# TAMUCrypto/virgo-plus

Measured on AMD Instinct MI355X. Metric: prover sec + field-ops/sec, SHA-256 circuit, 1/2/4/8 MI355X (bit-exact), higher is better.
Workload: dtype u64 (F_p^2, p=2^61-1); 1 GPU; SHA-256 1024-block circuit (SHA256_64.pws x1024, 102347776 gates, 15 layers, 2^23 input wires), GKR sumcheck + Virgo FFT/LDT commit on GPU (BASELINE configs[2]); pass_mode=sync, field_ops_per_proof=8299342697

## Files before the change

include/vpgpu.h:

```cpp
#ifndef VPGPU_H
#define VPGPU_H
#include <stdint.h>
#ifdef __cplusplus
extern "C" {
#endif

typedef struct vp_ctx vp_ctx;
typedef struct { uint64_t real, img; } vp_F;

enum {
    VP_OK = 0,
    VP_EINVAL = -1,
    VP_EHIP = -2,
    VP_ENOGPU = -3,
    VP_EASSERT = -4,
    VP_ELIMIT = -5,
    VP_EXCHANGE = 1
};

enum { VP_MUL = 0, VP_ADD, VP_SUB, VP_ANTISUB, VP_NAAB, VP_ANTINAAB, VP_INPUT, VP_MULC, VP_ADDC, VP_XOR, VP_NOT, VP_COPY };

typedef struct {
    uint64_t size;
    int32_t bit_length;
// ... 17 lines not shown
    int32_t plan_autotune;
    int32_t real_values;
    int32_t real_pairs;
    int32_t pc_tensor_pub;
    int32_t persistent_rounds;
    int32_t persistent_timeout_ms;
    int32_t poll;
    int32_t prefetch_round1;
    int32_t interactive_fast_init;
    int32_t split_cost_percent;
    int32_t debug;
    int32_t reserved[4];
} vp_options;
void vp_options_default(vp_options *opt);

int vp_create(int device, vp_ctx **out);
int vp_create_with_options(int device, const vp_options *opt, vp_ctx **out);
int vp_get_options(const vp_ctx *, vp_options *out);
int vp_tuning_get(const vp_ctx *, const char *name, int32_t *value);
int vp_test_drivers(void);
int vp_plan_tuning_get(const vp_ctx *, int32_t v[6]);
int vp_plan_tuning_set(vp_ctx *, const int32_t v[6]);
#define VP_WARM_COMMITMENT 1u
#define VP_WARM_FFT_GKR 2u
int vp_warm(vp_ctx *, uint32_t what);
void vp_destroy(vp_ctx *);
const char *vp_last_error(const vp_ctx *);
const char *vp_version(void);
int vp_checked_build(void);

int vp_circuit_upload(vp_ctx *, int n_layers, const vp_layer_desc *layers);

int vp_evaluate(vp_ctx *, const vp_F *inputs, uint64_t n_inputs);
int vp_layer_values(vp_ctx *, int layer, vp_F *out, uint64_t n);

int vp_vres(vp_ctx *, const vp_F *r_0, int r_0_size, vp_F *out);

int vp_phase1_init(vp_ctx *, int layer, const vp_F *r_liu, const vp_F *assert_random);
int vp_phase2_init(vp_ctx *, int layer, const vp_F *r_u);
int vp_liu_init(vp_ctx *, int layer, const vp_F *r_u, const vp_F *const *r_v, const vp_F *s);

int vp_round(vp_ctx *, const vp_F *previous_random, vp_F out_poly[3]);

int vp_finalize(vp_ctx *, const vp_F *previous_random, vp_F *claims, int n_claims);

int vp_prove_gkr(vp_ctx *, const vp_F *tape, uint64_t n_tape, uint8_t *transcript, uint64_t capacity,
                 uint64_t *n_written);
int vp_gkr_sizes(vp_ctx *, uint64_t *n_tape, uint64_t *n_transcript_bytes);

int vp_set_shard(vp_ctx *, int rank, int world);
int vp_set_shard_split(vp_ctx *, int min_log);
int vp_shard_finish(vp_ctx *, uint8_t *summed, uint64_t n_bytes, uint64_t *n_transcript_bytes);
int vp_set_round_shard(vp_ctx *, int rank, int world, int min_log);
int vp_get_round_shard(vp_ctx *, int *rank, int *world, int *split_live);
int vp_shard_vu_partials(vp_ctx *, const vp_F *tape, uint64_t n_tape, vp_F *partials, uint64_t capacity, uint64_t *n);
int vp_shard_vu_set(vp_ctx *, const vp_F *sums, uint64_t n);
int vp_shard_chains(vp_ctx *, int32_t *owner, double *cost, int capacity, int *n_chains);

int vp_commit_private(vp_ctx *, uint8_t root[32]);
int vp_commit_public(vp_ctx *, const vp_F *pub, uint64_t n_pub, vp_F *inner_product_sum, vp_F all_sum[65],
                     uint8_t root_h[32]);
int vp_commit_public_eq(vp_ctx *, const vp_F *point, int n_point, vp_F *inner_product_sum, vp_F all_sum[65], uint8_t root_h[32]);
int vp_fri_step(vp_ctx *, const vp_F *r, uint8_t root[32]);
int vp_fri_commit(vp_ctx *, const vp_F *r, int n_steps, uint8_t *roots);
int vp_fri_final(vp_ctx *, vp_F *final_code);
int vp_fri_open(vp_ctx *, int oracle, uint64_t leaf, vp_F values[130], uint8_t *path, int path_capacity, int *path_len);
int vp_fri_open_many(vp_ctx *, int n, const int32_t *oracle, const uint64_t *leaf, vp_F *values , uint8_t *paths, int path_stride,
                     int32_t *path_len );
int vp_fri_query_bytes(vp_ctx *, int n_queries, uint64_t *bytes);
int vp_fri_query(vp_ctx *, int n_queries, const uint64_t *leaf0, uint8_t *out, uint64_t capacity, uint64_t *n_written);
int vp_fft_gkr_sizes(int lg, uint64_t *n_tape, uint64_t *n_msgs);
int vp_fft_gkr(vp_ctx *, int lg, const vp_F *tape, uint64_t n_tape, vp_F *msgs, uint64_t capacity, uint64_t *n_written);
int vp_fft_gkr_begin(vp_ctx *, int lg, const vp_F *tape, uint64_t n_tape);
int vp_fft_gkr_end(vp_ctx *, vp_F *msgs, uint64_t capacity, uint64_t *n_written);
int vp_fft_gkr_cancel(vp_ctx *);
int vp_commit_private_masked(vp_ctx *, const vp_F *mask, uint64_t n_mask, uint8_t root[32]);
int vp_commit_public_masked(vp_ctx *, const vp_F *pub, uint64_t n_pub, const vp_F *pub_mask, uint64_t n_pub_mask, vp_F *inner, vp_F all_sum[65], uint8_t root_h[32]);
int vp_fri_final_mask(vp_ctx *, vp_F out[32]);
int vp_commit_stats(vp_ctx *, double *commit_ms);

int vp_set_deferred(vp_ctx *, int on);
int vp_flush(vp_ctx *, int count);
int vp_pending(vp_ctx *, int *n);
int vp_phase_ms(vp_ctx *, double out[5]);
int vp_commit_private_state(vp_ctx *, uint64_t *epoch, int *valid);

int vp_pc_load_input(vp_ctx *, const vp_F *inputs, uint64_t n_inputs, int bit_length);
int vp_pc_set_shard(vp_ctx *, int rank, int world);
int vp_shard_exchange_local(vp_ctx **ctxs, int world);
int vp_pc_shard_owner(vp_ctx *, int oracle, uint64_t leaf);
int vp_shard_pending(vp_ctx *, int *n);
int vp_shard_exchange_info(vp_ctx *, int i, int *kind, uint64_t *bytes);
int vp_shard_exchange_get(vp_ctx *, int i, void *host_send);
int vp_shard_exchange_put(vp_ctx *, int i, const void *host_recv);
int vp_shard_exchange_done(vp_ctx *);
int vp_comm_unique_id(uint8_t id[128]);
int vp_comm_init(vp_ctx *, const uint8_t id[128], int rank, int world);
int vp_comm_destroy(vp_ctx *);
int vp_comm_count(vp_ctx *, int *n_ranks);
int vp_allreduce_u64(vp_ctx *, void *device_buffer, uint64_t count);

int vp_predicates(vp_ctx *, int layer, const vp_F *r_g, const vp_F *assert_random, const vp_F *r_u, const vp_F *r_v, int n_v,
                  vp_F *out, uint64_t n_out);

int vp_liu_gr(vp_ctx *, int layer, const vp_F *r_u, const vp_F *const *r_v, const vp_F *s, const vp_F *r_liu, vp_F *out);
int vp_layer_mle(vp_ctx *, int layer, const vp_F *r, int n, vp_F *out);

typedef struct {
    double gkr_ms;
    double evaluate_ms;
    double fold_ms;
    uint64_t fold_launches;
    uint64_t fold_bytes;
    uint64_t rounds;
    uint64_t launches;
} vp_stats;
int vp_get_stats(vp_ctx *, vp_stats *out);
typedef struct {
    int32_t phase, layer, round, how, tables;
    uint64_t bytes;
    double us;
} vp_round_stat;
int vp_get_round_stats(vp_ctx *, vp_round_stat *out, int capacity, int *n);
int vp_get_resident_resumes(const vp_ctx *, uint64_t *n);
int vp_set_profiling(vp_ctx *, int level);

enum { VP_K_BETA = 0, VP_K_LIGHT, VP_K_CHUNKS, VP_K_COMBINE, VP_K_DOT, VP_K_DOTFIN, VP_K_SFGEN, VP_K_SF, VP_K_SEG, VP_K_EMIT,
       VP_K_FIXUP, VP_K_NTT_SPLIT, VP_K_NTT_LDS, VP_K_NTT_UNSPLIT, VP_K_LEAF_HASH, VP_K_MERKLE, VP_K_PC_POINTWISE, VP_K_FRI_FOLD,
       VP_K_ROUND, VP_K_NTT8_COLS, VP_K_NTT8_ROWS, VP_K_NTT_LONG_SPLIT, VP_K_NTT_LONG_MERGE, VP_K_PC_OPEN_MANY, VP_K_COUNT };
typedef struct {
    int32_t kind;
    int32_t step;
    uint32_t workgroups;
    uint32_t jobs;
    uint32_t rounds, first_round;
    uint64_t bytes;
    uint64_t work;
    double us;
} vp_launch_stat;
int vp_get_launch_stats(vp_ctx *, vp_launch_stat *out, int capacity, int *n);
const char *vp_kernel_name(int kind);

int vp_test_field(vp_ctx *, int op, const vp_F *a, const vp_F *b, vp_F *out, uint64_t n);
int vp_test_beta(vp_ctx *, const vp_F *r, int n, const vp_F *init, vp_F *out);
int vp_test_sha3(vp_ctx *, const uint8_t *in, uint8_t *out, uint64_t n);
int vp_test_fft(vp_ctx *, const vp_F *coefs, int coef_len, int order, int inverse, vp_F *out);

#ifdef __cplusplus
}
#endif
#endif
```

virgo-plus_amd/__init__.py:

```python
import ctypes
import os
import shutil
import subprocess

PKG_DIR = os.path.dirname(os.path.abspath(__file__))
ROOT = os.path.dirname(PKG_DIR)
CSRC = os.path.join(PKG_DIR, "csrc")
HOST = os.path.join(PKG_DIR, "host")
LIB_GPU = os.environ.get("VP_LIBGPU") or os.path.join(CSRC, "libvpgpu.so")
LIB_GPU_CHECKED = os.path.join(ROOT, "tools", "_build", "checked", "libvpgpu.so")
LIB_GPU_TESTDRV = os.path.join(ROOT, "tools", "_build", "testdrv", "libvpgpu.so")
LIB_HOST = os.path.join(HOST, "libvphost.so")
CLI = os.path.join(HOST, "virgo_plus_run")

GPU_SRC = [os.path.join(CSRC, f) for f in ("vpgpu.hip", "vpgpu_batched.inc", "vpgpu_pc.inc", "vpgpu_pc_shard.inc", "vpgpu_fftgkr.inc", "vpgpu_upload.inc", "vp_kernels_fftgkr.h", "vp_kernels.h", "vp_kernels_round.h", "vp_kernels_persist.h", "vp_kernels_batch.h",
                                              "vp_kernels_plan.h", "vp_kernels_pc.h", "vp_kernels_ntt8.h", "vp_kernels_ntt_long.h", "vp_keccak_asm.h", "vp_check.h", "vp_field.h")] + [
    os.path.join(ROOT, "include", "vpgpu.h")]
HOST_SRC = [os.path.join(HOST, f) for f in ("circuit.cpp", "prover.cpp", "verifier.cpp", "vphost.cpp")]
HOST_HDR = [os.path.join(HOST, f) for f in ("circuit.hpp", "prover.hpp", "verifier.hpp", "vphost.h", "field.hpp",
                                              "polynomial.hpp")]


def _stale(target, sources):
    if not os.path.exists(target):
# ... 10 lines not shown


def build(force=False, verbose=False):
    def run(cmd):
        if verbose:
            print(" ".join(cmd), flush=True)
        subprocess.run(cmd, check=True)

    if os.environ.get("VP_LIBGPU"):
        pass
    elif force or _stale(LIB_GPU, GPU_SRC):
        hipcc = _hipcc()
        if hipcc is None:
            if os.path.exists(LIB_GPU):
                return
            raise RuntimeError("hipcc not found and no prebuilt libvpgpu.so")
        run([hipcc, "--offload-arch=gfx950", "-O3", "-std=c++17", "-fPIC", "-shared", "-Wno-unused-value",
             "-o", LIB_GPU, os.path.join(CSRC, "vpgpu.hip")])
    if (force or _stale(LIB_GPU_CHECKED, GPU_SRC)) and _hipcc() is not None:
        os.makedirs(os.path.dirname(LIB_GPU_CHECKED), exist_ok=True)
        run([_hipcc(), "--offload-arch=gfx950", "-O3", "-std=c++17", "-fPIC", "-shared", "-Wno-unused-value", "-DVP_CHECKED",
             "-o", LIB_GPU_CHECKED, os.path.join(CSRC, "vpgpu.hip")])
    if (force or _stale(LIB_GPU_TESTDRV, GPU_SRC)) and _hipcc() is not None:
        os.makedirs(os.path.dirname(LIB_GPU_TESTDRV), exist_ok=True)
        run([_hipcc(), "--offload-arch=gfx950", "-O3", "-std=c++17", "-fPIC", "-shared", "-Wno-unused-value", "-DVP_TEST_DRIVERS",
             "-o", LIB_GPU_TESTDRV, os.path.join(CSRC, "vpgpu.hip")])
    if force or _stale(LIB_HOST, HOST_SRC + HOST_HDR + [LIB_GPU]):
        run(["g++", "-std=c++17", "-O2", "-fPIC", "-shared", "-Wall", "-pthread", "-o", LIB_HOST] + HOST_SRC +
            ["-L" + CSRC, "-lvpgpu", "-Wl,-rpath,$ORIGIN/../csrc", "-Wl,-rpath,/opt/rocm/lib"])
    if force or _stale(CLI, [os.path.join(HOST, "virgo_plus_run.cpp"), LIB_HOST]):
        run(["g++", "-std=c++17", "-O2", "-Wall", "-pthread", "-o", CLI, os.path.join(HOST, "virgo_plus_run.cpp"),
             "-L" + HOST, "-lvphost", "-L" + CSRC, "-lvpgpu", "-Wl,-rpath,$ORIGIN", "-Wl,-rpath,$ORIGIN/../csrc",
             "-Wl,-rpath,/opt/rocm/lib"])


class VphResult(ctypes.Structure):
    _fields_ = [("prove_sec", ctypes.c_double), ("gkr_device_ms", ctypes.c_double), ("evaluate_ms", ctypes.c_double),
                ("verify_sec", ctypes.c_double), ("fold_ms", ctypes.c_double), ("fold_launches", ctypes.c_uint64),
                ("fold_bytes", ctypes.c_uint64), ("rounds", ctypes.c_uint64), ("launches", ctypes.c_uint64),
                ("proof_kb", ctypes.c_double), ("verified", ctypes.c_int)]

    def as_dict(self):
        return {k: getattr(self, k) for k, _ in self._fields_}


class RoundStat(ctypes.Structure):
    _fields_ = [("phase", ctypes.c_int32), ("layer", ctypes.c_int32), ("round", ctypes.c_int32), ("how", ctypes.c_int32), ("tables", ctypes.c_int32),
                ("bytes", ctypes.c_uint64), ("us", ctypes.c_double)]


class LaunchStat(ctypes.Structure):
    _fields_ = [("kind", ctypes.c_int32), ("step", ctypes.c_int32), ("workgroups", ctypes.c_uint32), ("jobs", ctypes.c_uint32),
                ("rounds", ctypes.c_uint32), ("first_round", ctypes.c_uint32), ("bytes", ctypes.c_uint64), ("work", ctypes.c_uint64),
                ("us", ctypes.c_double)]


_gpu = None
_host = None


def lib_gpu():
    global _gpu
    if _gpu is None:
        if not os.path.exists(LIB_GPU):
            raise RuntimeError("libvpgpu.so is not built: run __graft_entry__.build()")
        L = ctypes.CDLL(LIB_GPU, mode=ctypes.RTLD_GLOBAL)
        vp = ctypes.c_void_p
        L.vp_create.argtypes = [ctypes.c_int, ctypes.POINTER(vp)]
        L.vp_create_with_options.argtypes = [ctypes.c_int, vp, ctypes.POINTER(vp)]
        L.vp_get_options.argtypes = [vp, vp]
        L.vp_get_resident_resumes.argtypes = [vp, ctypes.POINTER(ctypes.c_uint64)]
        L.vp_set_shard_split.argtypes = [vp, ctypes.c_int]
        L.vp_set_round_shard.argtypes = [vp, ctypes.c_int, ctypes.c_int, ctypes.c_int]
        L.vp_get_round_shard.argtypes = [vp, ctypes.POINTER(ctypes.c_int), ctypes.POINTER(ctypes.c_int), ctypes.POINTER(ctypes.c_int)]
        L.vp_shard_finish.argtypes = [vp, vp, ctypes.c_uint64, vp]
        L.vp_gkr_sizes.argtypes = [vp, vp, vp]
        L.vp_options_default.argtypes = [vp]
        L.vp_tuning_get.argtypes = [vp, ctypes.c_char_p, ctypes.POINTER(ctypes.c_int32)]
        u64_ = ctypes.c_uint64
        L.vp_set_deferred.argtypes = [vp, ctypes.c_int]
        L.vp_warm.argtypes = [vp, ctypes.c_uint32]
        L.vp_flush.argtypes = [vp, ctypes.c_int]
        L.vp_pending.argtypes = [vp, ctypes.POINTER(ctypes.c_int)]
        L.vp_phase_ms.argtypes = [vp, ctypes.POINTER(ctypes.c_double)]
        L.vp_commit_private.argtypes = [vp, vp]
        L.vp_fft_gkr_sizes.argtypes = [ctypes.c_int, vp, vp]
        L.vp_fft_gkr.argtypes = [vp, ctypes.c_int, vp, u64_, vp, u64_, vp]
        L.vp_fft_gkr_begin.argtypes = [vp, ctypes.c_int, vp, u64_]
        L.vp_fft_gkr_end.argtypes = [vp, vp, u64_, vp]
        L.vp_fft_gkr_cancel.argtypes = [vp]
        L.vp_options_default.restype = None
        L.vp_destroy.argtypes = [vp]
        L.vp_last_error.argtypes = [vp]
        L.vp_last_error.restype = ctypes.c_char_p
        L.vp_version.restype = ctypes.c_char_p
        L.vp_test_field.argtypes = [vp, ctypes.c_int, vp, vp, vp, ctypes.c_uint64]
        L.vp_test_beta.argtypes = [vp, vp, ctypes.c_int, vp, vp]
        L.vp_test_sha3.argtypes = [vp, vp, vp, ctypes.c_uint64]
        L.vp_test_fft.argtypes = [vp, vp, ctypes.c_int, ctypes.c_int, ctypes.c_int, vp]
        L.vp_pc_load_input.argtypes = [vp, vp, ctypes.c_uint64, ctypes.c_int]
        L.vp_pc_set_shard.argtypes = [vp, ctypes.c_int, ctypes.c_int]
        L.vp_shard_exchange_local.argtypes = [ctypes.POINTER(vp), ctypes.c_int]
        L.vp_commit_private.argtypes = [vp, vp]
        L.vp_commit_public.argtypes = [vp, vp, ctypes.c_uint64, vp, vp, vp]
        L.vp_commit_public_eq.argtypes = [vp, vp, ctypes.c_int, vp, vp, vp]
        L.vp_fri_commit.argtypes = [vp, vp, ctypes.c_int, vp]
        L.vp_fri_step.argtypes = [vp, vp, vp]
        L.vp_commit_private_masked.argtypes = [vp, vp, ctypes.c_uint64, vp]
        L.vp_shard_pending.argtypes = [vp, ctypes.POINTER(ctypes.c_int)]
        L.vp_pc_shard_owner.argtypes = [vp, ctypes.c_int, ctypes.c_uint64]
        L.vp_fri_final.argtypes = [vp, vp]
        L.vp_fri_open.argtypes = [vp, ctypes.c_int, ctypes.c_uint64, vp, vp, ctypes.c_int, ctypes.POINTER(ctypes.c_int)]
        L.vp_fri_open_many.argtypes = [vp, ctypes.c_int, vp, vp, vp, vp, ctypes.c_int, vp]
        L.vp_fri_query_bytes.argtypes = [vp, ctypes.c_int, ctypes.POINTER(ctypes.c_uint64)]
        L.vp_fri_query.argtypes = [vp, ctypes.c_int, vp, vp, ctypes.c_uint64, ctypes.POINTER(ctypes.c_uint64)]
        L.vp_commit_stats.argtypes = [vp, ctypes.POINTER(ctypes.c_double)]
        L.vp_comm_unique_id.argtypes = [vp]
        L.vp_comm_init.argtypes = [vp, vp, ctypes.c_int, ctypes.c_int]
        L.vp_comm_destroy.argtypes = [vp]
        L.vp_comm_count.argtypes = [vp, ctypes.POINTER(ctypes.c_int)]
        L.vp_get_round_stats.argtypes = [vp, ctypes.POINTER(RoundStat), ctypes.c_int, ctypes.POINTER(ctypes.c_int)]
        L.vp_allreduce_u64.argtypes = [vp, vp, ctypes.c_uint64]
        L.vp_set_profiling.argtypes = [vp, ctypes.c_int]
        L.vp_get_launch_stats.argtypes = [vp, ctypes.POINTER(LaunchStat), ctypes.c_int, ctypes.POINTER(ctypes.c_int)]
        L.vp_kernel_name.argtypes = [ctypes.c_int]
        L.vp_kernel_name.restype = ctypes.c_char_p
        _gpu = L
    return _gpu


def lib_host():
    global _host
    if _host is None:
        lib_gpu()
        if not os.path.exists(LIB_HOST):
            raise RuntimeError("libvphost.so is not built: run __graft_entry__.build()")
        L = ctypes.CDLL(LIB_HOST)
        vp = ctypes.c_void_p
        u64 = ctypes.c_uint64
        L.vph_circuit_from_pws.restype = vp
        L.vph_circuit_from_pws.argtypes = [ctypes.c_char_p, ctypes.c_int, ctypes.c_long, ctypes.c_char_p, ctypes.c_int]
        L.vph_circuit_randomize.restype = vp
        L.vph_circuit_randomize.argtypes = [ctypes.c_int, ctypes.c_int, ctypes.c_long]
        L.vph_circuit_custom.restype = vp
        L.vph_circuit_custom.argtypes = [ctypes.c_int] + [vp] * 7
        L.vph_circuit_free.argtypes = [vp]
        L.vph_circuit_layers.argtypes = [vp]
        L.vph_circuit_gates.restype = u64
        L.vph_circuit_gates.argtypes = [vp]
        L.vph_circuit_layer_size.restype = u64
        L.vph_circuit_layer_size.argtypes = [vp, ctypes.c_int]
        L.vph_circuit_layer_bitlen.argtypes = [vp, ctypes.c_int]
        L.vph_circuit_hash.argtypes = [vp, ctypes.POINTER(u64)]
        L.vph_session_create.restype = vp
        L.vph_session_create.argtypes = [vp, ctypes.c_int, ctypes.c_char_p, ctypes.c_int]
        L.vph_session_create_opts.restype = vp
        L.vph_session_create_opts.argtypes = [vp, ctypes.c_int, vp, ctypes.c_char_p, ctypes.c_int]
        L.vph_session_create_round_sharded.restype = vp
        L.vph_session_create_round_sharded.argtypes = [vp, ctypes.POINTER(ctypes.c_int), ctypes.c_int, ctypes.c_int, vp, ctypes.c_char_p, ctypes.c_int]
        L.vph_session_create_sharded.restype = vp
        L.vph_session_create_sharded.argtypes = [vp, ctypes.POINTER(ctypes.c_int), ctypes.c_int, ctypes.c_int, ctypes.c_int, vp, ctypes.c_char_p, ctypes.c_int]
        L.vph_commit_private_masked.argtypes = [vp, vp, u64, vp, ctypes.POINTER(ctypes.c_double), ctypes.c_char_p, ctypes.c_int]
        L.vph_commit_public_eq.argtypes = [vp, vp, ctypes.c_int, vp, ctypes.POINTER(ctypes.c_double), ctypes.c_char_p, ctypes.c_int]
        L.vph_fri_open_many.argtypes = [vp, ctypes.c_int, vp, vp, vp, vp, ctypes.c_int, vp, ctypes.c_char_p, ctypes.c_int]
        L.vph_fri_query.argtypes = [vp, ctypes.c_int, vp, vp, u64, ctypes.POINTER(u64), ctypes.c_char_p, ctypes.c_int]
        L.vph_session_rank_ctx.restype = vp
# ... 623 lines not shown
        if lib_host().vph_shard_vu_set(self.h, a.ctypes.data, int(a.shape[0])):
            raise RuntimeError("shard_vu_set refused")

    def shard_finish(self, summed):
        ctx = lib_host().vph_session_ctx(self.h)
        buf = ctypes.create_string_buffer(bytes(summed), len(summed))
        n = ctypes.c_uint64(0)
        if lib_gpu().vp_shard_finish(ctx, buf, len(summed), ctypes.byref(n)):
            raise RuntimeError("shard_finish refused")
        return buf.raw[:int(n.value)]

    def shard_chains(self):
        import numpy as np
        cap = 3 * self.circuit.layers + 1
        owner = np.zeros(cap, dtype=np.int32)
        cost = np.zeros(cap, dtype=np.float64)
        n = lib_host().vph_shard_chains(self.h, owner.ctypes.data, cost.ctypes.data, cap)
        if n < 0:
            raise RuntimeError("shard_chains failed")
        return owner[:n].copy(), cost[:n].copy()

    def commit_private(self, mask=None):
        root = ctypes.create_string_buffer(32)
        ms = ctypes.c_double(0)
        err = ctypes.create_string_buffer(512)
        if mask is not None:
            import numpy as np
            mask = np.ascontiguousarray(mask, dtype=np.uint64).reshape(-1, 2)
            rc = lib_host().vph_commit_private_masked(self.h, mask.ctypes.data, mask.shape[0], ctypes.cast(root, ctypes.c_void_p), ctypes.byref(ms), err, len(err))
        else:
            rc = lib_host().vph_commit_private(self.h, ctypes.cast(root, ctypes.c_void_p), ctypes.byref(ms), err, len(err))
        if rc:
            raise RuntimeError("commit_private failed: " + err.value.decode())
        return root.raw, ms.value

    def commit_public(self, pub):
        import numpy as np
        pub = np.ascontiguousarray(pub, dtype=np.uint64)
        out = ctypes.create_string_buffer(32 + 16 + 65 * 16)
        ms = ctypes.c_double(0)
        err = ctypes.create_string_buffer(512)
        rc = lib_host().vph_commit_public(self.h, pub.ctypes.data, pub.shape[0], ctypes.cast(out, ctypes.c_void_p), ctypes.byref(ms),
                                          err, len(err))
        if rc:
            raise RuntimeError("commit_public failed: " + err.value.decode())
        return out.raw[:32], out.raw[32:48], out.raw[48:], ms.value

    def prove_full(self, batched=False):
        cap = self._cap + 32 + 32 + 16 + 65 * 16
        buf = ctypes.create_string_buffer(cap)
        n = ctypes.c_uint64(0)
        err = ctypes.create_string_buffer(512)
        rc = lib_host().vph_prove_full(self.h, ctypes.cast(buf, ctypes.c_void_p), cap, ctypes.byref(n), 1 if batched else 0, err, len(err))
        if rc < 0:
            raise RuntimeError("prove_full failed: " + err.value.decode())
        return buf.raw[: n.value], rc == 0

    def commit_public_eq(self, point):
        import numpy as np
        point = np.ascontiguousarray(point, dtype=np.uint64)
        out = ctypes.create_string_buffer(32 + 16 + 65 * 16)
        if self._shard_pc:
            ms = ctypes.c_double(0)
            err = ctypes.create_string_buffer(512)
            if lib_host().vph_commit_public_eq(self.h, point.ctypes.data, point.shape[0], ctypes.cast(out, ctypes.c_void_p), ctypes.byref(ms), err, len(err)):
                raise RuntimeError("vp_commit_public_eq failed: " + err.value.decode())
            return out.raw[:32], out.raw[32:48], out.raw[48:], ms.value
        ctx = lib_host().vph_session_ctx(self.h)
        base = ctypes.addressof(out)
        rc = lib_gpu().vp_commit_public_eq(ctx, point.ctypes.data, point.shape[0], base + 32, base + 48, base)
        if rc:
            raise RuntimeError("vp_commit_public_eq failed: %d %s" % (rc, (lib_gpu().vp_last_error(ctx) or b"").decode()))
        return out.raw[:32], out.raw[32:48], out.raw[48:], self.commit_device_ms()

    def warm(self):
        ctx = lib_host().vph_session_ctx(self.h)
        if lib_gpu().vp_warm(ctx, 3):
            raise RuntimeError("vp_warm failed: " + (lib_gpu().vp_last_error(ctx) or b"").decode())

    def draw_protocol_tape(self):
        if lib_host().vph_draw_protocol_tape(self.h):
            raise RuntimeError("draw_protocol_tape: the commitment needs an input layer of at least 2^7 wires")

    def prove_protocol(self, deferred=False, queue_next=False):
        import numpy as np
        if not hasattr(self, "_pp"):
            cap = self._cap + 32 + 32 + 16 + 65 * 16
            self._pp = (ctypes.create_string_buffer(cap), cap, ctypes.create_string_buffer(32 * 32), np.zeros((2048, 2), dtype=np.uint64),
                        (ctypes.c_double * 6)(), ctypes.c_uint64(0), ctypes.create_string_buffer(512))
        buf, cap, roots, fin, sec, n, err = self._pp
        rc = lib_host().vph_prove_protocol_ex(self.h, ctypes.cast(buf, ctypes.c_void_p), cap, ctypes.byref(n), ctypes.cast(roots, ctypes.c_void_p), len(roots),
                                              fin.ctypes.data, sec, (1 if deferred or queue_next else 0) | (2 if queue_next else 0), err, len(err))
        if rc:
            raise RuntimeError("prove_protocol failed: " + err.value.decode())
        st = self.circuit.layer_bitlen(0) - 6
        return (buf.raw[: n.value], roots.raw[:32 * st], fin.copy(),
                {"total": sec[0], "commit_private": sec[1], "gkr": sec[2], "commit_public": sec[3], "fft_gkr": sec[4], "fri_commit": sec[5]})

    def prove_and_verify_full(self, reps=33, batched_openings=False):
        cap = self._cap + 32 + 32 + 16 + 65 * 16
        buf = ctypes.create_string_buffer(cap)
        n = ctypes.c_uint64(0)
        t = [ctypes.c_double(0) for _ in range(3)]
        err = ctypes.create_string_buffer(512)
        if batched_openings:
            rc = lib_host().vph_prove_and_verify_full_ex(self.h, reps, 1, ctypes.cast(buf, ctypes.c_void_p), cap, ctypes.byref(n),
                                                         ctypes.byref(t[0]), ctypes.byref(t[1]), ctypes.byref(t[2]), err, len(err))
        else:
            rc = lib_host().vph_prove_and_verify_full(self.h, reps, ctypes.cast(buf, ctypes.c_void_p), cap, ctypes.byref(n),
                                                      ctypes.byref(t[0]), ctypes.byref(t[1]), ctypes.byref(t[2]), err, len(err))
        if rc < 0:
            raise RuntimeError("prove_and_verify_full failed: " + err.value.decode())
        pt = (ctypes.c_double * 3)()
        lib_host().vph_last_pc_times(self.h, pt)
        return buf.raw[: n.value], rc == 0, {"gkr_prove_sec": t[0].value, "pc_prove_sec": t[1].value, "verify_sec": t[2].value,
                                            "pc_fft_gkr_sec": pt[1], "pc_query_answer_sec": pt[2]}

    def last_full_record(self):
        n = ctypes.c_uint64(0)
        lib_host().vph_last_full_record(self.h, None, 0, ctypes.byref(n))
        if not n.value:
            raise RuntimeError("no accepted complete-protocol run on this session yet")
        buf = ctypes.create_string_buffer(n.value)
        if lib_host().vph_last_full_record(self.h, ctypes.cast(buf, ctypes.c_void_p), n.value, ctypes.byref(n)):
            raise RuntimeError("vph_last_full_record failed")
        return buf.raw[: n.value]

    def fri_open_many(self, requests, path_stride=OPEN_PATH_STRIDE):
        if self._shard_pc:
            import numpy as np
            n = len(requests)
            oracle = np.ascontiguousarray([r[0] for r in requests], dtype=np.int32).reshape(n)
            leaf = np.ascontiguousarray([r[1] for r in requests], dtype=np.uint64).reshape(n)
            v = np.zeros((max(n, 1), 130, 2), dtype=np.uint64)
            p = np.zeros((max(n, 1), max(path_stride, 1)), dtype=np.uint8)
            pl = np.zeros(max(n, 1), dtype=np.int32)
            err = ctypes.create_string_buffer(512)
            if lib_host().vph_fri_open_many(self.h, n, oracle.ctypes.data, leaf.ctypes.data, v.ctypes.data, p.ctypes.data, path_stride, pl.ctypes.data, err, len(err)):
                raise RuntimeError("vp_fri_open_many failed: " + err.value.decode())
            return v[:n], p[:n], pl[:n]
        ctx = self.gpu_ctx()
        rc, v, p, pl = fri_open_many(ctx, requests, path_stride)
        if rc:
            raise RuntimeError("vp_fri_open_many failed: %d %s" % (rc, (lib_gpu().vp_last_error(ctx) or b"").decode()))
        return v, p, pl

    def fri_query(self, leaf0):
        if self._shard_pc:
            import numpy as np
            leaf0 = np.ascontiguousarray(leaf0, dtype=np.uint64)
            n_bits = self.circuit.layer_bitlen(0)
            cap = leaf0.shape[0] * sum(2080 + 32 * d for d in [n_bits - 1, n_bits - 1] + [n_bits - 2 - k for k in range(n_bits - 6)])
            out = ctypes.create_string_buffer(max(cap, 1))
            n = ctypes.c_uint64(0)
            err = ctypes.create_string_buffer(512)
            if lib_host().vph_fri_query(self.h, leaf0.shape[0], leaf0.ctypes.data, ctypes.cast(out, ctypes.c_void_p), cap, ctypes.byref(n), err, len(err)):
                raise RuntimeError("vp_fri_query failed: " + err.value.decode())
            return out.raw[: n.value]
        ctx = self.gpu_ctx()
        rc, out = fri_query(ctx, leaf0)
        if rc:
            raise RuntimeError("vp_fri_query failed: %d %s" % (rc, (lib_gpu().vp_last_error(ctx) or b"").decode()))
        return out

    def last_fft_gkr(self):
        import numpy as np
        out = np.zeros((4096, 2), dtype=np.uint64)
        n = lib_host().vph_last_fft_gkr(self.h, out.ctypes.data, out.shape[0])
        if n < 0:
            raise RuntimeError("no complete-protocol run on this session yet")
        return out[:n].tobytes()

    def last_fri(self):
        import numpy as np
        roots = ctypes.create_string_buffer(32 * 32)
# ... 50 lines not shown
```

virgo-plus_amd/csrc/vpgpu.hip:

```cpp
#include <hip/hip_runtime.h>

#include <algorithm>
#include <chrono>
#include <cstdio>
#include <cstring>
#include <deque>
#include <functional>
#include <map>
#include <mutex>
#include <set>
#include <atomic>
#include <string>
#include <thread>
#include <vector>

#include "../../include/vpgpu.h"
#include "vp_kernels.h"

using namespace vp;

static_assert(sizeof(vp_F) == sizeof(F), "vp_F layout");

namespace {

// ... 113 lines not shown
    int32_t persistent_rounds, poll, debug, prefetch_round1, split_cost_percent;
    int32_t kernel_copies;
    int32_t fold_branches;
    int32_t fuse_combine;
    int32_t plan_autotune, pc_tensor_pub, persistent_timeout_ms;
    int32_t graph_explicit;
    int32_t ntt_r8;
    int32_t interactive_fast_init;
    int32_t fuse_p2;
    int32_t leaf_asm;
    int32_t real_pairs;
    int32_t fft_gkr_batched;
    int32_t split_vu;
};

struct vp_ctx {
    int device = 0;
    hipStream_t stream = nullptr;
    std::string err = "";
    int n_layers = 0, max_bl = 0;
    std::vector<LayerDev> L;
    F **d_vals = nullptr;
    unsigned long long **d_valsr = nullptr;
    F *beta_g = nullptr, *beta_u = nullptr, *bf = nullptr, *bs = nullptr, *liu_half = nullptr;
    u32 half_cap = 0;
    F *tab[2][3] = {{nullptr, nullptr, nullptr}, {nullptr, nullptr, nullptr}};
    u32 cap = 0;
    F *partials = nullptr;
    unsigned int *round_arrivals = nullptr;
    F *small = nullptr;
    F *chunk_part = nullptr; u32 chunk_cap = 0;
    F *d_tape = nullptr; u64 n_tape = 0;
    F *d_tr = nullptr; u64 n_tr = 0;
    F *h_pin = nullptr;
    unsigned long long *h_seq = nullptr, seq = 0;
    TailMail *h_req = nullptr; TailReply *h_rep = nullptr; std::atomic<bool> tail_active{false}; unsigned long long tail_seq = 0; int tail_enabled = 1;
    PTailArgs tail_args{}; F *tail_save = nullptr; bool tail_suspended = false, tail_lost = false; u64 tail_resumes = 0;
    TailAux *h_aux = nullptr;
    int poll = 1;
    F *h_io = nullptr; size_t h_io_cap = 0;
    int r1_pending = 0;
    vp_F r1_stash[3];
    F *h_stage = nullptr; u32 stage_at = 0;
    VpOpt opt{};
    int *d_flag = nullptr;
    u32 *d_vcplx = nullptr;
    int vreal = 0, plan_vreal = 0;
    bool evaluated = false;
    SumcheckState sc;
    std::vector<u64> ru_off, as_off, rv_off, sig_off, rliu_off;
    int profiling = 0;
    vp_stats st{};
    std::vector<EvPair> ev_pool; size_t ev_used = 0;
    std::vector<vp_launch_stat> lstats;
    std::vector<vp_round_stat> rlog;
    int rlog_round = 0;
    u64 rec_gen_bytes = 0, rec_gen_work = 0;
    hipEvent_t ev0 = nullptr, ev1 = nullptr;
    std::vector<void *> allocs;
    BetaJob *all_jobs = nullptr; u32 n_all_jobs = 0, beta_bpj = 1; F *half_pool = nullptr;
    F *pc_rt = nullptr, *pc_coef = nullptr, *pc_cw = nullptr; Dig *pc_tree = nullptr; int pc_lm = -1; double commit_ms = 0;
    std::map<std::pair<const void *, int>, F *> pc_rtc;
    F *pc_q0 = nullptr, *pc_eq = nullptr, *pc_cbuf = nullptr; int pc_cbuf_lm = -1; int *pc_flag = nullptr; bool pc_q_tensor = false;
    F *pc_pub = nullptr, *pc_qcw = nullptr, *pc_hcw = nullptr, *pc_tmp = nullptr, *pc_small = nullptr; Dig *pc_tree_h = nullptr; bool pc_private_done = false;
    F *pc_scr = nullptr; size_t pc_scr_cap = 0;
    F *pc_fri_all = nullptr; std::vector<size_t> fri_cw_off, fri_tree_off; F *pc_open_buf = nullptr;
    PcOpenRec *pc_many_buf = nullptr; unsigned char *pc_many_in = nullptr; u32 pc_many_cap = 0; unsigned char *h_many = nullptr; size_t h_many_cap = 0;
    Dig *pc_fri_roots = nullptr;
    F *pc_fri[2] = {nullptr, nullptr}; Dig *pc_fri_tree = nullptr; int fri_step = -1; size_t fri_tree_used = 0; bool pc_public_done = false;
    u32 pc_mask_ms = 0; F *pc_lm_cw = nullptr, *pc_qm_cw = nullptr, *pc_hm_cw = nullptr, *pc_fm = nullptr, *pc_mtmp = nullptr; std::vector<size_t> fri_m_off;
    size_t pc_mtmp_cap = 0, pc_mB = 0;

    int deferred = 0;
    struct Pending { hipEvent_t a, b; int phase; std::function<int(float)> fin; };
    std::deque<Pending> pending;
    std::vector<hipEvent_t> ev_spare;
    unsigned char *h_ring = nullptr; size_t ring_cap = 0, ring_at = 0;
    size_t ring_live = 0, ring_call = 0;
    double phase_ms[8] = {0, 0, 0, 0, 0, 0, 0, 0};
    std::string plan_cache_path;
    bool pc_dry = false;
    unsigned char *h_pub = nullptr; size_t h_pub_cap = 0;
    u64 private_epoch = 0;

    PcShard *pcs = nullptr;
    FgkState *fgk = nullptr;
    VpComm *cm = nullptr;
    F *part2 = nullptr;
    int simple_path = 0, serial = 0;
    Lane lane0; Lane *ln = nullptr;
    std::vector<Lane> lanes;
    std::vector<hipStream_t> lane_streams; std::vector<hipEvent_t> lane_events; hipEvent_t ev_fork = nullptr;
    F *pred_r = nullptr, *pred_pool = nullptr, *pred_part = nullptr, *pred_out = nullptr; BetaJob *pred_jobs = nullptr; u32 pred_bpj = 1;
    DotJob *pred_dot = nullptr; BlkMap *pred_map = nullptr;
    PlanRec *rec = nullptr;
    DotJob rec_dot{};
    SfGenJob rec_gen{};
    int fuse_init = 1;
    Plan *plan = nullptr; int plan_path = 1;
    std::recursive_mutex mu;
    bool plan_tuned = false;
    bool plan_tune_cached = false;
    int leaf_attr_done = 0;
    uint32_t opt_pinned = 0;
    hipGraphExec_t gkr_graph = nullptr; int use_graph = 1; bool graph_failed = false; u64 graph_launches = 0, graph_rounds = 0;
    int shard_rank = 0, shard_world = 1;
    int split_lw = 0, split_min_log = 11;
    struct SplitTab { int j, bl; u32 slot0; };
    struct SplitChain { u64 poly_pos = 0, claims_pos = 0, r_off = 0; int rounds = 0, has_a = 1, n_tab = 0, small_owner = 0; std::vector<SplitTab> tabs; };
    std::vector<SplitChain> split;
    F *d_trs = nullptr; u64 n_exp = 0;
    F *tr_base() const { return (split_lw > 0 && d_trs) ? d_trs : d_tr; }
    std::vector<int> chain_owner;
    std::vector<double> chain_cost;
    bool drop_round1 = false;
    std::vector<FixJob> rec_fix;
    bool owned(int chain) const { return shard_world <= 1 || chain_owner.empty() || chain_owner[chain] == shard_rank; }
    bool vu_supplied = false; float vu_pre_ms = 0; u64 vu_tape_tag = 0;
    RoundShard *rsh = nullptr;
    bool sc_open = false;

    F *zero() const { return small; }
    F *one() const { return small + 1; }
    F *add_term() const { return small + 2; }
    F *Vu() const { return small + 3; }
    F *coef() const { return small + 4; }
    F *scalarV() const { return small + 32; }
};

namespace {

#define HIPCHK(x)                                                                                   \
    do {                                                                                            \
        hipError_t e_ = (x);                                                                        \
        if (e_ != hipSuccess) {                                                                     \
            ctx->err = std::string(#x) + ": " + hipGetErrorString(e_);                              \
            return VP_EHIP;                                                                         \
        }                                                                                           \
    } while (0)
#define VPCHK(x) do { int r_ = (x); if (r_ != VP_OK) return r_; } while (0)
int tail_quit(vp_ctx *ctx);
void vp_suspend_others(vp_ctx *ctx);
static thread_local int tl_entry_depth = 0;
struct CtxLock {
    vp_ctx *c;
    CtxLock(vp_ctx *ctx, bool suspend_others) : c(ctx) {
        if (suspend_others && tl_entry_depth == 0) vp_suspend_others(ctx);
        c->mu.lock(); ++tl_entry_depth;
    }
    ~CtxLock() { --tl_entry_depth; c->mu.unlock(); }
    CtxLock(const CtxLock &) = delete; CtxLock &operator=(const CtxLock &) = delete;
};
#define VP_LOCK(ctx) CtxLock vp_ctx_lock_(ctx, false)
int flush_pending(vp_ctx *ctx, size_t count);
#define VP_ENTER_Q(ctx) CtxLock vp_ctx_lock_(ctx, true); do { HIPCHK(hipSetDevice((ctx)->device)); if ((ctx)->tail_active) (void) tail_quit(ctx); (ctx)->tail_suspended = false; (ctx)->tail_lost = false; (ctx)->ring_call = 0; } while (0)
#define VP_ENTER(ctx) VP_ENTER_Q(ctx); do { if (!(ctx)->pending.empty()) VPCHK(flush_pending((ctx), (size_t) -1)); } while (0)

constexpr u32 MAX_BLOCKS = 2048;

template <class T>
int dalloc(vp_ctx *ctx, T **p, size_t n) {
    *p = nullptr;
    if (n == 0) n = 1;
    HIPCHK(hipMalloc((void **) p, n * sizeof(T)));
    ctx->allocs.push_back((void *) *p);
    return VP_OK;
}
template <class T>
int dupload(vp_ctx *ctx, T **p, const std::vector<T> &h) {
    VPCHK(dalloc(ctx, p, h.size()));
    if (!h.empty()) HIPCHK(hipMemcpy(*p, h.data(), h.size() * sizeof(T), hipMemcpyHostToDevice));
    return VP_OK;
}
void free_all(vp_ctx *ctx) {
    for (void *p : ctx->allocs) (void) hipFree(p);
    ctx->allocs.clear();
}

inline u32 nblk(u64 n) { return (u32) ((n + VP_BLOCK - 1) / VP_BLOCK); }
inline u32 grid_for(u64 n) { return std::max<u32>(1, std::min<u32>(nblk(n), MAX_BLOCKS)); }
inline int ceil_log2(u64 x) { int b = 0; while ((1ull << b) < x) ++b; return b; }
inline bool is_unary(int ty) { return ty == VP_ADDC || ty == VP_MULC || ty == VP_COPY || ty == VP_NOT; }

void count_launch(vp_ctx *ctx) { ++ctx->st.launches; }

int prof_begin(vp_ctx *ctx, hipStream_t st, int kind, u32 grid, u32 jobs, u64 bytes, u64 work, u32 rounds = 0, u32 first_round = 0) {
    if (!ctx->profiling || ctx->ev_used >= ctx->ev_pool.size()) return -1;
    EvPair &e = ctx->ev_pool[ctx->ev_used];
    e.kind = kind; e.grid = grid; e.jobs = jobs; e.bytes = bytes; e.work = work; e.rounds = rounds; e.first_round = first_round;
    hipEventRecord(e.a, st);
    return (int) ctx->ev_used++;
}
void prof_end(vp_ctx *ctx, hipStream_t st, int slot) { if (slot >= 0) hipEventRecord(ctx->ev_pool[slot].b, st); }
void prof_collect(vp_ctx *ctx) {
    ctx->lstats.clear();
    for (size_t e = 0; e < ctx->ev_used; ++e) {
        const EvPair &p = ctx->ev_pool[e];
        float t = 0;
        if (hipEventElapsedTime(&t, p.a, p.b) != hipSuccess) t = 0;
        vp_launch_stat s{};
        s.kind = p.kind; s.step = (int) e; s.workgroups = p.grid; s.jobs = p.jobs; s.rounds = p.rounds; s.first_round = p.first_round;
        s.bytes = p.bytes; s.work = p.work; s.us = 1e3 * (double) t;
        ctx->lstats.push_back(s);
    }
}

int run_beta_half(vp_ctx *ctx, const F *r, int n, const F *init) {
    hipLaunchKernelGGL(k_beta_half, dim3(1), dim3(VP_BLOCK), 0, ctx->stream, r, n, init, ctx->bf, ctx->bs);
    count_launch(ctx);
    return VP_OK;
}

template <int PHASE>
int run_init_rows(vp_ctx *ctx, const Csr &c, InitArgs &a) {
    a.rowptr = c.rowptr; a.e_g = c.e_g; a.e_x = c.e_x; a.e_tl = c.e_tl; a.n_rows = c.n_rows;
    if (c.n_rows) {
        hipLaunchKernelGGL(k_init_light<PHASE>, dim3(nblk(c.n_rows)), dim3(VP_BLOCK), 0, ctx->stream, a);
        count_launch(ctx);
    }
    if (c.n_chunks) {
        hipLaunchKernelGGL(k_init_chunks<PHASE>, dim3((c.n_chunks + 3) / 4), dim3(VP_BLOCK), 0, ctx->stream, a,
                           c.chunk_beg, c.chunk_end, c.n_chunks, ctx->chunk_part);
        hipLaunchKernelGGL(k_init_combine, dim3((c.n_heavy + 3) / 4), dim3(VP_BLOCK), 0, ctx->stream, c.heavy_row,
                           c.heavy_cptr, c.n_heavy, ctx->chunk_part, a.M, a.A);
        count_launch(ctx); count_launch(ctx);
    }
    return VP_OK;
}

int do_phase1_init(vp_ctx *ctx, int i, const F *d_rliu, const F *d_assert) {
    LayerDev &cur = ctx->L[i], &pre = ctx->L[i - 1];
    VPCHK(run_beta_half(ctx, d_rliu, cur.bl, ctx->one()));
    hipLaunchKernelGGL(k_beta_expand, dim3(grid_for(cur.size)), dim3(VP_BLOCK), 0, ctx->stream, ctx->bf, ctx->bs,
                       cur.bl >> 1, (u32) cur.size, ctx->beta_g);
    count_launch(ctx);
    if (cur.n_assert) {
        hipLaunchKernelGGL(k_scale_entries, dim3(nblk(cur.n_assert)), dim3(VP_BLOCK), 0, ctx->stream, ctx->beta_g,
// ... 620 lines not shown
              (o->fuse_min_log != d.fuse_min_log ? 8u : 0u) | (o->sf3b_grid != d.sf3b_grid ? 16u : 0u) | (o->graph_explicit != d.graph_explicit ? 32u : 0u);
    return VP_OK;
}

int vp_plan_tuning_get(const vp_ctx *ctx, int32_t v[6]) {
    if (!ctx || !v) return VP_EINVAL;
    v[0] = ctx->opt.fuse_combine; v[1] = ctx->opt.fold_branches; v[2] = ctx->opt.plan_align; v[3] = ctx->opt.fuse_min_log; v[4] = ctx->opt.sf3b_grid; v[5] = ctx->opt.graph_explicit;
    return VP_OK;
}
int vp_plan_tuning_set(vp_ctx *ctx, const int32_t v[6]) {
    if (!ctx || !v) return VP_EINVAL;
    if (v[0] < 0 || v[0] > 2 || v[1] < 0 || v[1] > 1 || v[2] < 0 || v[2] > 2 || v[3] < 0 || v[3] > 30 || v[4] < 1 || v[4] > 4096 || v[5] < 0 || v[5] > 3) return VP_EINVAL;
    VP_ENTER(ctx);
    if (ctx->plan || ctx->gkr_graph) { ctx->err = "vp_plan_tuning_set: the context has already recorded its launch plan"; return VP_EINVAL; }
    ctx->opt.fuse_combine = v[0]; ctx->opt.fold_branches = v[1]; ctx->opt.plan_align = v[2]; ctx->opt.fuse_min_log = v[3]; ctx->opt.sf3b_grid = v[4]; ctx->opt.graph_explicit = v[5];
    ctx->plan_tuned = true;
    return VP_OK;
}
int vp_create(int device, vp_ctx **out) { return vp_create_with_options(device, nullptr, out); }
int vp_get_options(const vp_ctx *ctx, vp_options *out) {
    if (!ctx || !out) return VP_EINVAL;
    opt_to_public(ctx->opt, out);
    return VP_OK;
}

static std::recursive_mutex g_rand_mu;
struct RandKeep {
    char priv[128]; char *caller;
    RandKeep() { g_rand_mu.lock(); memset(priv, 0, sizeof priv); caller = initstate(1u, priv, sizeof priv); }
    ~RandKeep() { if (caller) setstate(caller); g_rand_mu.unlock(); }
};

int vp_create_with_options(int device, const vp_options *user, vp_ctx **out) {
    if (!out) return VP_EINVAL;
    *out = nullptr;
    RandKeep keep_callers_random_stream;
    int n = 0;
    if (hipGetDeviceCount(&n) != hipSuccess || n <= 0 || device < 0 || device >= n) return VP_ENOGPU;
    if (hipSetDevice(device) != hipSuccess) return VP_ENOGPU;
    vp_ctx *ctx = new vp_ctx();
    ctx->device = device;
    if (resolve_options(&ctx->opt, user, &ctx->opt_pinned) != VP_OK) { delete ctx; return VP_EINVAL; }
    if (const char *pcf = getenv("VP_PLAN_CACHE")) ctx->plan_cache_path = pcf;
    if (hipStreamCreateWithFlags(&ctx->stream, hipStreamNonBlocking) != hipSuccess) { delete ctx; return VP_EHIP; }
    if (hipHostMalloc((void **) &ctx->h_pin, (4 + VP_MAX_TAB) * sizeof(F), hipHostMallocDefault) != hipSuccess) {
        delete ctx; return VP_EHIP;
    }
    if (hipHostMalloc((void **) &ctx->h_seq, 64, hipHostMallocDefault) != hipSuccess) { delete ctx; return VP_EHIP; }
    *ctx->h_seq = 0;
    if (hipHostMalloc((void **) &ctx->h_req, sizeof(TailMail), hipHostMallocDefault) != hipSuccess ||
        hipHostMalloc((void **) &ctx->h_rep, sizeof(TailReply), hipHostMallocDefault) != hipSuccess) { delete ctx; return VP_EHIP; }
    if (hipHostMalloc((void **) &ctx->h_aux, sizeof(TailAux), hipHostMallocDefault) != hipSuccess) { delete ctx; return VP_EHIP; }
    if (hipHostMalloc((void **) &ctx->h_stage, 4096 * sizeof(F), hipHostMallocDefault) != hipSuccess) { delete ctx; return VP_EHIP; }
    memset(ctx->h_req, 0, sizeof(TailMail)); memset(ctx->h_rep, 0, sizeof(TailReply)); memset(ctx->h_aux, 0, sizeof(TailAux));
    (void) hipFuncSetAttribute(reinterpret_cast<const void *>(k_phase), hipFuncAttributeMaxDynamicSharedMemorySize, 3 * 2 * VP_PH_PMAX * (int) sizeof(F));
    ctx->poll = ctx->opt.poll; ctx->tail_enabled = ctx->opt.persistent_rounds;
    hipEventCreate(&ctx->ev0); hipEventCreate(&ctx->ev1);
    (void) hipFuncSetAttribute(reinterpret_cast<const void *>(k_emit_multi), hipFuncAttributeMaxDynamicSharedMemorySize, 160 * 1024 - 256);
    (void) hipFuncSetAttribute(reinterpret_cast<const void *>(k_emit), hipFuncAttributeMaxDynamicSharedMemorySize, 160 * 1024 - 256);
    (void) hipFuncSetAttribute(reinterpret_cast<const void *>(k_ntt_lds), hipFuncAttributeMaxDynamicSharedMemorySize, 160 * 1024 - 256);
    (void) hipFuncSetAttribute(reinterpret_cast<const void *>(k_ntt8_cols<false>), hipFuncAttributeMaxDynamicSharedMemorySize, 80 * 1024);
    (void) hipFuncSetAttribute(reinterpret_cast<const void *>(k_ntt8_cols<true>), hipFuncAttributeMaxDynamicSharedMemorySize, 80 * 1024);
    (void) hipFuncSetAttribute(reinterpret_cast<const void *>(k_ntt8_rows<false>), hipFuncAttributeMaxDynamicSharedMemorySize, 80 * 1024);
    (void) hipFuncSetAttribute(reinterpret_cast<const void *>(k_ntt8_rows<true>), hipFuncAttributeMaxDynamicSharedMemorySize, 80 * 1024);
    { std::lock_guard<std::mutex> lk(g_ctx_mu); g_ctxs.push_back(ctx); }
    *out = ctx;
    return VP_OK;
}

static void free_plan(vp_ctx *ctx);
void vp_free_shard_state(vp_ctx *ctx);
void vp_free_comm(vp_ctx *ctx);
void vp_free_fgk(vp_ctx *ctx);

static void rs_free(vp_ctx *ctx);
void vp_destroy(vp_ctx *ctx) {
    if (!ctx) return;
    if (tl_entry_depth == 0) vp_suspend_others(ctx);
    { std::lock_guard<std::mutex> lk(g_ctx_mu); g_ctxs.erase(std::remove(g_ctxs.begin(), g_ctxs.end(), ctx), g_ctxs.end()); }
    { std::lock_guard<std::recursive_mutex> lo(ctx->mu); }
    (void) hipSetDevice(ctx->device);
    if (ctx->tail_active) (void) tail_quit(ctx);
    (void) hipStreamSynchronize(ctx->stream);
    vp_free_shard_state(ctx);
    rs_free(ctx);
    vp_free_comm(ctx);
    vp_free_fgk(ctx);
    if (ctx->gkr_graph) (void) hipGraphExecDestroy(ctx->gkr_graph);
    free_plan(ctx);
    free_all(ctx);
    for (auto &e : ctx->ev_pool) { (void) hipEventDestroy(e.a); (void) hipEventDestroy(e.b); }
    if (ctx->ev0) (void) hipEventDestroy(ctx->ev0);
    if (ctx->ev1) (void) hipEventDestroy(ctx->ev1);
    if (ctx->h_pin) (void) hipHostFree(ctx->h_pin);
    if (ctx->h_seq) (void) hipHostFree(ctx->h_seq);
    if (ctx->h_req) (void) hipHostFree(ctx->h_req);
    if (ctx->h_rep) (void) hipHostFree(ctx->h_rep);
    if (ctx->h_aux) (void) hipHostFree(ctx->h_aux);
    if (ctx->h_stage) (void) hipHostFree(ctx->h_stage);
    if (ctx->h_io) (void) hipHostFree(ctx->h_io);
    if (ctx->h_ring) (void) hipHostFree(ctx->h_ring);
    if (ctx->h_pub) (void) hipHostFree(ctx->h_pub);
    if (ctx->h_many) (void) hipHostFree(ctx->h_many);
    for (auto &p : ctx->pending) { (void) hipEventDestroy(p.a); (void) hipEventDestroy(p.b); }
    for (auto e : ctx->ev_spare) (void) hipEventDestroy(e);
    for (auto st : ctx->lane_streams) (void) hipStreamDestroy(st);
    for (auto ev : ctx->lane_events) (void) hipEventDestroy(ev);
    if (ctx->ev_fork) (void) hipEventDestroy(ctx->ev_fork);
    (void) hipStreamDestroy(ctx->stream);
    delete ctx;
}

int vp_circuit_upload(vp_ctx *ctx, int n_layers, const vp_layer_desc *ld) {
    if (!ctx || !ld || n_layers < 2) return VP_EINVAL;
    if (n_layers > VP_MAX_TAB) { ctx->err = "too many layers"; return VP_ELIMIT; }
    RandKeep keep_callers_random_stream;
    VP_ENTER(ctx);
    HIPCHK(hipStreamSynchronize(ctx->stream));
    if (ctx->gkr_graph) { (void) hipGraphExecDestroy(ctx->gkr_graph); ctx->gkr_graph = nullptr; }
    ctx->graph_failed = false; ctx->plan_tuned = false; ctx->plan_tune_cached = false;
    free_plan(ctx);
    vp_free_shard_state(ctx);
    free_all(ctx);
    ctx->L.assign(n_layers, LayerDev());
    ctx->n_layers = n_layers;
    ctx->evaluated = false;
    ctx->chain_owner.clear(); ctx->chain_cost.clear();
    ctx->chunk_cap = 0;
    ctx->pred_r = ctx->pred_pool = ctx->pred_part = ctx->pred_out = nullptr; ctx->pred_jobs = nullptr; ctx->pred_dot = nullptr; ctx->pred_map = nullptr;
    ctx->pc_rt = ctx->pc_coef = ctx->pc_cw = nullptr; ctx->pc_tree = nullptr; ctx->pc_lm = -1; ctx->pc_rtc.clear();
    ctx->pc_pub = ctx->pc_qcw = ctx->pc_hcw = ctx->pc_tmp = ctx->pc_small = nullptr; ctx->pc_tree_h = nullptr; ctx->pc_private_done = false;
    ctx->pc_q0 = nullptr; ctx->pc_eq = nullptr; ctx->pc_cbuf = nullptr; ctx->pc_cbuf_lm = -1; ctx->pc_flag = nullptr; ctx->pc_q_tensor = false;
    ctx->pc_scr = nullptr; ctx->pc_scr_cap = 0; ctx->pc_fri_all = nullptr; ctx->pc_open_buf = nullptr; ctx->pc_many_buf = nullptr; ctx->pc_many_in = nullptr; ctx->pc_many_cap = 0; ctx->fri_cw_off.clear(); ctx->fri_tree_off.clear();
    ctx->pc_fri[0] = ctx->pc_fri[1] = nullptr; ctx->pc_fri_tree = nullptr; ctx->pc_fri_roots = nullptr; ctx->fri_step = -1; ctx->pc_public_done = false;
    ctx->pc_mask_ms = 0; ctx->pc_lm_cw = ctx->pc_qm_cw = ctx->pc_hm_cw = ctx->pc_fm = ctx->pc_mtmp = nullptr; ctx->fri_m_off.clear(); ctx->pc_mtmp_cap = 0; ctx->pc_mB = 0;
    int max_bl = 0;
    for (int i = 0; i < n_layers; ++i) {
        if (ld[i].size == 0 || ld[i].size > (1ull << 30) || ld[i].bit_length < 0 || ld[i].bit_length > 30 ||
            (1ull << ld[i].bit_length) < ld[i].size) { ctx->err = "bad layer size"; return VP_ELIMIT; }
        max_bl = std::max(max_bl, (int) ld[i].bit_length);
    }
    ctx->max_bl = max_bl;
    UpScratch S;
    const bool up_dbg = (ctx->opt.debug & 2) != 0;
    const auto up_t0 = std::chrono::steady_clock::now();
    auto up_since = [&]() { return std::chrono::duration<double>(std::chrono::steady_clock::now() - up_t0).count(); };
    u64 *d_sizes = nullptr;
    {
        std::vector<u64> sizes(n_layers);
        for (int i = 0; i < n_layers; ++i) sizes[i] = ld[i].size;
        VPCHK(dupload(ctx, &d_sizes, sizes));
    }
    for (int i = 0; i < n_layers; ++i) {
        LayerDev &D = ctx->L[i];
        const vp_layer_desc &L = ld[i];
        D.size = L.size; D.bl = L.bit_length;
        const u64 nval = i == 0 ? (1ull << L.bit_length) : L.size;
        VPCHK(dalloc(ctx, &D.val, nval));
        if (i == 0) continue;
        if (!L.ty || !L.l || !L.u || !L.v || !L.lv || !L.dad_size || !L.dad_bitlen || !L.dad_id) { ctx->err = "layer arrays missing"; return VP_EINVAL; }
        VPCHK(upload_layer_dev(ctx, S, i, ld, d_sizes));
    }
    if (up_dbg) fprintf(stderr, "[vp_circuit_upload] layers %.3f s", up_since());
    u32 cap = 0;
    for (int i = 1; i < n_layers; ++i) cap = std::max<u32>(cap, std::max<u32>(1u << ctx->L[i - 1].bl, ctx->L[i].p2_total));
    ctx->cap = cap;
    for (int b = 0; b < 2; ++b) for (int t = 0; t < 3; ++t) VPCHK(dalloc(ctx, &ctx->tab[b][t], (size_t) cap));
    VPCHK(dalloc(ctx, &ctx->beta_g, (size_t) 1 << max_bl));
    VPCHK(dalloc(ctx, &ctx->beta_u, (size_t) 1 << max_bl));
    ctx->half_cap = 1u << ((max_bl + 1) / 2);
    VPCHK(dalloc(ctx, &ctx->bf, (size_t) ctx->half_cap));
    VPCHK(dalloc(ctx, &ctx->bs, (size_t) ctx->half_cap));
    VPCHK(dalloc(ctx, &ctx->liu_half, (size_t) 2 * (n_layers + 1) * ctx->half_cap));
    VPCHK(dalloc(ctx, &ctx->partials, (size_t) 3 * MAX_BLOCKS));
    VPCHK(dalloc(ctx, &ctx->round_arrivals, (size_t) 16)); HIPCHK(hipMemsetAsync(ctx->round_arrivals, 0, 64, ctx->stream));
    VPCHK(dalloc(ctx, &ctx->chunk_part, (size_t) 2 * std::max<u32>(1, ctx->chunk_cap)));
    VPCHK(dalloc(ctx, &ctx->small, (size_t) 32 + VP_MAX_TAB));
    VPCHK(dalloc(ctx, &ctx->d_flag, (size_t) 1));
    VPCHK(dalloc(ctx, &ctx->d_vcplx, (size_t) 1));
    {
        std::vector<F> sm(32 + VP_MAX_TAB, f_zero());
        sm[1] = f_one();
        HIPCHK(hipMemcpy(ctx->small, sm.data(), sm.size() * sizeof(F), hipMemcpyHostToDevice));
        std::vector<F *> vals(n_layers);
        for (int i = 0; i < n_layers; ++i) vals[i] = ctx->L[i].val;
        VPCHK(dupload(ctx, &ctx->d_vals, vals));
    }
    if (up_dbg) fprintf(stderr, "  shared %.3f", up_since());
    compute_layout(ctx);
    VPCHK(dalloc(ctx, &ctx->d_tape, (size_t) ctx->n_tape));
    VPCHK(dalloc(ctx, &ctx->d_tr, (size_t) ctx->n_tr + 3 + VP_MAX_TAB));
    HIPCHK(hipMemset(ctx->d_tape, 0, ctx->n_tape * sizeof(F)));
    for (int i = 1; i < n_layers; ++i) {
        LayerDev &D = ctx->L[i];
        std::vector<BetaJob> jobs;
        const u32 hc = ctx->half_cap;
        auto add = [&](const F *r, const F *init, int nbits, int k) {
            BetaJob jb{};
            const size_t q = jobs.size();
            jb.r = r; jb.init = init; jb.bf = ctx->liu_half + 2 * q * hc; jb.bs = ctx->liu_half + (2 * q + 1) * hc; jb.n = nbits;
// ... 47 lines not shown
            D.job_hg = hg_id[i]; D.job_hu = hu_id[i]; D.job_liu0 = liu_id[i].front(); D.job_liun = (int) liu_id[i].size();
            std::vector<Half> hs;
            for (int q : liu_id[i]) hs.push_back(half_of(q));
            VPCHK(dupload(ctx, &D.liu_H, hs));
            VPCHK(upload_liu_dev(ctx, S, i));
        }
    if (up_dbg) fprintf(stderr, "  liulists %.3f", up_since());
        VPCHK(dalloc(ctx, &ctx->part2, (size_t) 32 * MAX_BLOCKS * 3));
        VPCHK(dalloc(ctx, &ctx->tail_save, (size_t) 3 * 2 * VP_PH_PMAX + 8 + VP_MAX_TAB));
        ctx->lane0.stream = ctx->stream;
        for (int b = 0; b < 2; ++b) for (int t = 0; t < 3; ++t) ctx->lane0.tab[b][t] = ctx->tab[b][t];
        ctx->lane0.part2 = ctx->part2; ctx->lane0.chunk_part = ctx->chunk_part; ctx->lane0.Vu = ctx->Vu();
        ctx->ln = &ctx->lane0;
        const int n_lanes = 2 * (n_layers - 1);
        while ((int) ctx->lane_streams.size() < std::max(n_lanes, 3)) {
            hipStream_t st; hipEvent_t ev;
            HIPCHK(hipStreamCreateWithFlags(&st, hipStreamNonBlocking));
            HIPCHK(hipEventCreateWithFlags(&ev, hipEventDisableTiming));
            ctx->lane_streams.push_back(st); ctx->lane_events.push_back(ev);
        }
        if (!ctx->ev_fork) HIPCHK(hipEventCreateWithFlags(&ctx->ev_fork, hipEventDisableTiming));
        ctx->lanes.assign(n_lanes + (n_layers - 1), Lane());
        F *vus = nullptr;
        VPCHK(dalloc(ctx, &vus, (size_t) n_layers));
        for (int i = 1; i < n_layers; ++i) {
            for (int h = 0; h < 2; ++h) {
                Lane &ln = ctx->lanes[2 * (i - 1) + h];
                ln.stream = ctx->lane_streams[2 * (i - 1) + h];
                ln.done = ctx->lane_events[2 * (i - 1) + h];
                const size_t capi = h == 0 ? std::max<size_t>((size_t) 1 << ctx->L[i - 1].bl, ctx->L[i].p2_total) : ((size_t) 1 << ctx->L[i - 1].bl);
                for (int b = 0; b < 2; ++b) for (int t = 0; t < 3; ++t) {
                    if (h == 1 && t == 2) { ln.tab[b][t] = ctx->tab[0][2]; continue; }
                    VPCHK(dalloc(ctx, &ln.tab[b][t], capi));
                }
                VPCHK(dalloc(ctx, &ln.part2, (size_t) 16 * MAX_BLOCKS * 3));
                const u32 nch = h == 0 ? std::max(ctx->L[i].c1.n_chunks, ctx->L[i].c2.n_chunks) : 0;
                VPCHK(dalloc(ctx, &ln.chunk_part, (size_t) 2 * std::max<u32>(1, nch)));
                ln.Vu = vus + i;
            }
            if (ctx->L[i].max_dad_bl != -1) {
                Lane &ln = ctx->lanes[n_lanes + (i - 1)];
                ln.stream = ctx->stream;
                for (int b = 0; b < 2; ++b) for (int t = 0; t < 3; ++t) VPCHK(dalloc(ctx, &ln.tab[b][t], std::max<size_t>(1, ctx->L[i].p2_total)));
                VPCHK(dalloc(ctx, &ln.part2, (size_t) 16 * MAX_BLOCKS * 3));
                VPCHK(dalloc(ctx, &ln.chunk_part, (size_t) 2 * std::max<u32>(1, ctx->L[i].c2.n_chunks)));
                VPCHK(dalloc(ctx, &ln.dot_part, (size_t) nblk(ctx->L[i - 1].size) + 1));
                ln.Vu = vus + i;
            }
        }
        ctx->serial = ctx->opt.serial; ctx->use_graph = ctx->opt.use_graph;
        ctx->simple_path = ctx->opt.gkr_path == VP_PATH_SIMPLE;
        ctx->plan_path = ctx->opt.gkr_path == VP_PATH_LANES ? 0 : 1;
        ctx->fuse_init = ctx->opt.fuse_init;
    }
    if (up_dbg) fprintf(stderr, "  total %.3f s\n", up_since());
#ifdef VP_CHECKED
    {
        VpChkDesc d{};
        d.n_layers = (unsigned) n_layers;
        unsigned long long cap = 1;
        for (int i = 0; i < n_layers; ++i) {
            d.lsize[i] = (unsigned) ctx->L[i].size;
            cap = std::max<unsigned long long>(cap, 1ull << ctx->L[i].bl);
            cap = std::max<unsigned long long>(cap, ctx->L[i].p2_total);
            d.n_liu_tables_max = std::max<unsigned>(d.n_liu_tables_max, (unsigned) ctx->L[i].job_liun);
        }
        d.table_cap = cap;
        if (getenv("VP_CHECKED_INJECT")) d.lsize[0] = 1;
        HIPCHK(hipMemcpyToSymbol(HIP_SYMBOL(g_vp_chk), &d, sizeof d));
        const unsigned int z[4] = {0, 0, 0, 0};
        HIPCHK(hipMemcpyToSymbol(HIP_SYMBOL(g_vp_chk_err), z, sizeof z));
    }
#endif
    if (ctx->ev_pool.empty()) {
        ctx->ev_pool.resize(1024);
        for (auto &e : ctx->ev_pool) { hipEventCreate(&e.a); hipEventCreate(&e.b); e.bytes = 0; e.kind = -1; e.grid = e.jobs = e.rounds = e.first_round = 0; e.work = 0; }
    }
    return VP_OK;
}

int vp_evaluate(vp_ctx *ctx, const vp_F *inputs, uint64_t n_inputs) {
    if (!ctx || !inputs || ctx->n_layers < 2 || n_inputs != ctx->L[0].size) return VP_EINVAL;
    VP_ENTER(ctx);
    LayerDev &L0 = ctx->L[0];
    ctx->pc_private_done = false; ctx->pc_public_done = false; ctx->pc_mask_ms = 0;
    HIPCHK(hipEventRecord(ctx->ev0, ctx->stream));
    HIPCHK(hipMemsetAsync(L0.val, 0, (sizeof(F) << L0.bl), ctx->stream));
    HIPCHK(hipMemcpyAsync(L0.val, inputs, n_inputs * sizeof(F), hipMemcpyHostToDevice, ctx->stream));
    HIPCHK(hipMemsetAsync(ctx->d_flag, 0, sizeof(int), ctx->stream));
    HIPCHK(hipMemsetAsync(ctx->d_vcplx, 0, sizeof(u32), ctx->stream));
    hipLaunchKernelGGL(k_mark_complex, dim3(nblk(L0.size)), dim3(VP_BLOCK), 0, ctx->stream, L0.val, (u32) L0.size, ctx->d_vcplx);
    for (int i = 1; i < ctx->n_layers; ++i) {
        LayerDev &D = ctx->L[i];
        hipLaunchKernelGGL(k_evaluate_layer, dim3(nblk(D.size)), dim3(VP_BLOCK), 0, ctx->stream, i, (u32) D.size, D.ty,
                           D.gl, D.gu, D.gv, D.gc, ctx->d_vals, ctx->d_vcplx);
        if (D.n_assert)
            hipLaunchKernelGGL(k_check_asserts, dim3(nblk(D.n_assert)), dim3(VP_BLOCK), 0, ctx->stream, D.assert_idx,
                               D.n_assert, D.val, ctx->d_flag);
    }
    HIPCHK(hipEventRecord(ctx->ev1, ctx->stream));
    int flag = 0; u32 vcplx = 1;
    HIPCHK(hipMemcpyAsync(&flag, ctx->d_flag, sizeof(int), hipMemcpyDeviceToHost, ctx->stream));
    HIPCHK(hipMemcpyAsync(&vcplx, ctx->d_vcplx, sizeof(u32), hipMemcpyDeviceToHost, ctx->stream));
    VPCHK(check_stream(ctx));
    ctx->vreal = (vcplx == 0 && ctx->opt.real_values) ? 1 : 0;
    if (ctx->vreal) {
        std::vector<unsigned long long *> vr(ctx->n_layers);
        for (int i = 0; i < ctx->n_layers; ++i) {
            LayerDev &D = ctx->L[i];
            if (!D.valr) VPCHK(dalloc(ctx, &D.valr, (size_t) D.size));
            hipLaunchKernelGGL(k_real_parts, dim3(nblk(D.size)), dim3(VP_BLOCK), 0, ctx->stream, D.val, (u32) D.size, D.valr);
            vr[i] = D.valr;
        }
        if (!ctx->d_valsr) VPCHK(dalloc(ctx, &ctx->d_valsr, (size_t) ctx->n_layers));
        HIPCHK(hipMemcpyAsync(ctx->d_valsr, vr.data(), vr.size() * sizeof(unsigned long long *), hipMemcpyHostToDevice, ctx->stream));
        HIPCHK(hipStreamSynchronize(ctx->stream));
    }
    float ms = 0;
    hipEventElapsedTime(&ms, ctx->ev0, ctx->ev1);
    ctx->st.evaluate_ms = ms;
    ctx->evaluated = true;
    HIPCHK(hipMemsetAsync(ctx->add_term(), 0, sizeof(F), ctx->stream));
    if (flag) { ctx->err = "assert gate is non-zero"; return VP_EASSERT; }
    return VP_OK;
}

int vp_layer_values(vp_ctx *ctx, int layer, vp_F *out, uint64_t n) {
    if (!ctx || !out || layer < 0 || layer >= ctx->n_layers || n > ctx->L[layer].size) return VP_EINVAL;
    VP_ENTER(ctx);
    VPCHK(check_stream(ctx));
    HIPCHK(hipMemcpy(out, ctx->L[layer].val, n * sizeof(F), hipMemcpyDeviceToHost));
    return VP_OK;
}

static int stage(vp_ctx *ctx, u64 off, const vp_F *src, u64 n) {
    if (!n) return VP_OK;
    if (!src || off + n > ctx->n_tape) return VP_EINVAL;
    if (n > 1024) { HIPCHK(hipMemcpy(ctx->d_tape + off, src, n * sizeof(F), hipMemcpyHostToDevice)); return VP_OK; }
    if (ctx->stage_at + n > 4096) ctx->stage_at = 0;
    F *slot = ctx->h_stage + ctx->stage_at;
    memcpy(slot, src, n * sizeof(F));
    ctx->stage_at += (u32) n;
    HIPCHK(hipMemcpyAsync(ctx->d_tape + off, slot, n * sizeof(F), hipMemcpyHostToDevice, ctx->stream));
    return VP_OK;
}
static int round1_prefetch(vp_ctx *ctx) {
    ctx->r1_pending = 0;
    if (!ctx->opt.prefetch_round1 || ctx->sc.total_rounds < 1 || ctx->profiling) return check_stream(ctx);
    const F zero = f_zero();
    if (tail_try_launch(ctx, zero)) { ctx->r1_pending = 1; return VP_OK; }
    VPCHK(do_round(ctx, nullptr, zero, ctx->d_tr + ctx->n_tr, ctx->h_pin));
    ctx->r1_pending = 2;
    return VP_OK;
}

int vp_predicates(vp_ctx *ctx, int layer, const vp_F *r_g, const vp_F *assert_random, const vp_F *r_u, const vp_F *r_v, int n_v,
                  vp_F *out, uint64_t n_out) {
    if (!ctx || layer < 1 || layer >= ctx->n_layers || !assert_random || !out) return VP_EINVAL;
    LayerDev &D = ctx->L[layer], &pre = ctx->L[layer - 1];
    if ((D.bl > 0 && !r_g) || (pre.bl > 0 && !r_u)) return VP_EINVAL;
    if (n_v < 0 || n_v > 31 || (n_v > 0 && !r_v) || n_out != D.p_buckets) { ctx->err = "vp_predicates: bad sizes"; return VP_EINVAL; }
    VP_ENTER(ctx);
    if (!ctx->pred_r) {
        u32 max_chunks = 1, max_buckets = 1;
        for (int i = 1; i < ctx->n_layers; ++i) { max_chunks = std::max(max_chunks, ctx->L[i].p_chunks); max_buckets = std::max(max_buckets, ctx->L[i].p_buckets); }
        VPCHK(dalloc(ctx, &ctx->pred_r, (size_t) 3 * 32 + 2));
// ... 385 lines not shown
    {
        LayerDev &T = ctx->L[n - 1];
        VPCHK(run_beta_half(ctx, ctx->d_tape, T.bl, ctx->one()));
        hipLaunchKernelGGL(k_vres, dim3(1), dim3(VP_BLOCK), 0, ctx->stream, ctx->bf, ctx->bs, T.bl >> 1, T.val,
                           (u32) T.size, tr + pos, (F *) nullptr);
        count_launch(ctx);
        pos += 1;
    }
    for (int i = n - 1; i >= 1; --i) {
        const int pbl = ctx->L[i - 1].bl;
        const F *ru = ctx->d_tape + ctx->ru_off[i];
        VPCHK(do_phase1_init(ctx, i, rliu_ptr(ctx, i), ctx->d_tape + ctx->as_off[i]));
        for (int j = 0; j < pbl; ++j) { VPCHK(do_round(ctx, j ? ru + (j - 1) : ctx->zero(), zero, tr + pos, nullptr)); pos += 3; }
        VPCHK(do_finalize(ctx, pbl ? ru + (pbl - 1) : ctx->zero(), zero, tr + pos, nullptr));
        pos += 1;
        const int mdb = ctx->L[i].max_dad_bl;
        if (mdb != -1) {
            const F *rv = ctx->d_tape + ctx->rv_off[i];
            VPCHK(do_phase2_init(ctx, i, ru));
            for (int j = 0; j < mdb; ++j) { VPCHK(do_round(ctx, j ? rv + (j - 1) : ctx->zero(), zero, tr + pos, nullptr)); pos += 3; }
            VPCHK(do_finalize(ctx, mdb ? rv + (mdb - 1) : ctx->zero(), zero, tr + pos, nullptr));
            pos += i;
        }
        const F *rl = ctx->d_tape + ctx->rliu_off[i];
        VPCHK(do_liu_init(ctx, i));
        for (int j = 0; j < pbl; ++j) { VPCHK(do_round(ctx, j ? rl + (j - 1) : ctx->zero(), zero, tr + pos, nullptr)); pos += 3; }
        VPCHK(do_finalize(ctx, pbl ? rl + (pbl - 1) : ctx->zero(), zero, tr + pos, nullptr));
        pos += 1;
    }
    HIPCHK(hipEventRecord(ctx->ev1, ctx->stream));
    if (pos != ctx->n_tr) { ctx->err = "internal: transcript size"; return VP_EINVAL; }
    HIPCHK(hipMemcpyAsync(transcript, tr, pos * sizeof(F), hipMemcpyDeviceToHost, ctx->stream));
    VPCHK(check_stream(ctx));
    float ms = 0;
    hipEventElapsedTime(&ms, ctx->ev0, ctx->ev1);
    ctx->st.gkr_ms = ms;
    ctx->st.fold_ms = 0; ctx->st.fold_bytes = 0; ctx->st.fold_launches = ctx->ev_used;
    if (ctx->profiling) prof_collect(ctx);
    for (size_t e = 0; e < ctx->ev_used; ++e) {
        float t = 0;
        hipEventElapsedTime(&t, ctx->ev_pool[e].a, ctx->ev_pool[e].b);
        ctx->st.fold_ms += t; ctx->st.fold_bytes += ctx->ev_pool[e].bytes;
    }
    if (n_written) *n_written = pos * sizeof(F);
    return VP_OK;
#endif
}

int vp_get_stats(vp_ctx *ctx, vp_stats *out) {
    if (!ctx || !out) return VP_EINVAL;
    VP_LOCK(ctx);
    *out = ctx->st;
    return VP_OK;
}
int vp_get_resident_resumes(const vp_ctx *cctx, uint64_t *n) {
    if (!cctx || !n) return VP_EINVAL;
    vp_ctx *ctx = const_cast<vp_ctx *>(cctx);
    VP_LOCK(ctx);
    *n = ctx->tail_resumes;
    return VP_OK;
}
int vp_get_round_stats(vp_ctx *ctx, vp_round_stat *out, int capacity, int *n) {
    if (!ctx || !n || (capacity > 0 && !out)) return VP_EINVAL;
    VP_LOCK(ctx);
    *n = (int) ctx->rlog.size();
    for (int i = 0; i < *n && i < capacity; ++i) out[i] = ctx->rlog[i];
    return VP_OK;
}
int vp_set_deferred(vp_ctx *ctx, int on) {
    if (!ctx) return VP_EINVAL;
    VP_ENTER_Q(ctx);
    ctx->deferred = on ? 1 : 0;
    return VP_OK;
}
int vp_pending(vp_ctx *ctx, int *n) {
    if (!ctx || !n) return VP_EINVAL;
    VP_LOCK(ctx);
    *n = (int) ctx->pending.size();
    return VP_OK;
}
int vp_flush(vp_ctx *ctx, int count) {
    if (!ctx) return VP_EINVAL;
    VP_ENTER_Q(ctx);
    return flush_pending(ctx, count < 0 ? (size_t) -1 : (size_t) count);
}
int vp_phase_ms(vp_ctx *ctx, double out[5]) {
    if (!ctx || !out) return VP_EINVAL;
    VP_LOCK(ctx);
    for (int i = 0; i < 5; ++i) out[i] = ctx->phase_ms[i];
    return VP_OK;
}
int vp_commit_private_state(vp_ctx *ctx, uint64_t *epoch, int *valid) {
    if (!ctx || !epoch || !valid) return VP_EINVAL;
    VP_LOCK(ctx);
    *epoch = ctx->private_epoch;
    *valid = ctx->pc_private_done && !ctx->pcs ? 1 : 0;
    return VP_OK;
}
int vp_set_profiling(vp_ctx *ctx, int level) {
    if (!ctx) return VP_EINVAL;
    ctx->profiling = level;
    return VP_OK;
}
int vp_get_launch_stats(vp_ctx *ctx, vp_launch_stat *out, int capacity, int *n) {
    if (!ctx || !n || (capacity > 0 && !out)) return VP_EINVAL;
    VP_LOCK(ctx);
    *n = (int) ctx->lstats.size();
    for (int i = 0; i < *n && i < capacity; ++i) out[i] = ctx->lstats[i];
    return VP_OK;
}
const char *vp_kernel_name(int kind) {
    static const char *names[VP_K_COUNT] = {"k_beta_half_direct", "k_light_multi", "k_chunks_multi", "k_combine_multi", "k_dot_multi", "k_dotfin_multi",
        "k_sumfold3b_gen_multi", "k_sumfold3b_multi", "k_seg_multi", "k_emit_multi", "k_fixup", "k_ntt_split", "k_ntt_lds", "k_ntt_unsplit",
        "k_leaf_hash", "k_merkle", "k_pc_pointwise", "k_fri_fold", "k_round", "k_ntt8_cols", "k_ntt8_rows",
        "k_ntt_long_split", "k_ntt_long_merge", "k_pc_open_many"};
    return (kind >= 0 && kind < VP_K_COUNT) ? names[kind] : "?";
}

int vp_test_field(vp_ctx *ctx, int op, const vp_F *a, const vp_F *b, vp_F *out, uint64_t n) {
    if (!ctx || !a || !b || !out || op < 0 || op > 38) return VP_EINVAL;
    const unsigned group = op == 32 || op == 33 ? 8 : op == 34 || op == 35 ? 4 : op == 36 ? 2 : 1;
    if (n % group) return VP_EINVAL;
    if (n == 0) return VP_OK;
    VP_ENTER(ctx);
    F *da = nullptr, *db = nullptr, *dout = nullptr;
    HIPCHK(hipMalloc((void **) &da, n * sizeof(F)));
    HIPCHK(hipMalloc((void **) &db, n * sizeof(F)));
    HIPCHK(hipMalloc((void **) &dout, n * sizeof(F)));
    HIPCHK(hipMemcpy(da, a, n * sizeof(F), hipMemcpyHostToDevice));
    HIPCHK(hipMemcpy(db, b, n * sizeof(F), hipMemcpyHostToDevice));
    const dim3 grid((unsigned) ((n / group + 255) / 256));
    if (op <= 3) hipLaunchKernelGGL(k_test_field, grid, dim3(256), 0, ctx->stream, op, da, db, dout, (u64) n);
    else if (op <= 31) hipLaunchKernelGGL(k_test_field_lazy, grid, dim3(256), 0, ctx->stream, op, da, db, dout, (u64) n);
    else if (op <= 36) hipLaunchKernelGGL(k_test_field_dft, grid, dim3(256), 0, ctx->stream, op, da, dout, (u64) (n / group));
    else hipLaunchKernelGGL(k_test_field_sum, grid, dim3(256), 0, ctx->stream, op, da, db, dout, (u64) n);
    int rc = check_stream(ctx);
    if (rc == VP_OK && hipMemcpy(out, dout, n * sizeof(F), hipMemcpyDeviceToHost) != hipSuccess) rc = VP_EHIP;
    (void) hipFree(da); (void) hipFree(db); (void) hipFree(dout);
    return rc;
}

int vp_test_beta(vp_ctx *ctx, const vp_F *r, int n, const vp_F *init, vp_F *out) {
    if (!ctx || !init || !out || n < 0 || n > 28 || (n && !r)) return VP_EINVAL;
    VP_ENTER(ctx);
    F *dr = nullptr, *dbf = nullptr, *dbs = nullptr, *dout = nullptr;
    const size_t half = (size_t) 1 << ((n + 1) / 2);
    HIPCHK(hipMalloc((void **) &dr, (n + 2) * sizeof(F)));
    HIPCHK(hipMalloc((void **) &dbf, half * sizeof(F)));
    HIPCHK(hipMalloc((void **) &dbs, half * sizeof(F)));
    HIPCHK(hipMalloc((void **) &dout, sizeof(F) << n));
    if (n) HIPCHK(hipMemcpy(dr, r, n * sizeof(F), hipMemcpyHostToDevice));
    HIPCHK(hipMemcpy(dr + n, init, sizeof(F), hipMemcpyHostToDevice));
    hipLaunchKernelGGL(k_beta_half, dim3(1), dim3(VP_BLOCK), 0, ctx->stream, dr, n, dr + n, dbf, dbs);
    hipLaunchKernelGGL(k_beta_expand, dim3(grid_for(1ull << n)), dim3(VP_BLOCK), 0, ctx->stream, dbf, dbs, n >> 1,
                       (u32) (1u << n), dout);
    int rc = check_stream(ctx);
    if (rc == VP_OK && hipMemcpy(out, dout, sizeof(F) << n, hipMemcpyDeviceToHost) != hipSuccess) rc = VP_EHIP;
    (void) hipFree(dr); (void) hipFree(dbf); (void) hipFree(dbs); (void) hipFree(dout);
    return rc;
}

}

#include "vpgpu_batched.inc"
#include "vpgpu_pc.inc"
#include "vpgpu_pc_shard.inc"
#include "vpgpu_fftgkr.inc"
// ... 1 lines not shown
```

virgo-plus_amd/csrc/vpgpu_pc.inc:

```
namespace {

constexpr int PC_MAX_LN = 13;
#ifndef VP_NTT_SPLIT_LOG
#define VP_NTT_SPLIT_LOG 12
#endif
constexpr int PC_SPLIT_LN = VP_NTT_SPLIT_LOG;

#define PC_PROF(kind, grid, jobs, bytes, work, launch)                                                   \
    do {                                                                                                  \
        const int sl_ = prof_begin(ctx, ctx->stream, (kind), (u32) (grid), (u32) (jobs), (u64) (bytes), (u64) (work)); \
        launch;                                                                                           \
        prof_end(ctx, ctx->stream, sl_);                                                                  \
    } while (0)

F host_pow(F x, unsigned __int128 e) { F r = f_one(); while (e) { if (e & 1) r = f_mul(r, x); x = f_mul(x, x); e >>= 1; } return r; }
F host_root_of_unity(int log_order) {
    F r = f_make(2147483648ull, 1033321771269002680ull);
    for (int i = 0; i < 62 - log_order; ++i) r = f_mul(r, r);
    return r;
}
F host_inv_real(u64 x) { return host_pow(f_make(x, 0), (unsigned __int128) P61 - 2); }

int pc_root_table(vp_ctx *ctx, int lm) {
    if (ctx->pc_lm == lm && ctx->pc_rt) return VP_OK;
// ... 224 lines not shown
    if (ctx->pc_dry) { const F *rtp = nullptr; return pc_compact_roots(ctx, lm, PC_SPLIT_LN, &rtp); }
    F *s1 = ctx->pc_scr;
    SplitArgs sa{};
    sa.in = in; sa.out = s1; sa.RT = ctx->pc_rt; sa.half_m = 1u << (lm - 1); sa.ln = ln; sa.l1 = l1; sa.inverse = inverse;
    sa.in_stride = in_stride; sa.ncoset = nc;
    const dim3 g1(nblk(N2), rows, nc);
    {
        const u64 tr = (u64) rows * nc;
        const int sl_ = prof_begin(ctx, ctx->stream, VP_K_NTT_SPLIT, (u32) (nblk(N2) * rows * nc), (u32) tr, 32ull * N * tr,
                                   tr * (split_dft_mults(l1) * (N >> l1) + (N - (N >> l1)) + (!inverse && nc > 1 ? N : 0)));
        if (l1 == 5) hipLaunchKernelGGL(k_ntt_split<5>, g1, dim3(VP_BLOCK), 0, ctx->stream, sa);
        else if (l1 == 1) hipLaunchKernelGGL(k_ntt_split<1>, g1, dim3(VP_BLOCK), 0, ctx->stream, sa);
        else if (l1 == 2) hipLaunchKernelGGL(k_ntt_split<2>, g1, dim3(VP_BLOCK), 0, ctx->stream, sa);
        else if (l1 == 3) hipLaunchKernelGGL(k_ntt_split<3>, g1, dim3(VP_BLOCK), 0, ctx->stream, sa);
        else hipLaunchKernelGGL(k_ntt_split<4>, g1, dim3(VP_BLOCK), 0, ctx->stream, sa);
        prof_end(ctx, ctx->stream, sl_);
    }
    NttArgs a{};
    a.in = s1; a.RT = ctx->pc_rt; a.half_m = 1u << (lm - 1); a.lm = lm; a.ln = PC_SPLIT_LN; a.inverse = inverse;
    a.in_stride = N2; a.inv_n = f_one();
    VPCHK(pc_compact_roots(ctx, lm, PC_SPLIT_LN, &a.RTp));
    a.half_p = a.RTp == ctx->pc_rt ? a.half_m : 1u << (PC_SPLIT_LN - 1);
    const u32 long_rows = rows * nc;
    for (u32 r0 = 0; r0 < long_rows; r0 += 1024) {
        NttArgs b = a;
        const u32 nr = std::min<u32>(1024, long_rows - r0);
        b.in = s1 + (size_t) r0 * N; b.out = out + (size_t) r0 * N;
        b.scat_l1 = l1; b.scat_rows = nr; b.scat_do_scale = inverse ? 1 : 0; b.scat_scale = inverse ? host_inv_real(1ull << ln) : f_one();
        const u64 nt = (u64) ((nr + 7) / 8 * 8) << l1;
        PC_PROF(VP_K_NTT_LDS, nt, (u64) nr << l1, 32ull * N2 * ((u64) nr << l1), ((u64) nr << l1) * ntt_lds_mults(PC_SPLIT_LN) + (inverse ? (u64) N * nr : 0),
                hipLaunchKernelGGL(k_ntt_lds, dim3((u32) nt, 1), dim3(1024), sizeof(F) << PC_SPLIT_LN, ctx->stream, b));
    }
    return VP_OK;
}

static inline u32 pc_leaf_wg(const vp_ctx *ctx, u64 n_leaves) {
#ifdef VP_CHECKED
    (void) ctx; (void) n_leaves; return 0;
#else
    if (!ctx->opt.leaf_asm) return 0;
    return n_leaves >= (1u << 18) ? 1024u : n_leaves >= (1u << 17) ? 512u : 0u;
#endif
}
static inline size_t pc_leaf_lds(u32 wg) { return wg == 1024 ? 0 : 96 * 1024; }
static inline int pc_leaf_prepare(vp_ctx *ctx) {
    if (ctx->leaf_attr_done) return ctx->leaf_attr_done > 0 ? VP_OK : VP_EHIP;
    hipError_t err = hipFuncSetAttribute((const void *) k_leaf_hash, hipFuncAttributeMaxDynamicSharedMemorySize, 96 * 1024);
    if (err == hipSuccess) err = hipFuncSetAttribute((const void *) k_leaf_hash_multi, hipFuncAttributeMaxDynamicSharedMemorySize, 96 * 1024);
    ctx->leaf_attr_done = err == hipSuccess ? 1 : -1;
    if (err != hipSuccess) { ctx->err = "hipFuncSetAttribute (leaf hash)"; return VP_EHIP; }
    return VP_OK;
}
static inline u32 pc_leaf_blocks(u32 wg, u64 n_leaves) { const u32 th = wg ? wg : VP_BLOCK; return (u32) ((n_leaves + th - 1) / th); }
static inline void pc_launch_leaf_hash(vp_ctx *ctx, const F *cw, u32 N, Dig *leaves) {
    const u32 n_leaves = 16 * N, wg = pc_leaf_wg(ctx, n_leaves);
    if (wg && pc_leaf_prepare(ctx) == VP_OK) hipLaunchKernelGGL(k_leaf_hash, dim3(pc_leaf_blocks(wg, n_leaves)), dim3(wg), pc_leaf_lds(wg), ctx->stream, cw, N, 64, leaves);
    else hipLaunchKernelGGL(k_leaf_hash_c, dim3(nblk(n_leaves)), dim3(VP_BLOCK), 0, ctx->stream, cw, N, 64, leaves);
}
static inline u32 pc_launch_leaf_hash_multi(vp_ctx *ctx, FriLeafArgs &la) {
    u64 all = 0;
    for (int q = 0; q < la.n; ++q) all += la.N[q] >= 2 ? 16ull * la.N[q] : 16ull;
    u32 wg = pc_leaf_wg(ctx, all);
    if (wg && pc_leaf_prepare(ctx) != VP_OK) wg = 0;
    u32 blocks = 0, leaves = 0;
    for (int q = 0; q < la.n; ++q) {
        const u32 nl = la.N[q] >= 2 ? 16 * la.N[q] : 16u;
        la.blk_start[q] = blocks; la.leaf_start[q] = leaves;
        blocks += nblk(nl); leaves += nl;
    }
    la.blk_start[la.n] = blocks; la.leaf_start[la.n] = leaves;
    if (wg) { blocks = pc_leaf_blocks(wg, leaves); hipLaunchKernelGGL(k_leaf_hash_multi, dim3(blocks), dim3(wg), pc_leaf_lds(wg), ctx->stream, la); }
    else hipLaunchKernelGGL(k_leaf_hash_multi_c, dim3(blocks), dim3(VP_BLOCK), 0, ctx->stream, la);
    return blocks;
}

int pc_merkle(vp_ctx *ctx, Dig *tree, u32 n_leaves) {
    u32 c = n_leaves >> 1;
    for (; c > 512; c >>= 1)
        PC_PROF(VP_K_MERKLE, nblk(c), 1, 96ull * c, c, hipLaunchKernelGGL(k_merkle_level, dim3(nblk(c)), dim3(VP_BLOCK), 0, ctx->stream, tree, c, c));
    if (c >= 1) PC_PROF(VP_K_MERKLE, 1, 1, 96ull * 2 * c, 2 * c - 1, hipLaunchKernelGGL(k_merkle_top, dim3(1), dim3(VP_BLOCK), 0, ctx->stream, tree, 2 * c));
    return VP_OK;
}

int pcs_commit_private(vp_ctx *ctx, uint8_t root[32]);
int pcs_commit_public(vp_ctx *ctx, const vp_F *pub, uint64_t n_pub, const vp_F *point, vp_F *inner, vp_F all_sum[65], uint8_t root_h[32]);
int pcs_fri_commit(vp_ctx *ctx, const vp_F *r, int n_steps, uint8_t *roots);
int pcs_fri_step(vp_ctx *ctx, const vp_F *r, uint8_t root[32]);
bool pcs_private_done(vp_ctx *ctx);
bool pcs_public_done(vp_ctx *ctx);
int pcs_fri_done(vp_ctx *ctx);
bool pcs_fri_one_pass(vp_ctx *ctx);
int pcs_fri_final(vp_ctx *ctx, vp_F *final_code);
int pcs_fri_open(vp_ctx *ctx, int oracle, uint64_t leaf, vp_F values[130], uint8_t *path, int path_capacity, int *path_len);
int pcs_open_desc(vp_ctx *ctx, int oracle, PcOpenDesc *d);
bool pcs_owns(vp_ctx *ctx, uint64_t leaf);

constexpr int PC_MANY_PIECE = 4096, PC_MANY_MAX = 1 << 16;
static inline size_t pc_many_in_bytes(u32 cap) { return VP_OPEN_MAX_ORACLES * sizeof(PcOpenDesc) + (size_t) cap * sizeof(uint2); }
static int pc_many_reserve(vp_ctx *ctx, u32 want) {
    want = std::min<u32>(want, PC_MANY_PIECE);
    if (ctx->pc_many_buf && ctx->pc_many_cap >= want) return VP_OK;
    const u32 cap = want <= 1024 ? 1024 : PC_MANY_PIECE;
    const size_t hb = pc_many_in_bytes(cap) + (size_t) cap * sizeof(PcOpenRec);
    if (ctx->h_many_cap < hb) {
        if (ctx->h_many) (void) hipHostFree(ctx->h_many);
        ctx->h_many = nullptr; ctx->h_many_cap = 0;
        HIPCHK(hipHostMalloc((void **) &ctx->h_many, hb, hipHostMallocDefault));
        ctx->h_many_cap = hb;
    }
    ctx->pc_many_cap = 0;
    VPCHK(dalloc(ctx, &ctx->pc_many_buf, (size_t) cap));
    VPCHK(dalloc(ctx, &ctx->pc_many_in, pc_many_in_bytes(cap)));
    ctx->pc_many_cap = cap;
    return VP_OK;
}
static int pc_open_desc(vp_ctx *ctx, int oracle, PcOpenDesc *d) {
    *d = PcOpenDesc{};
    if (oracle < 0 || ctx->L.empty()) return VP_EINVAL;
    if (oracle >= VP_OPEN_MAX_ORACLES) { ctx->err = "FRI level not committed yet"; return VP_EINVAL; }
    if (ctx->pcs) return pcs_open_desc(ctx, oracle, d);
    const int n = ctx->L[0].bl, ln = n - 6, lm = n - 1;
    const u32 N = 1u << ln, M = 1u << lm;
    if (oracle == 0) { if (!ctx->pc_private_done) return VP_EINVAL; d->cw = ctx->pc_cw; d->tree = ctx->pc_tree; d->Nc = N; d->n_leaves = M >> 1; }
    else if (oracle == 1) { if (!ctx->pc_public_done) return VP_EINVAL; d->cw = ctx->pc_hcw; d->tree = ctx->pc_tree_h; d->Nc = N; d->n_leaves = M >> 1; }
    else {
        const int lvl = oracle - 2;
        if (lvl >= ctx->fri_step || lvl >= (int) ctx->fri_cw_off.size()) { ctx->err = "FRI level not committed yet"; return VP_EINVAL; }
        d->cw = ctx->pc_fri_all + ctx->fri_cw_off[lvl]; d->tree = ctx->pc_fri_tree + ctx->fri_tree_off[lvl];
        d->Nc = N >> (lvl + 1); d->n_leaves = 16 * d->Nc;
    }
    if (ctx->pc_mask_ms) d->mask = oracle == 0 ? ctx->pc_lm_cw : oracle == 1 ? ctx->pc_hm_cw : (oracle - 2 < (int) ctx->fri_m_off.size() ? ctx->pc_fm + ctx->fri_m_off[oracle - 2] : nullptr);
    return VP_OK;
}
static inline int pc_open_depth(u32 n_leaves) { int depth = 0; while ((1u << depth) < n_leaves) ++depth; return depth; }
struct PcManyPlan { PcOpenDesc tab[VP_OPEN_MAX_ORACLES]; std::vector<int> plen, dlen; u64 bytes = 0, layout = 0; };
static int pc_many_plan(vp_ctx *ctx, int n, const int32_t *oracle, const uint64_t *leaf, int path_stride, PcManyPlan &pl) {
    int have[VP_OPEN_MAX_ORACLES]; for (int &h : have) h = 0;
    pl.plen.assign((size_t) n, 0); pl.dlen.assign((size_t) n, 0); pl.bytes = pl.layout = 0;
    for (auto &t : pl.tab) t = PcOpenDesc{};
    for (int i = 0; i < n; ++i) {
        const int o = oracle[i];
        if (o < 0) return VP_EINVAL;
        if (o >= VP_OPEN_MAX_ORACLES || !have[o]) { VPCHK(pc_open_desc(ctx, o, &pl.tab[std::min(o, VP_OPEN_MAX_ORACLES - 1)])); have[o] = 1; }
        const PcOpenDesc &d = pl.tab[o];
        if (leaf[i] >= d.n_leaves) return VP_EINVAL;
        const int depth = pc_open_depth(d.n_leaves);
        if (depth + 1 > VP_OPEN_MAX_PATH) return VP_ELIMIT;
        if (path_stride >= 0 && path_stride < 32 * (depth + 1)) return VP_EINVAL;
        pl.dlen[i] = depth + 1;
        pl.layout += 130 * sizeof(F) + 32ull * (depth + 1);
        if (d.top && !pcs_owns(ctx, leaf[i])) continue;
        pl.plen[i] = depth + 1;
        pl.bytes += 130 * sizeof(F) + 32ull * (depth + 1);
    }
    return VP_OK;
}
static int pc_many_run(vp_ctx *ctx, int n, const int32_t *oracle, const uint64_t *leaf, const PcManyPlan &pl, const std::function<void(int, const PcOpenRec &)> &sink) {
    std::vector<int> mine; mine.reserve((size_t) n);
    for (int i = 0; i < n; ++i) if (pl.plen[i]) mine.push_back(i);
    ctx->ev_used = 0;
    if (mine.empty()) { if (ctx->profiling) prof_collect(ctx); return VP_OK; }
    VPCHK(pc_many_reserve(ctx, (u32) std::min<size_t>(mine.size(), PC_MANY_PIECE)));
    const u32 cap = ctx->pc_many_cap;
    PcOpenDesc *h_tab = reinterpret_cast<PcOpenDesc *>(ctx->h_many);
    uint2 *h_req = reinterpret_cast<uint2 *>(ctx->h_many + VP_OPEN_MAX_ORACLES * sizeof(PcOpenDesc));
    const PcOpenRec *h_rec = reinterpret_cast<const PcOpenRec *>(ctx->h_many + pc_many_in_bytes(cap));
    const PcOpenDesc *d_tab = reinterpret_cast<const PcOpenDesc *>(ctx->pc_many_in);
    const uint2 *d_req = reinterpret_cast<const uint2 *>(ctx->pc_many_in + VP_OPEN_MAX_ORACLES * sizeof(PcOpenDesc));
    memcpy(h_tab, pl.tab, sizeof pl.tab);
    for (size_t at = 0; at < mine.size(); at += PC_MANY_PIECE) {
        const u32 cnt = (u32) std::min<size_t>(PC_MANY_PIECE, mine.size() - at);
        u64 bytes = 0;
        for (u32 j = 0; j < cnt; ++j) {
            const int i = mine[at + j];
            h_req[j] = make_uint2((u32) oracle[i], (u32) leaf[i]);
            bytes += 130 * sizeof(F) + 32ull * pl.plen[i];
        }
        HIPCHK(hipMemcpyAsync(ctx->pc_many_in, ctx->h_many, pc_many_in_bytes(cnt), hipMemcpyHostToDevice, ctx->stream));
        PC_PROF(VP_K_PC_OPEN_MANY, cnt, cnt, bytes, 0,
                hipLaunchKernelGGL(k_pc_open_many, dim3(cnt), dim3(128), 0, ctx->stream, d_tab, (u32) VP_OPEN_MAX_ORACLES, d_req, cnt, ctx->pc_many_buf));
        HIPCHK(hipMemcpyAsync(const_cast<PcOpenRec *>(h_rec), ctx->pc_many_buf, (size_t) cnt * sizeof(PcOpenRec), hipMemcpyDeviceToHost, ctx->stream));
        VPCHK(check_stream(ctx));
        for (u32 j = 0; j < cnt; ++j) sink(mine[at + j], h_rec[j]);
    }
    if (ctx->profiling) prof_collect(ctx);
    return VP_OK;
}


static int pc_mask_geometry(vp_ctx *ctx, uint64_t n_mask, u32 *ms_out) {
    const int n = ctx->L[0].bl, lm = n - 1;
    const u64 M = 1ull << lm;
    if (n_mask < 1 || n_mask > M) { ctx->err = "mask longer than a slice"; return VP_EINVAL; }
    u64 gap = 1;
    while (gap * 2 <= M / n_mask) gap *= 2;
    const u64 ms = M / gap;
    if (ms < 8) { ctx->err = "mask pads to fewer than 8 elements: the reference's transforms of that size read stale scratch (RS_polynomial.cpp:104-133), its commitment is not a function of such a mask"; return VP_EINVAL; }
    if (gap < 2) { ctx->err = "mask longer than half a slice (the reference asserts mask_position_gap != 1, poly_commit.h:195)"; return VP_EINVAL; }
    if (2 * ms > (1ull << PC_MAX_LN_SPLIT)) { ctx->err = "mask pads to more than 2^16 elements: its quotient's transform would be longer than 2^17 points (not supported)"; return VP_ELIMIT; }
    *ms_out = (u32) ms;
    return VP_OK;
}
static inline F *pc_mask_S0(vp_ctx *ctx) { return ctx->pc_mtmp + ctx->pc_mtmp_cap - 64; }
static int pc_mask_alloc(vp_ctx *ctx, u32 ms) {
    const int n = ctx->L[0].bl;
    const size_t M = (size_t) 1 << (n - 1), N = (size_t) 1 << (n - 6), B = std::max<size_t>(ms, N);
    if (!ctx->pc_lm_cw) { VPCHK(dalloc(ctx, &ctx->pc_lm_cw, M)); VPCHK(dalloc(ctx, &ctx->pc_qm_cw, M)); VPCHK(dalloc(ctx, &ctx->pc_hm_cw, M)); VPCHK(dalloc(ctx, &ctx->pc_fm, M)); }
    const size_t need = 6 * B + 32 * N + 64;
    if (ctx->pc_mtmp_cap < need) {
        F *fresh = nullptr;
        VPCHK(dalloc(ctx, &fresh, need));
        if (ctx->pc_mtmp) {
            HIPCHK(hipStreamSynchronize(ctx->stream));
            auto it = std::find(ctx->allocs.begin(), ctx->allocs.end(), (void *) ctx->pc_mtmp);
            if (it != ctx->allocs.end()) ctx->allocs.erase(it);
            (void) hipFree(ctx->pc_mtmp);
        }
        ctx->pc_mtmp = fresh; ctx->pc_mtmp_cap = need;
    }
    ctx->pc_mB = B;
    return VP_OK;
}
static int pc_mask_encode(vp_ctx *ctx, F *coef, u32 ms, F *dst) {
    const int n = ctx->L[0].bl, ln = n - 6, lm = n - 1;
    const u32 N = 1u << ln;
    if (ms <= N) {
        if (ms < N) hipLaunchKernelGGL(k_zero_f, dim3(nblk(N - ms)), dim3(VP_BLOCK), 0, ctx->stream, coef + ms, N - ms);
        return pc_launch_ntt(ctx, coef, dst, ln, lm, 0, 1, 32, N);
    }
    F *rows = ctx->pc_mtmp + 6 * ctx->pc_mB;
    hipLaunchKernelGGL(k_mask_combine, dim3(nblk((u64) 32 * N)), dim3(VP_BLOCK), 0, ctx->stream, (const F *) coef, N, ms / N, (const F *) ctx->pc_rt, 1u << (lm - 1), rows);
    return pc_launch_ntt(ctx, rows, dst, ln, lm, 0, 32, 1, N);
}
static int pc_mask_lde(vp_ctx *ctx, const vp_F *mask, uint64_t n_mask, u32 ms, F *dst) {
    const int lm = ctx->L[0].bl - 1;
    for (uint64_t i = 0; i < n_mask; ++i) if (mask[i].real >= P61 || mask[i].img >= P61) { ctx->err = "non-canonical mask element"; return VP_EINVAL; }
    std::vector<F> h(ms, f_zero());
    for (uint64_t i = 0; i < n_mask; ++i) h[i] = f_make(mask[i].real, mask[i].img);
    F *t = ctx->pc_mtmp;
    HIPCHK(hipMemcpyAsync(t, h.data(), (size_t) ms * sizeof(F), hipMemcpyHostToDevice, ctx->stream));
    HIPCHK(hipStreamSynchronize(ctx->stream));
    VPCHK(pc_launch_ntt(ctx, t, t + ctx->pc_mB, ilog2(ms), lm, 1, 1, 1, ms));
    return pc_mask_encode(ctx, t + ctx->pc_mB, ms, dst);
}
static inline void pc_launch_leaf_hash_masked(vp_ctx *ctx, const F *cw, u32 N, const F *mask, Dig *leaves) {
    const u32 n_leaves = N >= 2 ? 16 * N : 16u;
    hipLaunchKernelGGL(k_leaf_hash_cm, dim3(nblk(n_leaves)), dim3(VP_BLOCK), 0, ctx->stream, cw, N, 64, mask, leaves);
}

int pc_public_alloc(vp_ctx *ctx) {
    if (ctx->pc_pub) return VP_OK;
    const int n = ctx->L[0].bl, ln = n - 6, lm = n - 1;
    const u32 N = 1u << ln, M = 1u << lm;
    VPCHK(dalloc(ctx, &ctx->pc_pub, (size_t) 1 << n));
    VPCHK(dalloc(ctx, &ctx->pc_qcw, (size_t) 64 * M));
    VPCHK(dalloc(ctx, &ctx->pc_hcw, (size_t) 64 * M));
    VPCHK(dalloc(ctx, &ctx->pc_tmp, (size_t) 3 * 128 * N));
    VPCHK(dalloc(ctx, &ctx->pc_small, (size_t) 1024 + 160 + 64));
    VPCHK(dalloc(ctx, &ctx->pc_q0, (size_t) M));
    VPCHK(dalloc(ctx, &ctx->pc_flag, (size_t) 1));
    VPCHK(dalloc(ctx, &ctx->pc_eq, (size_t) 32 + 2 * ((size_t) 1 << ((n + 1) / 2))));
    VPCHK(dalloc(ctx, &ctx->pc_cbuf, (size_t) 64));
    VPCHK(dalloc(ctx, &ctx->pc_tree_h, (size_t) M));
    VPCHK(dalloc(ctx, &ctx->pc_fri_all, (size_t) 64 * M));
    VPCHK(dalloc(ctx, &ctx->pc_fri_tree, (size_t) M));
    VPCHK(dalloc(ctx, &ctx->pc_fri_roots, (size_t) VP_FRI_MAX));
    return VP_OK;
}

int pc_commit_public_body(vp_ctx *ctx, hipEvent_t &ev_a, const F corner[64], int tensor_state, vp_F *inner, vp_F all_sum[65], uint8_t root_h[32],
                          const vp_F *pub_mask = nullptr, uint64_t n_pub_mask = 0) {
    const int n = ctx->L[0].bl, ln = n - 6, lm = n - 1;
    const u32 N = 1u << ln, M = 1u << lm;
    F *P = ctx->pc_tmp, *ST = ctx->pc_tmp + (size_t) 128 * N, *H = ctx->pc_tmp + (size_t) 256 * N;
    F *parts = ctx->pc_small, *d_inner = ctx->pc_small + 1024, *d_all = ctx->pc_small + 1025;
    const u32 used = (u32) ctx->L[0].size, g = std::min<u32>(1024, nblk(used));
    PC_PROF(VP_K_PC_POINTWISE, g, 1, 32ull * used, used, hipLaunchKernelGGL(k_pc_dot, dim3(g), dim3(VP_BLOCK), 0, ctx->stream, ctx->L[0].val, ctx->pc_pub, used, parts));
    hipLaunchKernelGGL(k_pc_sum_parts, dim3(1), dim3(VP_BLOCK), 0, ctx->stream, parts, g, d_inner);
    F *qscal = ctx->pc_small + 1184;
    bool tensor = false;
    if (ctx->opt.pc_tensor_pub && (corner[0].re | corner[0].im) != 0 && corner[0].re < P61 && corner[0].im < P61) {
        if (tensor_state == 1) tensor = true;
        else {
            HIPCHK(hipMemsetAsync(ctx->pc_flag, 0, sizeof(int), ctx->stream));
            PC_PROF(VP_K_PC_POINTWISE, nblk((u64) 64 * N), 1, 16ull * 64 * N, (u64) 2 * 64 * N,
                    hipLaunchKernelGGL(k_pc_rank1_check, dim3(nblk((u64) 64 * N)), dim3(VP_BLOCK), 0, ctx->stream, (const F *) ctx->pc_pub, N, 64u, ctx->pc_flag));
            int bad = 1;
            HIPCHK(hipMemcpyAsync(&bad, ctx->pc_flag, sizeof(int), hipMemcpyDeviceToHost, ctx->stream));
            HIPCHK(hipStreamSynchronize(ctx->stream));
            tensor = bad == 0;
        }
    }
    ctx->pc_q_tensor = tensor;
    if (tensor) {
        F *sc = nullptr;
        VPCHK(ring_alloc(ctx, 64 * sizeof(F), (void **) &sc));
        const F inv0 = host_pow(corner[0], (unsigned __int128) P61 * P61 - 2);
        for (int i = 0; i < 64; ++i) sc[i] = f_mul(corner[i], inv0);
        HIPCHK(hipMemcpyAsync(qscal, sc, 64 * sizeof(F), hipMemcpyHostToDevice, ctx->stream));
        VPCHK(pc_launch_ntt(ctx, ctx->pc_pub, ctx->pc_coef, ln, lm, 1, 1, 1, N));
        VPCHK(pc_launch_ntt(ctx, ctx->pc_coef, ctx->pc_q0, ln, lm, 0, 1, 32, N));
    } else {
        VPCHK(pc_launch_ntt(ctx, ctx->pc_pub, ctx->pc_coef, ln, lm, 1, 64, 1, N));
        VPCHK(pc_launch_ntt(ctx, ctx->pc_coef, ctx->pc_qcw, ln, lm, 0, 64, 32, N));
    }
    const F *q0 = tensor ? ctx->pc_q0 : nullptr, *qs = tensor ? qscal : nullptr;
    PC_PROF(VP_K_PC_POINTWISE, nblk((u64) 128 * N), 1, 48ull * 128 * N, (u64) 128 * N,
            hipLaunchKernelGGL(k_pc_products, dim3(nblk((u64) 128 * N)), dim3(VP_BLOCK), 0, ctx->stream, ctx->pc_cw, ctx->pc_qcw, N, P, 64u, q0, qs));
    VPCHK(pc_launch_ntt(ctx, P, ST, ln, lm, 1, 128, 1, N));
    hipLaunchKernelGGL(k_zero_f, dim3(1), dim3(128), 0, ctx->stream, d_all, 65u);
    PC_PROF(VP_K_PC_POINTWISE, nblk((u64) 64 * N), 1, 48ull * 64 * N, (u64) 2 * 64 * N,
            hipLaunchKernelGGL(k_pc_quotient, dim3(nblk((u64) 64 * N)), dim3(VP_BLOCK), 0, ctx->stream, ST, N, ctx->pc_rt, M >> 1,
                               host_inv_real(2), f_make(N, 0), H, d_all, 64u));
    VPCHK(pc_launch_ntt(ctx, H, ctx->pc_hcw, ln, lm, 0, 64, 32, N));
    const u32 n_leaves = M >> 1;
    if (pub_mask) {
        const u32 ms = ctx->pc_mask_ms, gap = M / ms;
        const size_t B = ctx->pc_mB;
        F *t = ctx->pc_mtmp, *S0m = pc_mask_S0(ctx);
        VPCHK(pc_mask_lde(ctx, pub_mask, n_pub_mask, ms, ctx->pc_qm_cw));
        hipLaunchKernelGGL(k_mask_lq, dim3(nblk(2 * ms)), dim3(VP_BLOCK), 0, ctx->stream, (const F *) ctx->pc_lm_cw, (const F *) ctx->pc_qm_cw, N, gap >> 1, 2 * ms, t + 2 * B);
        VPCHK(pc_launch_ntt(ctx, t + 2 * B, t + 4 * B, ilog2(2 * ms), lm, 1, 1, 1, 2 * ms));
        hipLaunchKernelGGL(k_mask_hcoef, dim3(nblk((u64) B)), dim3(VP_BLOCK), 0, ctx->stream, (const F *) (t + 4 * B), ms, (u32) B, f_make(ms, 0), t, S0m, d_all + 64);
        VPCHK(pc_mask_encode(ctx, t, ms, ctx->pc_hm_cw));
        pc_launch_leaf_hash_masked(ctx, ctx->pc_hcw, N, ctx->pc_hm_cw, ctx->pc_tree_h + n_leaves);
    } else
    PC_PROF(VP_K_LEAF_HASH, nblk(n_leaves), 1, (u64) n_leaves * (64 * 32 + 32), (u64) n_leaves * 65,
            pc_launch_leaf_hash(ctx, ctx->pc_hcw, N, ctx->pc_tree_h + n_leaves));
    VPCHK(pc_merkle(ctx, ctx->pc_tree_h, n_leaves));
    unsigned char *st = nullptr;
    VPCHK(ring_alloc(ctx, 32 + 66 * sizeof(F), (void **) &st));
    HIPCHK(hipMemcpyAsync(st, ctx->pc_tree_h + 1, 32, hipMemcpyDeviceToHost, ctx->stream));
    HIPCHK(hipMemcpyAsync(st + 32, d_inner, 66 * sizeof(F), hipMemcpyDeviceToHost, ctx->stream));
    ctx->pc_public_done = true; ctx->fri_step = -1;
    return defer_end(ctx, ev_a, VP_PH_PUBLIC, [ctx, st, root_h, inner, all_sum](float ms) {
        memcpy(root_h, st, 32); memcpy(inner, st + 32, sizeof(F)); memcpy(all_sum, st + 32 + sizeof(F), 65 * sizeof(F));
        ctx->commit_ms = ms;
        return VP_OK;
    });
}

}

extern "C" {

static int pc_commit_private_body(vp_ctx *ctx, uint8_t root[32], const vp_F *mask, uint64_t n_mask) {
    const int n = ctx->L[0].bl;
    if (n < 7) { ctx->err = "input layer too small for the commitment (bit length < 7)"; return VP_EINVAL; }
    if (ctx->pcs) { if (mask) { ctx->err = "masked commitment: not on a sharded commitment"; return VP_EINVAL; } VPCHK(flush_pending(ctx, (size_t) -1)); return pcs_commit_private(ctx, root); }
    const int ln = n - 6, lm = n - 1;
    if (n > PC_MAX_N) { ctx->err = "input layer of more than 2^25 wires: the reference's commitment indexes its codeword with int (poly_commit.h:87-166), "
                                   "which overflows at 2^26 wires"; return VP_ELIMIT; }
    const u32 N = 1u << ln, M = 1u << lm;
    u32 ms = 0;
    if (mask) { VPCHK(pc_mask_geometry(ctx, n_mask, &ms)); VPCHK(flush_pending(ctx, (size_t) -1)); }
    VPCHK(pc_root_table(ctx, lm));
    if (mask) VPCHK(pc_mask_alloc(ctx, ms));
    if (!ctx->pc_coef) {
        VPCHK(dalloc(ctx, &ctx->pc_coef, (size_t) 64 * N));
        VPCHK(dalloc(ctx, &ctx->pc_cw, (size_t) 64 * M));
        VPCHK(dalloc(ctx, &ctx->pc_tree, (size_t) M));
    }
    ctx->ev_used = 0;
    hipEvent_t ev_a = nullptr;
    VPCHK(defer_begin(ctx, &ev_a));
    EvGuard ev_guard{ctx, &ev_a};
    if (ctx->opt.real_pairs && ctx->vreal == 1 && ctx->opt.ntt_r8 && ln >= 13 && ln <= 17) {
        VPCHK(pc_launch_ntt8(ctx, ctx->L[0].val, ctx->pc_coef, ln, lm, 1, 32, 1, N, 32));
        VPCHK(pc_launch_ntt8(ctx, ctx->pc_coef, ctx->pc_cw, ln, lm, 0, 32, 32, N, 32));
    } else {
        VPCHK(pc_launch_ntt(ctx, ctx->L[0].val, ctx->pc_coef, ln, lm, 1, 64, 1, N));
        VPCHK(pc_launch_ntt(ctx, ctx->pc_coef, ctx->pc_cw, ln, lm, 0, 64, 32, N));
    }
    const u32 n_leaves = M >> 1;
    ctx->pc_mask_ms = 0;
    if (mask) {
        VPCHK(pc_mask_lde(ctx, mask, n_mask, ms, ctx->pc_lm_cw));
        pc_launch_leaf_hash_masked(ctx, ctx->pc_cw, N, ctx->pc_lm_cw, ctx->pc_tree + n_leaves);
        ctx->pc_mask_ms = ms;
    } else
    PC_PROF(VP_K_LEAF_HASH, nblk(n_leaves), 1, (u64) n_leaves * (64 * 32 + 32), (u64) n_leaves * 65,
            pc_launch_leaf_hash(ctx, ctx->pc_cw, N, ctx->pc_tree + n_leaves));
    VPCHK(pc_merkle(ctx, ctx->pc_tree, n_leaves));
    void *st = nullptr;
    VPCHK(ring_alloc(ctx, 32, &st));
    HIPCHK(hipMemcpyAsync(st, ctx->pc_tree + 1, 32, hipMemcpyDeviceToHost, ctx->stream));
    ctx->pc_private_done = true; ++ctx->private_epoch;
    ctx->pc_public_done = false;
    return defer_end(ctx, ev_a, VP_PH_PRIVATE, [ctx, root, st](float ms) { memcpy(root, st, 32); ctx->commit_ms = ms; return VP_OK; });
}

int vp_commit_private(vp_ctx *ctx, uint8_t root[32]) {
    if (!ctx || !ctx->evaluated || !root) return VP_EINVAL;
    VP_ENTER_Q(ctx);
    return pc_commit_private_body(ctx, root, nullptr, 0);
}
int vp_commit_private_masked(vp_ctx *ctx, const vp_F *mask, uint64_t n_mask, uint8_t root[32]) {
    if (!ctx || !ctx->evaluated || !root || !mask) return VP_EINVAL;
    VP_ENTER(ctx);
    const int keep = ctx->deferred;
    ctx->deferred = 0;
    const int rc = pc_commit_private_body(ctx, root, mask, n_mask);
    ctx->deferred = keep;
    return rc;
}

static int pc_upload_pub(vp_ctx *ctx, const vp_F *pub, size_t bytes) {
    if (!ctx->h_pub || ctx->h_pub_cap < bytes || bytes < ((size_t) 8 << 20)) {
        HIPCHK(hipMemcpyAsync(ctx->pc_pub, pub, bytes, hipMemcpyHostToDevice, ctx->stream));
        return VP_OK;
    }
    const size_t piece = (size_t) 4 << 20, n_pieces = (bytes + piece - 1) / piece;
    const int n_thr = 4;
    std::vector<std::atomic<int>> ready(n_pieces);
    for (auto &r : ready) r.store(0, std::memory_order_relaxed);
    const unsigned char *src = reinterpret_cast<const unsigned char *>(pub);
    std::vector<std::thread> thr;
    for (int t = 0; t < n_thr; ++t)
        thr.emplace_back([&, t]() {
            for (size_t q = t; q < n_pieces; q += n_thr) {
                const size_t off = q * piece, len = std::min(piece, bytes - off);
                memcpy(ctx->h_pub + off, src + off, len);
                ready[q].store(1, std::memory_order_release);
            }
        });
    int rc = VP_OK;
    for (size_t q = 0; q < n_pieces && rc == VP_OK; ++q) {
        while (!ready[q].load(std::memory_order_acquire)) std::this_thread::yield();
        const size_t off = q * piece, len = std::min(piece, bytes - off);
        if (hipMemcpyAsync(reinterpret_cast<unsigned char *>(ctx->pc_pub) + off, ctx->h_pub + off, len, hipMemcpyHostToDevice, ctx->stream) != hipSuccess) { ctx->err = "hipMemcpyAsync (public vector)"; rc = VP_EHIP; }
    }
    for (auto &t : thr) t.join();
    return rc;
}

static int pc_fold0_consts(vp_ctx *ctx, int lm);
static int pc_warm(vp_ctx *ctx) {
    const int n = ctx->L[0].bl;
    if (n < 7 || ctx->pcs) return VP_OK;
    const int ln = n - 6, lm = n - 1;
    if (n > PC_MAX_N) return VP_OK;
    const u32 N = 1u << ln, M = 1u << lm;
    VPCHK(pc_root_table(ctx, lm));
    if (!ctx->pc_coef) {
        VPCHK(dalloc(ctx, &ctx->pc_coef, (size_t) 64 * N));
        VPCHK(dalloc(ctx, &ctx->pc_cw, (size_t) 64 * M));
        VPCHK(dalloc(ctx, &ctx->pc_tree, (size_t) M));
    }
    VPCHK(pc_public_alloc(ctx));
    struct Dry { vp_ctx *c; ~Dry() { c->pc_dry = false; } } dry{ctx};
    ctx->pc_dry = true;
    if (ctx->opt.real_pairs && ctx->vreal == 1 && ctx->opt.ntt_r8 && ln >= 13 && ln <= 17) {
        VPCHK(pc_launch_ntt8(ctx, ctx->L[0].val, ctx->pc_coef, ln, lm, 1, 32, 1, N, 32));
        VPCHK(pc_launch_ntt8(ctx, ctx->pc_coef, ctx->pc_cw, ln, lm, 0, 32, 32, N, 32));
    }
    VPCHK(pc_launch_ntt(ctx, ctx->L[0].val, ctx->pc_coef, ln, lm, 1, 64, 1, N));
    VPCHK(pc_launch_ntt(ctx, ctx->pc_coef, ctx->pc_cw, ln, lm, 0, 64, 32, N));
    VPCHK(pc_launch_ntt(ctx, ctx->pc_pub, ctx->pc_coef, ln, lm, 1, 1, 1, N));
    VPCHK(pc_launch_ntt(ctx, ctx->pc_coef, ctx->pc_q0, ln, lm, 0, 1, 32, N));
    VPCHK(pc_launch_ntt(ctx, ctx->pc_tmp, ctx->pc_tmp + (size_t) 128 * N, ln, lm, 1, 128, 1, N));
    ctx->pc_dry = false;
    VPCHK(pc_fold0_consts(ctx, lm));
// ... 5 lines not shown
        else { ctx->h_pub = nullptr; (void) hipGetLastError(); }
    }
    return VP_OK;
}
static int pc_commit_public_host(vp_ctx *ctx, const vp_F *pub, uint64_t n_pub, vp_F *inner, vp_F all_sum[65], uint8_t root_h[32], const vp_F *pub_mask, uint64_t n_pub_mask) {
    if (ctx->pcs) { if (pub_mask) { ctx->err = "masked commitment: not on a sharded commitment"; return VP_EINVAL; } return pcs_commit_public(ctx, pub, n_pub, nullptr, inner, all_sum, root_h); }
    if (!ctx->pc_private_done) return VP_EINVAL;
    const int n = ctx->L[0].bl;
    if (n_pub != (1ull << n)) return VP_EINVAL;
    const u32 N = 1u << (n - 6);
    VPCHK(pc_public_alloc(ctx));
    VPCHK(pc_upload_pub(ctx, pub, sizeof(F) << n));
    ctx->ev_used = 0;
    hipEvent_t ev_a = nullptr;
    VPCHK(defer_begin(ctx, &ev_a));
    EvGuard ev_guard{ctx, &ev_a};
    F corner[64];
    for (int i = 0; i < 64; ++i) corner[i] = f_make(pub[(size_t) i * N].real, pub[(size_t) i * N].img);
    const int keep_deferred = ctx->deferred;
    ctx->deferred = 0;
    const int rc = pc_commit_public_body(ctx, ev_a, corner, 0, inner, all_sum, root_h, pub_mask, n_pub_mask);
    ctx->deferred = keep_deferred;
    return rc;
}

int vp_commit_public(vp_ctx *ctx, const vp_F *pub, uint64_t n_pub, vp_F *inner, vp_F all_sum[65], uint8_t root_h[32]) {
    if (!ctx || !ctx->evaluated || !pub || !inner || !all_sum || !root_h) return VP_EINVAL;
    VP_ENTER(ctx);
    if (ctx->pc_mask_ms) { ctx->err = "vp_commit_public: the private commitment carries a mask (vp_commit_public_masked)"; return VP_EINVAL; }
    return pc_commit_public_host(ctx, pub, n_pub, inner, all_sum, root_h, nullptr, 0);
}
int vp_commit_public_masked(vp_ctx *ctx, const vp_F *pub, uint64_t n_pub, const vp_F *pub_mask, uint64_t n_pub_mask, vp_F *inner, vp_F all_sum[65], uint8_t root_h[32]) {
    if (!ctx || !ctx->evaluated || !pub || !pub_mask || !inner || !all_sum || !root_h) return VP_EINVAL;
    VP_ENTER(ctx);
    if (!ctx->pc_mask_ms) { ctx->err = "vp_commit_public_masked: vp_commit_private_masked first"; return VP_EINVAL; }
    if (n_pub_mask < 1 || n_pub_mask > ctx->pc_mask_ms) { ctx->err = "public mask longer than the private commitment's padded mask"; return VP_EINVAL; }
    return pc_commit_public_host(ctx, pub, n_pub, inner, all_sum, root_h, pub_mask, n_pub_mask);
}

int vp_commit_public_eq(vp_ctx *ctx, const vp_F *point, int n_point, vp_F *inner, vp_F all_sum[65], uint8_t root_h[32]) {
    if (!ctx || !ctx->evaluated || !point || !inner || !all_sum || !root_h) return VP_EINVAL;
    VP_ENTER_Q(ctx);
    if (ctx->pc_mask_ms) { ctx->err = "vp_commit_public_eq: the private commitment carries a mask (vp_commit_public_masked)"; return VP_EINVAL; }
    if (!(ctx->pcs ? pcs_private_done(ctx) : ctx->pc_private_done)) return VP_EINVAL;
    const int n = ctx->L[0].bl;
    if (n_point != n) return VP_EINVAL;
    for (int i = 0; i < n; ++i) if (point[i].real >= P61 || point[i].img >= P61) { ctx->err = "vp_commit_public_eq: non-canonical coordinate"; return VP_EINVAL; }
    if (ctx->pcs) { VPCHK(flush_pending(ctx, (size_t) -1)); return pcs_commit_public(ctx, nullptr, 0, point, inner, all_sum, root_h); }
    const u32 N = 1u << (n - 6);
    VPCHK(pc_public_alloc(ctx));
    F *dr = ctx->pc_eq, *dbf = ctx->pc_eq + 32, *dbs = dbf + ((size_t) 1 << ((n + 1) / 2));
    F *hr = nullptr;
    VPCHK(ring_alloc(ctx, 32 * sizeof(F), (void **) &hr));
    for (int i = 0; i < n; ++i) hr[i] = f_make(point[i].real, point[i].img);
    hr[n] = f_one();
    ctx->ev_used = 0;
    hipEvent_t ev_a = nullptr;
    VPCHK(defer_begin(ctx, &ev_a));
    EvGuard ev_guard{ctx, &ev_a};
    HIPCHK(hipMemcpyAsync(dr, hr, (n + 1) * sizeof(F), hipMemcpyHostToDevice, ctx->stream));
    hipLaunchKernelGGL(k_beta_half, dim3(1), dim3(VP_BLOCK), 0, ctx->stream, (const F *) dr, n, (const F *) (dr + n), dbf, dbs);
    PC_PROF(VP_K_PC_POINTWISE, grid_for(1ull << n), 1, 16ull << n, 1ull << n,
            hipLaunchKernelGGL(k_beta_expand, dim3(grid_for(1ull << n)), dim3(VP_BLOCK), 0, ctx->stream, (const F *) dbf, (const F *) dbs, n >> 1,
                               (u32) (1u << n), ctx->pc_pub));
    F corner[64];
    {
        F low = f_one();
        for (int k = 0; k < n - 6; ++k) low = f_mul(low, f_sub(f_one(), hr[k]));
        for (int i = 0; i < 64; ++i) {
            F v = low;
            for (int k = 0; k < 6; ++k) v = f_mul(v, ((i >> k) & 1) ? hr[n - 6 + k] : f_sub(f_one(), hr[n - 6 + k]));
            corner[i] = v;
        }
    }
    (void) N;
    return pc_commit_public_body(ctx, ev_a, corner, 1, inner, all_sum, root_h);
}

int vp_fri_step(vp_ctx *ctx, const vp_F *r, uint8_t root[32]) {
    if (!ctx || !r || !root) return VP_EINVAL;
    if (ctx->pcs) { VP_ENTER(ctx); return pcs_fri_step(ctx, r, root); }
    if (!ctx->pc_public_done) return VP_EINVAL;
    VP_ENTER(ctx);
    const int n = ctx->L[0].bl, ln = n - 6, lm = n - 1;
    const u32 N = 1u << ln, M = 1u << lm;
    if (!ctx->pc_fri_all) {
        VPCHK(dalloc(ctx, &ctx->pc_fri_all, (size_t) 64 * M));
        VPCHK(dalloc(ctx, &ctx->pc_fri_tree, (size_t) M));
    }
    HIPCHK(hipEventRecord(ctx->ev0, ctx->stream));
    if (ctx->fri_step < 0) {
        hipLaunchKernelGGL(k_pc_virtual_oracle, dim3(nblk((u64) 64 * M)), dim3(VP_BLOCK), 0, ctx->stream, ctx->pc_cw, ctx->pc_qcw,
                           ctx->pc_hcw, ctx->pc_small + 1025 + 80, N, ctx->pc_rt, M >> 1, f_make(N, 0), 64u,
                           (const F *) (ctx->pc_q_tensor ? ctx->pc_q0 : nullptr), (const F *) (ctx->pc_q_tensor ? ctx->pc_small + 1184 : nullptr));
        ctx->fri_step = 0; ctx->fri_tree_used = 0;
        ctx->fri_cw_off.clear(); ctx->fri_tree_off.clear(); ctx->fri_m_off.clear();
        if (ctx->pc_mask_ms)
            hipLaunchKernelGGL(k_mask_vo, dim3(nblk(M)), dim3(VP_BLOCK), 0, ctx->stream, (const F *) ctx->pc_lm_cw, (const F *) ctx->pc_qm_cw, (const F *) ctx->pc_hm_cw,
                               (const F *) pc_mask_S0(ctx), N, ctx->pc_rt, M >> 1, f_make(ctx->pc_mask_ms, 0), ctx->pc_mask_ms, ctx->pc_qm_cw);
    }
    const int k = ctx->fri_step;
    if (k >= ln) { ctx->err = "FRI commit phase already finished"; return VP_EINVAL; }
    const u32 Nk = N >> k, No = Nk >> 1;
    size_t cw_off = 0;
    for (int q = 0; q < k; ++q) cw_off += (size_t) 64 * 32 * (N >> (q + 1));
    const F *in = k == 0 ? ctx->pc_qcw : ctx->pc_fri_all + ctx->fri_cw_off[k - 1];
    F *out = ctx->pc_fri_all + cw_off;
    ctx->fri_cw_off.push_back(cw_off);
    ctx->fri_tree_off.push_back(ctx->fri_tree_used);
    F rf; memcpy(&rf, r, sizeof(F));
    hipLaunchKernelGGL(k_fri_fold, dim3(nblk((u64) (64 / VP_FOLD_SPT) * 32 * No)), dim3(VP_BLOCK), 0, ctx->stream, in, out, Nk, k, ctx->pc_rt, M >> 1, rf,
                       host_inv_real(2), 0, 0u);
    const u32 n_leaves = 16 * No;
    Dig *tree = ctx->pc_fri_tree + ctx->fri_tree_used;
    if (ctx->pc_mask_ms) {
        size_t m_off = 0;
        for (int q = 0; q < k; ++q) m_off += (size_t) 32 * (N >> (q + 1));
        const F *in_m = k == 0 ? ctx->pc_qm_cw : ctx->pc_fm + ctx->fri_m_off[k - 1];
        F *out_m = ctx->pc_fm + m_off;
        ctx->fri_m_off.push_back(m_off);
        hipLaunchKernelGGL(k_fri_fold_one, dim3(nblk((u64) 32 * No)), dim3(VP_BLOCK), 0, ctx->stream, in_m, out_m, Nk, k, ctx->pc_rt, M >> 1, rf, host_inv_real(2));
        pc_launch_leaf_hash_masked(ctx, out, No, out_m, tree + n_leaves);
    } else
    if (No >= 2) pc_launch_leaf_hash(ctx, out, No, tree + n_leaves);
    else hipLaunchKernelGGL(k_leaf_hash_final, dim3(1), dim3(64), 0, ctx->stream, out, 64, tree + n_leaves);
    VPCHK(pc_merkle(ctx, tree, n_leaves));
    HIPCHK(hipEventRecord(ctx->ev1, ctx->stream));
    HIPCHK(hipMemcpyAsync(root, tree + 1, 32, hipMemcpyDeviceToHost, ctx->stream));
    VPCHK(check_stream(ctx));
    ctx->fri_tree_used += 2 * (size_t) n_leaves;
    ctx->fri_step = k + 1;
    float ms = 0;
    hipEventElapsedTime(&ms, ctx->ev0, ctx->ev1);
    ctx->commit_ms = ms;
    return VP_OK;
}

static int pc_fold0_consts(vp_ctx *ctx, int lm) {
    if (ctx->pc_cbuf_lm == lm) return VP_OK;
    F *cb = nullptr;
    VPCHK(ring_alloc(ctx, 64 * sizeof(F), (void **) &cb));
    const F wM = host_root_of_unity(lm), wMi = host_pow(wM, (unsigned __int128) P61 * P61 - 2), w32 = host_root_of_unity(5);
    F pb = f_one(), pn = f_one();
    for (int b = 0; b < 32; ++b) { cb[b] = pb; cb[32 + b] = f_sub(pn, f_one()); pb = f_mul(pb, wMi); pn = f_mul(pn, w32); }
    HIPCHK(hipMemcpyAsync(ctx->pc_cbuf, cb, 64 * sizeof(F), hipMemcpyHostToDevice, ctx->stream));
    ctx->pc_cbuf_lm = lm;
    return VP_OK;
}

int vp_fri_commit(vp_ctx *ctx, const vp_F *r, int n_steps, uint8_t *roots) {
    if (!ctx || !r || !roots || n_steps < 1) return VP_EINVAL;
    VP_ENTER_Q(ctx);
    if (ctx->pcs) { VPCHK(flush_pending(ctx, (size_t) -1)); return pcs_fri_commit(ctx, r, n_steps, roots); }
    if (!ctx->pc_public_done) return VP_EINVAL;
    const int n = ctx->L[0].bl, ln = n - 6, lm = n - 1;
    const u32 N = 1u << ln, M = 1u << lm;
    if (ctx->fri_step >= 0 && ctx->fri_step != 0) { ctx->err = "vp_fri_commit after vp_fri_step"; return VP_EINVAL; }
    if (n_steps > ln || n_steps > VP_FRI_MAX) { ctx->err = "too many FRI steps"; return VP_EINVAL; }
    if (ctx->pc_mask_ms) {
        VPCHK(flush_pending(ctx, (size_t) -1));
        double ms_sum = 0;
        for (int k = 0; k < n_steps; ++k) { VPCHK(vp_fri_step(ctx, r + k, roots + 32 * (size_t) k)); ms_sum += ctx->commit_ms; }
        ctx->commit_ms = ms_sum;
        return VP_OK;
    }
    if (!ctx->pc_fri_all) {
        VPCHK(dalloc(ctx, &ctx->pc_fri_all, (size_t) 64 * M));
        VPCHK(dalloc(ctx, &ctx->pc_fri_tree, (size_t) M));
    }
    Dig *d_roots = nullptr;
    if (!ctx->pc_fri_roots) VPCHK(dalloc(ctx, &ctx->pc_fri_roots, (size_t) VP_FRI_MAX));
    d_roots = ctx->pc_fri_roots;
    ctx->ev_used = 0;
    hipEvent_t ev_a = nullptr;
    VPCHK(defer_begin(ctx, &ev_a));
    EvGuard ev_guard{ctx, &ev_a};
    ctx->fri_step = 0; ctx->fri_tree_used = 0;
    ctx->fri_cw_off.clear(); ctx->fri_tree_off.clear();
    FriLeafArgs la{}; MerkleArgs ma{};
    u32 blocks = 0; size_t cw_off = 0;
    const bool fold3 = n_steps >= 3 && ln >= 9;
    for (int k = 0; k < n_steps; ++k) {
        const u32 Nk = N >> k, No = Nk >> 1;
        const F *in = k == 0 ? ctx->pc_qcw : ctx->pc_fri_all + ctx->fri_cw_off[k - 1];
        F *out = ctx->pc_fri_all + cw_off;
        ctx->fri_cw_off.push_back(cw_off);
        ctx->fri_tree_off.push_back(ctx->fri_tree_used);
        F rf; memcpy(&rf, r + k, sizeof(F));
        if (fold3 && k < 3) {
            if (k == 0) {
                const F *rtn = nullptr;
                VPCHK(pc_circle_roots(ctx, lm, ln, &rtn));
                VPCHK(pc_fold0_consts(ctx, lm));
                F r1, r2; memcpy(&r1, r + 1, sizeof(F)); memcpy(&r2, r + 2, sizeof(F));
                F *o1 = out, *o2 = o1 + (size_t) 64 * 32 * No, *o3 = o2 + (size_t) 64 * 32 * (No >> 1);
                const u32 E = N >> 3;
                const bool grouped = (64 / VP_VO_SPT / VP_VO_GRP) * 32 * (E >> 6) >= 2048;
                const u32 grid3 = (64 / VP_VO_SPT / (grouped ? VP_VO_GRP : 1)) * 32 * (E >> 6);
                const void *fold3 = ctx->pc_q_tensor ? (grouped ? (const void *) k_fri_fold0_vo3<true, VP_VO_GRP> : (const void *) k_fri_fold0_vo3<true, 1>)
                                                     : (grouped ? (const void *) k_fri_fold0_vo3<false, VP_VO_GRP> : (const void *) k_fri_fold0_vo3<false, 1>);
                const F *a_lcw = ctx->pc_cw, *a_qcw = ctx->pc_qcw, *a_hcw = ctx->pc_hcw, *a_S0 = ctx->pc_small + 1025 + 80, *a_cb = ctx->pc_cbuf;
                const F *a_q0 = ctx->pc_q_tensor ? ctx->pc_q0 : nullptr, *a_qs = ctx->pc_q_tensor ? ctx->pc_small + 1184 : nullptr;
                u32 a_N = N;
                F a_half = f_mul(f_make(N, 0), host_inv_real(2)), a_inv2 = host_inv_real(2);
                void *args3[] = {&a_lcw, &a_qcw, &a_hcw, &a_S0, &o1, &o2, &o3, &a_N, &rtn, &a_cb, &rf, &r1, &r2, &a_half, &a_inv2, &a_q0, &a_qs};
                PC_PROF(VP_K_FRI_FOLD, grid3, 1, (ctx->pc_q_tensor ? 80ull : 112ull) * 64 * 32 * No + 16ull * 64 * 32 * ((No >> 1) + (No >> 2)),
                        (u64) (ctx->pc_q_tensor ? 9 : 7) * 64 * 32 * No + 3ull * 64 * 32 * ((No >> 1) + (No >> 2)),
                        (void) hipLaunchKernel(fold3, dim3(grid3), dim3(256), args3, 0, ctx->stream));
            }
        }
        else if (k == 0)
        {
            const F *rtn = nullptr;
            VPCHK(pc_circle_roots(ctx, lm, ln, &rtn));
            VPCHK(pc_fold0_consts(ctx, lm));
            PC_PROF(VP_K_FRI_FOLD, nblk((u64) (64 / VP_VO_SPT) * 32 * No), 1, (ctx->pc_q_tensor ? 80ull : 112ull) * 64 * 32 * No, (u64) (ctx->pc_q_tensor ? 9 : 7) * 64 * 32 * No,
                    hipLaunchKernelGGL(k_fri_fold0_vo, dim3(nblk((u64) (64 / VP_VO_SPT) * 32 * No)), dim3(VP_BLOCK), 0, ctx->stream, (const F *) ctx->pc_cw, (const F *) ctx->pc_qcw,
                                       (const F *) ctx->pc_hcw, (const F *) (ctx->pc_small + 1025 + 80), out, N, rtn, (const F *) ctx->pc_cbuf, rf,
                                       f_mul(f_make(N, 0), host_inv_real(2)),
                                       (const F *) (ctx->pc_q_tensor ? ctx->pc_q0 : nullptr), (const F *) (ctx->pc_q_tensor ? ctx->pc_small + 1184 : nullptr)));
        }
        else
        PC_PROF(VP_K_FRI_FOLD, nblk((u64) 64 * 32 * No), 1, 48ull * 64 * 32 * No, (u64) 3 * 64 * 32 * No,
                hipLaunchKernelGGL(k_fri_fold, dim3(nblk((u64) (64 / VP_FOLD_SPT) * 32 * No)), dim3(VP_BLOCK), 0, ctx->stream, in, out, Nk, k, ctx->pc_rt, M >> 1, rf,
                                   host_inv_real(2), 0, 0u));
        const u32 n_leaves = 16 * No;
        Dig *tree = ctx->pc_fri_tree + ctx->fri_tree_used;
        ma.tree[k] = tree; ma.count[k] = n_leaves;
        {
            la.cw[la.n] = out; la.leaves[la.n] = tree + n_leaves; la.N[la.n] = No; blocks += nblk(n_leaves); ++la.n;
        }
        cw_off += (size_t) 64 * 32 * No;
        ctx->fri_tree_used += 2 * (size_t) n_leaves;
    }
    u64 all_leaves = 0;
    for (int k = 0; k < n_steps; ++k) all_leaves += ma.count[k];
    if (la.n) PC_PROF(VP_K_LEAF_HASH, blocks, la.n, all_leaves * (64 * 32 + 32), all_leaves * 65, pc_launch_leaf_hash_multi(ctx, la));
    for (;;) {
        MerkleArgs lv{}; u32 b = 0;
        for (int k = 0; k < n_steps; ++k) {
            const u32 c = ma.count[k] >> 1;
            if (c <= 512) continue;
            lv.tree[lv.n] = ma.tree[k]; lv.count[lv.n] = c; lv.blk_start[lv.n] = b; b += nblk(c); ++lv.n;
            ma.count[k] = c;
        }
        if (!lv.n) break;
        lv.blk_start[lv.n] = b;
        u64 hs = 0;
        for (int q = 0; q < lv.n; ++q) hs += lv.count[q];
        PC_PROF(VP_K_MERKLE, b, lv.n, 96ull * hs, hs, hipLaunchKernelGGL(k_merkle_level_multi, dim3(b), dim3(VP_BLOCK), 0, ctx->stream, lv));
    }
    ma.n = n_steps;
    {
        u64 hs = 0;
        for (int k = 0; k < n_steps; ++k) hs += ma.count[k] ? ma.count[k] - 1 : 0;
        PC_PROF(VP_K_MERKLE, n_steps, n_steps, 96ull * hs, hs, hipLaunchKernelGGL(k_merkle_top_multi, dim3(n_steps), dim3(VP_BLOCK), 0, ctx->stream, ma, d_roots));
    }
    void *st = nullptr;
    VPCHK(ring_alloc(ctx, (size_t) 32 * n_steps, &st));
    HIPCHK(hipMemcpyAsync(st, d_roots, (size_t) 32 * n_steps, hipMemcpyDeviceToHost, ctx->stream));
    ctx->fri_step = n_steps;
    return defer_end(ctx, ev_a, VP_PH_FRI, [ctx, st, roots, n_steps](float ms) { memcpy(roots, st, (size_t) 32 * n_steps); ctx->commit_ms = ms; return VP_OK; });
}

int vp_fri_final(vp_ctx *ctx, vp_F *final_code) {
    if (!ctx || !final_code) return VP_EINVAL;
    VP_ENTER_Q(ctx);
    if (ctx->pcs) { VPCHK(flush_pending(ctx, (size_t) -1)); return pcs_fri_final(ctx, final_code); }
    if (!ctx->pc_public_done) return VP_EINVAL;
    const int ln = ctx->L[0].bl - 6;
    if (ctx->fri_step != ln) { ctx->err = "FRI commit phase not finished"; return VP_EINVAL; }
    hipEvent_t ev_a = nullptr;
    VPCHK(defer_begin(ctx, &ev_a));
    EvGuard ev_guard{ctx, &ev_a};
    F *cw = nullptr;
    VPCHK(ring_alloc(ctx, 64 * 32 * sizeof(F), (void **) &cw));
    HIPCHK(hipMemcpyAsync(cw, ctx->pc_fri_all + ctx->fri_cw_off[ln - 1], 64 * 32 * sizeof(F), hipMemcpyDeviceToHost, ctx->stream));
    return defer_end(ctx, ev_a, VP_PH_FRI_FINAL, [cw, final_code](float) {
        F *o = reinterpret_cast<F *>(final_code);
        for (u32 i = 0; i < 16; ++i) for (u32 s = 0; s < 64; ++s) for (u32 hi = 0; hi < 2; ++hi) o[(i << 7) | (s << 1) | hi] = cw[s * 32 + i + 16 * hi];
        return VP_OK;
    });
}

int vp_fri_final_mask(vp_ctx *ctx, vp_F out[32]) {
    if (!ctx || !out) return VP_EINVAL;
    VP_ENTER(ctx);
    if (ctx->pcs) { ctx->err = "vp_fri_final_mask: not on a sharded commitment"; return VP_EINVAL; }
    if (!ctx->pc_public_done) return VP_EINVAL;
    const int ln = ctx->L[0].bl - 6;
    if (ctx->fri_step != ln) { ctx->err = "FRI commit phase not finished"; return VP_EINVAL; }
    memset(out, 0, 32 * sizeof(vp_F));
    if (!ctx->pc_mask_ms) return VP_OK;
    F v[32];
    HIPCHK(hipMemcpyAsync(v, ctx->pc_fm + ctx->fri_m_off[ln - 1], sizeof v, hipMemcpyDeviceToHost, ctx->stream));
    VPCHK(check_stream(ctx));
    for (u32 i = 0; i < 16; ++i) for (u32 hi = 0; hi < 2; ++hi) { out[2 * i + hi].real = v[i + 16 * hi].re; out[2 * i + hi].img = v[i + 16 * hi].im; }
    return VP_OK;
}

int vp_fri_open(vp_ctx *ctx, int oracle, uint64_t leaf, vp_F values[130], uint8_t *path, int path_capacity, int *path_len) {
    if (!ctx || !values || !path || !path_len || oracle < 0) return VP_EINVAL;
    VP_ENTER(ctx);
    if (ctx->pcs) return pcs_fri_open(ctx, oracle, leaf, values, path, path_capacity, path_len);
    const int n = ctx->L[0].bl, ln = n - 6, lm = n - 1;
    const u32 N = 1u << ln, M = 1u << lm;
    const F *cw; const Dig *tree; u32 Nc, n_leaves;
    if (oracle == 0) { if (!ctx->pc_private_done) return VP_EINVAL; cw = ctx->pc_cw; tree = ctx->pc_tree; Nc = N; n_leaves = M >> 1; }
    else if (oracle == 1) { if (!ctx->pc_public_done) return VP_EINVAL; cw = ctx->pc_hcw; tree = ctx->pc_tree_h; Nc = N; n_leaves = M >> 1; }
    else {
        const int lvl = oracle - 2;
        if (lvl >= ctx->fri_step || lvl >= (int) ctx->fri_cw_off.size()) { ctx->err = "FRI level not committed yet"; return VP_EINVAL; }
        cw = ctx->pc_fri_all + ctx->fri_cw_off[lvl]; tree = ctx->pc_fri_tree + ctx->fri_tree_off[lvl];
        Nc = N >> (lvl + 1); n_leaves = 16 * Nc;
    }
    if (leaf >= n_leaves) return VP_EINVAL;
    int depth = 0; while ((1u << depth) < n_leaves) ++depth;
    if (path_capacity < 32 * (depth + 1)) return VP_EINVAL;
    if (!ctx->pc_open_buf) VPCHK(dalloc(ctx, &ctx->pc_open_buf, (size_t) 130 + 2 * 40));
    Dig *dpath = reinterpret_cast<Dig *>(ctx->pc_open_buf + 130);
    const F *mask_cw = nullptr;
    if (ctx->pc_mask_ms) mask_cw = oracle == 0 ? ctx->pc_lm_cw : oracle == 1 ? ctx->pc_hm_cw : (oracle - 2 < (int) ctx->fri_m_off.size() ? ctx->pc_fm + ctx->fri_m_off[oracle - 2] : nullptr);
    hipLaunchKernelGGL(k_pc_open, dim3(1), dim3(128), 0, ctx->stream, cw, Nc, tree, n_leaves, (u32) leaf, ctx->pc_open_buf, dpath, mask_cw);
    HIPCHK(hipMemcpyAsync(values, ctx->pc_open_buf, 130 * sizeof(F), hipMemcpyDeviceToHost, ctx->stream));
    HIPCHK(hipMemcpyAsync(path, dpath, 32 * (size_t) (depth + 1), hipMemcpyDeviceToHost, ctx->stream));
    VPCHK(check_stream(ctx));
    *path_len = depth + 1;
    return VP_OK;
}

int vp_fri_open_many(vp_ctx *ctx, int n, const int32_t *oracle, const uint64_t *leaf, vp_F *values, uint8_t *paths, int path_stride, int32_t *path_len) {
    if (!ctx || n < 0) return VP_EINVAL;
    if (n == 0) return VP_OK;
    if (!oracle || !leaf || !values || !paths || !path_len || path_stride < 0) return VP_EINVAL;
    if (n > PC_MANY_MAX) { ctx->err = "vp_fri_open_many: more than 2^16 requests"; return VP_ELIMIT; }
    VP_ENTER(ctx);
    PcManyPlan pl;
    VPCHK(pc_many_plan(ctx, n, oracle, leaf, path_stride, pl));
    VPCHK(pc_many_run(ctx, n, oracle, leaf, pl, [&](int i, const PcOpenRec &r) {
        memcpy(values + (size_t) 130 * i, r.v, 130 * sizeof(F));
        memcpy(paths + (size_t) path_stride * i, r.path, 32 * (size_t) pl.plen[i]);
    }));
    for (int i = 0; i < n; ++i) path_len[i] = pl.plen[i];
    return VP_OK;
}

static int pc_query_requests(vp_ctx *ctx, int n_queries, const uint64_t *leaf0, std::vector<int32_t> &oracle, std::vector<uint64_t> &leaf) {
    if (ctx->pcs && pcs_fri_one_pass(ctx)) { ctx->err = "vp_fri_query: not after vp_fri_commit on a sharded commitment (merge vp_fri_open_many over the ranks)"; return VP_EINVAL; }
    if (ctx->L.empty() || !(ctx->pcs ? pcs_public_done(ctx) : ctx->pc_public_done)) return VP_EINVAL;
    const int ln = ctx->L[0].bl - 6;
    if ((ctx->pcs ? pcs_fri_done(ctx) : ctx->fri_step) != ln) { ctx->err = "FRI commit phase not finished"; return VP_EINVAL; }
    if ((u64) n_queries * (u64) (2 + ln) > (u64) PC_MANY_MAX) { ctx->err = "vp_fri_query: more than 2^16 openings"; return VP_ELIMIT; }
    const u64 M = 1ull << (ctx->L[0].bl - 1);
    oracle.clear(); leaf.clear();
    for (int q = 0; q < n_queries; ++q) {
        const u64 l0 = leaf0 ? leaf0[q] : 0;
        oracle.push_back(0); leaf.push_back(l0);
        oracle.push_back(1); leaf.push_back(l0);
        u64 D = M, t = l0;
        for (int k = 0; k < ln; ++k) { const u64 Dn = D / 2, lf = t % (Dn / 2); oracle.push_back(2 + k); leaf.push_back(lf); t = lf; D = Dn; }
    }
    return VP_OK;
}
int vp_fri_query_bytes(vp_ctx *ctx, int n_queries, uint64_t *bytes) {
    if (!ctx || !bytes || n_queries < 0) return VP_EINVAL;
    VP_ENTER(ctx);
    std::vector<int32_t> oracle; std::vector<uint64_t> leaf;
    VPCHK(pc_query_requests(ctx, n_queries, nullptr, oracle, leaf));
    PcManyPlan pl;
    VPCHK(pc_many_plan(ctx, (int) oracle.size(), oracle.data(), leaf.data(), -1, pl));
    *bytes = pl.layout;
    return VP_OK;
}
int vp_fri_query(vp_ctx *ctx, int n_queries, const uint64_t *leaf0, uint8_t *out, uint64_t capacity, uint64_t *n_written) {
    if (!ctx || n_queries < 0 || !n_written || (n_queries > 0 && (!leaf0 || !out))) return VP_EINVAL;
    VP_ENTER(ctx);
    std::vector<int32_t> oracle; std::vector<uint64_t> leaf;
    VPCHK(pc_query_requests(ctx, n_queries, leaf0, oracle, leaf));
    const int n = (int) oracle.size();
    PcManyPlan pl;
    VPCHK(pc_many_plan(ctx, n, oracle.data(), leaf.data(), -1, pl));
    if (pl.layout > capacity) { ctx->err = "vp_fri_query: output buffer too small (vp_fri_query_bytes)"; return VP_EINVAL; }
    std::vector<u64> at((size_t) n + 1, 0);
    for (int i = 0; i < n; ++i) at[i + 1] = at[i] + 130 * sizeof(F) + 32ull * pl.dlen[i];
    VPCHK(pc_many_run(ctx, n, oracle.data(), leaf.data(), pl, [&](int i, const PcOpenRec &r) {
        memcpy(out + at[i], r.v, 130 * sizeof(F));
        memcpy(out + at[i] + 130 * sizeof(F), r.path, 32 * (size_t) pl.plen[i]);
// ... 85 lines not shown
```

virgo-plus_amd/csrc/vpgpu_pc_shard.inc:

```
#include <dlfcn.h>

struct PcShard {
    int rank = 0, world = 1, lw = 0, S = 64;
    int op = 0, stage = 0;
    F *coef = nullptr, *lcw = nullptr, *qcw = nullptr, *hcw = nullptr, *tmp = nullptr, *small = nullptr, *pub = nullptr;
    F *l_loc = nullptr, *h_loc = nullptr, *fri_loc = nullptr; std::vector<size_t> fri_off;
    Dig *tree_l = nullptr, *tree_h = nullptr, *tree_f = nullptr;
    Dig *top_l = nullptr, *top_h = nullptr, *top_f = nullptr; std::vector<size_t> top_f_off;
    F *tail = nullptr; Dig *tail_tree = nullptr; std::vector<size_t> tail_cw_off, tail_tree_off;
    std::vector<size_t> tree_f_off;
    F *send = nullptr; size_t send_cap = 0;
    unsigned char *ag_send = nullptr, *ag_recv = nullptr; size_t ag_cap = 0;
    Dig *d_roots = nullptr;
    int n_local = 0, n_steps = 0;
    int f_done = 0, f_mode = 0;
    F step_r;
    float acc_ms = 0;
    F *eq = nullptr; F pt[32];
    std::vector<F> fri_r;
    bool private_done = false, public_done = false;
    F *pub0 = nullptr, *q0cw = nullptr, *qscal = nullptr; int *flag = nullptr; bool q_tensor = false;
    struct X { int kind; const void *send; void *recv; size_t bytes; } x[2];
    int nx = 0;
};
// ... 560 lines not shown
        vals[2 * t] = row[al]; vals[2 * t + 1] = row[al + (Nl >> 1)];
    } else if (t == 64) { vals[128] = f_zero(); vals[129] = f_zero(); }
    u32 depth = 5;
    while ((1u << (depth - 5)) < n5) ++depth;
    if (t <= depth) {
        if (t == depth) path[t] = tree_loc[nl + leaf_loc];
        else if (t < 5) path[t] = tree_loc[((nl + leaf_loc) >> t) ^ 1];
        else path[t] = top[((n5 + a) >> (t - 5)) ^ 1];
    }
}

int pcs_fri_open(vp_ctx *ctx, int oracle, uint64_t leaf, vp_F values[130], uint8_t *path, int path_capacity, int *path_len) {
    PcShard &s = *ctx->pcs;
    const int n = ctx->L[0].bl, ln = n - 6;
    const u32 N = 1u << ln, Nl = N >> s.lw;
    if (!ctx->pc_open_buf) VPCHK(dalloc(ctx, &ctx->pc_open_buf, (size_t) 130 + 2 * 40));
    Dig *dpath = reinterpret_cast<Dig *>(ctx->pc_open_buf + 130);
    u32 n_leaves;
    if (oracle >= 2 && oracle - 2 >= s.n_local - 1) {
        const int q = oracle - 2 - (s.n_local - 1);
        if (oracle - 2 >= s.f_done || q >= (int) s.tail_tree_off.size()) { ctx->err = "FRI level not committed yet"; return VP_EINVAL; }
        const u32 Nt = (1u << s.lw) >> q;
        n_leaves = Nt >= 2 ? 16 * Nt : 16;
        if (leaf >= n_leaves) return VP_EINVAL;
        hipLaunchKernelGGL(k_pc_open, dim3(1), dim3(128), 0, ctx->stream, s.tail + s.tail_cw_off[q], Nt, s.tail_tree + s.tail_tree_off[q], n_leaves, (u32) leaf,
                           ctx->pc_open_buf, dpath, (const F *) nullptr);
    } else {
        const F *cw; const Dig *tl, *top; u32 Nc;
        if (oracle == 0) { if (!s.private_done) return VP_EINVAL; cw = s.l_loc; tl = s.tree_l; top = s.top_l; Nc = Nl; }
        else if (oracle == 1) { if (!s.public_done) return VP_EINVAL; cw = s.h_loc; tl = s.tree_h; top = s.top_h; Nc = Nl; }
        else {
            const int lvl = oracle - 2;
            if (lvl >= s.f_done || lvl + 1 >= (int) s.fri_off.size() || lvl >= (int) s.tree_f_off.size()) { ctx->err = "FRI level not committed yet"; return VP_EINVAL; }
            cw = s.fri_loc + s.fri_off[lvl + 1]; tl = s.tree_f + s.tree_f_off[lvl]; top = s.top_f + s.top_f_off[lvl]; Nc = Nl >> (lvl + 1);
        }
        n_leaves = (16 * Nc) << s.lw;
        if (leaf >= n_leaves) return VP_EINVAL;
        if ((int) ((leaf >> 5) & (u64) (s.world - 1)) != s.rank) { ctx->err = "this rank does not own the leaf (owner = (leaf >> 5) mod world)"; return VP_EINVAL; }
        hipLaunchKernelGGL(k_pc_open_sh, dim3(1), dim3(128), 0, ctx->stream, cw, Nc, tl, top, (Nc >> 1) << s.lw, (u32) leaf, s.lw, ctx->pc_open_buf, dpath);
    }
    int depth = 0; while ((1u << depth) < n_leaves) ++depth;
    if (path_capacity < 32 * (depth + 1)) return VP_EINVAL;
    HIPCHK(hipMemcpyAsync(values, ctx->pc_open_buf, 130 * sizeof(F), hipMemcpyDeviceToHost, ctx->stream));
    HIPCHK(hipMemcpyAsync(path, dpath, 32 * (size_t) (depth + 1), hipMemcpyDeviceToHost, ctx->stream));
    VPCHK(check_stream(ctx));
    *path_len = depth + 1;
    return VP_OK;
}

int pcs_open_desc(vp_ctx *ctx, int oracle, PcOpenDesc *d) {
    PcShard &s = *ctx->pcs;
    const int n = ctx->L[0].bl, ln = n - 6;
    const u32 N = 1u << ln, Nl = N >> s.lw;
    if (oracle >= 2 && oracle - 2 >= s.n_local - 1) {
        const int q = oracle - 2 - (s.n_local - 1);
        if (oracle - 2 >= s.f_done || q >= (int) s.tail_tree_off.size()) { ctx->err = "FRI level not committed yet"; return VP_EINVAL; }
        const u32 Nt = (1u << s.lw) >> q;
        d->cw = s.tail + s.tail_cw_off[q]; d->tree = s.tail_tree + s.tail_tree_off[q]; d->Nc = Nt; d->n_leaves = Nt >= 2 ? 16 * Nt : 16;
        return VP_OK;
    }
    if (oracle == 0) { if (!s.private_done) return VP_EINVAL; d->cw = s.l_loc; d->tree = s.tree_l; d->top = s.top_l; d->Nc = Nl; }
    else if (oracle == 1) { if (!s.public_done) return VP_EINVAL; d->cw = s.h_loc; d->tree = s.tree_h; d->top = s.top_h; d->Nc = Nl; }
    else {
        const int lvl = oracle - 2;
        if (lvl >= s.f_done || lvl + 1 >= (int) s.fri_off.size() || lvl >= (int) s.tree_f_off.size()) { ctx->err = "FRI level not committed yet"; return VP_EINVAL; }
        d->cw = s.fri_loc + s.fri_off[lvl + 1]; d->tree = s.tree_f + s.tree_f_off[lvl]; d->top = s.top_f + s.top_f_off[lvl]; d->Nc = Nl >> (lvl + 1);
    }
    d->n_leaves = (16 * d->Nc) << s.lw; d->n5 = (d->Nc >> 1) << s.lw; d->lw = (u32) s.lw;
    return VP_OK;
}
bool pcs_private_done(vp_ctx *ctx) { return ctx->pcs->private_done; }
bool pcs_public_done(vp_ctx *ctx) { return ctx->pcs->public_done; }
int pcs_fri_done(vp_ctx *ctx) { return ctx->pcs->f_done; }
bool pcs_fri_one_pass(vp_ctx *ctx) { return ctx->pcs->f_mode == 1; }
bool pcs_owns(vp_ctx *ctx, uint64_t leaf) { const PcShard &s = *ctx->pcs; return (int) ((leaf >> 5) & (u64) (s.world - 1)) == s.rank; }

}

extern "C" {

int vp_pc_load_input(vp_ctx *ctx, const vp_F *inputs, uint64_t n_inputs, int bit_length) {
    if (!ctx || !inputs || bit_length < 7 || bit_length > 30 || n_inputs == 0 || n_inputs > (1ull << bit_length)) return VP_EINVAL;
    VP_ENTER(ctx);
    HIPCHK(hipStreamSynchronize(ctx->stream));
    if (ctx->gkr_graph) { (void) hipGraphExecDestroy(ctx->gkr_graph); ctx->gkr_graph = nullptr; }
    free_plan(ctx);
    free_all(ctx);
    vp_free_shard_state(ctx);
    ctx->L.assign(1, LayerDev());
    ctx->n_layers = 1;
    ctx->L[0].size = n_inputs; ctx->L[0].bl = bit_length;
    ctx->vreal = 0; ctx->plan_vreal = 0;
    VPCHK(dalloc(ctx, &ctx->L[0].val, (size_t) 1 << bit_length));
    HIPCHK(hipMemsetAsync(ctx->L[0].val, 0, sizeof(F) << bit_length, ctx->stream));
    HIPCHK(hipMemcpyAsync(ctx->L[0].val, inputs, n_inputs * sizeof(F), hipMemcpyHostToDevice, ctx->stream));
    VPCHK(check_stream(ctx));
    ctx->pc_rt = ctx->pc_coef = ctx->pc_cw = nullptr; ctx->pc_tree = nullptr; ctx->pc_lm = -1; ctx->pc_rtc.clear();
    ctx->pc_pub = ctx->pc_qcw = ctx->pc_hcw = ctx->pc_tmp = ctx->pc_small = nullptr; ctx->pc_tree_h = nullptr; ctx->pc_private_done = false;
    ctx->pc_q0 = nullptr; ctx->pc_eq = nullptr; ctx->pc_cbuf = nullptr; ctx->pc_cbuf_lm = -1; ctx->pc_flag = nullptr; ctx->pc_q_tensor = false;
    ctx->pc_scr = nullptr; ctx->pc_scr_cap = 0; ctx->pc_fri_all = nullptr; ctx->pc_open_buf = nullptr; ctx->pc_many_buf = nullptr; ctx->pc_many_in = nullptr; ctx->pc_many_cap = 0; ctx->fri_cw_off.clear(); ctx->fri_tree_off.clear();
    ctx->pc_fri[0] = ctx->pc_fri[1] = nullptr; ctx->pc_fri_tree = nullptr; ctx->pc_fri_roots = nullptr; ctx->fri_step = -1; ctx->pc_public_done = false;
    ctx->pc_mask_ms = 0; ctx->pc_lm_cw = ctx->pc_qm_cw = ctx->pc_hm_cw = ctx->pc_fm = ctx->pc_mtmp = nullptr; ctx->fri_m_off.clear(); ctx->pc_mtmp_cap = 0; ctx->pc_mB = 0;
    ctx->evaluated = true;
    if (ctx->ev_pool.empty()) {
        ctx->ev_pool.resize(1024);
        for (auto &e : ctx->ev_pool) { hipEventCreate(&e.a); hipEventCreate(&e.b); e.bytes = 0; e.kind = -1; e.grid = e.jobs = e.rounds = e.first_round = 0; e.work = 0; }
    }
    return VP_OK;
}

int vp_pc_set_shard(vp_ctx *ctx, int rank, int world) {
    if (!ctx || world < 1 || rank < 0 || rank >= world || (world & (world - 1)) || world > 64) return VP_EINVAL;
    if (!ctx->evaluated || ctx->L.empty()) { ctx->err = "vp_pc_set_shard: no input layer yet"; return VP_EINVAL; }
    const int ln = ctx->L[0].bl - 6;
    int lw = 0; while ((1 << lw) < world) ++lw;
    if (world > 1 && ln - lw < 1) { ctx->err = "vp_pc_set_shard: slice too short for this many ranks"; return VP_ELIMIT; }
    if (world > 1 && ln > PC_MAX_LN_LONG) { ctx->err = "vp_pc_set_shard: input layer of more than 2^25 wires"; return VP_ELIMIT; }
    VP_ENTER(ctx);
    HIPCHK(hipStreamSynchronize(ctx->stream));
    vp_free_shard_state(ctx);
    if (world == 1 && !(ctx->cm && ctx->cm->comm && ctx->cm->world == 1)) return VP_OK;
    ctx->pcs = new PcShard();
    ctx->pcs->rank = rank; ctx->pcs->world = world; ctx->pcs->lw = lw; ctx->pcs->S = 64 / world;
    ctx->pcs->n_local = ln - lw;
    return VP_OK;
}

static bool pending_x(vp_ctx *ctx, int i, int *kind, const void **send, void **recv, size_t *bytes, int *world) {
    if (ctx->pcs && ctx->pcs->nx) {
        if (i < 0 || i >= ctx->pcs->nx) return false;
        const PcShard::X &x = ctx->pcs->x[i];
        *kind = x.kind; *send = x.send; *recv = x.recv; *bytes = x.bytes; *world = ctx->pcs->world;
        return true;
    }
    if (ctx->rsh && ctx->rsh->nx) {
        if (i != 0) return false;
        const RoundShard::X &x = ctx->rsh->x;
        *kind = x.kind; *send = x.send; *recv = x.recv; *bytes = x.bytes; *world = ctx->rsh->world;
        return true;
    }
    return false;
}
static int rs_exchange_local(vp_ctx **ctxs, int world) {
    vp_ctx *ctx = ctxs[0];
    const int nx = ctx->rsh->nx;
    const size_t bytes = ctx->rsh->x.bytes;
    for (int r = 0; r < world; ++r)
        if (ctxs[r]->rsh->nx != nx || (nx && ctxs[r]->rsh->x.bytes != bytes)) { ctx->err = "vp_shard_exchange_local: ranks are at different gathers"; return VP_EINVAL; }
    if (!nx) return VP_OK;
    for (int dst = 0; dst < world; ++dst) {
        vp_ctx *d = ctxs[dst];
        HIPCHK(hipSetDevice(d->device));
        for (int src = 0; src < world; ++src)
            HIPCHK(hipMemcpyAsync((char *) d->rsh->x.recv + (size_t) src * bytes, ctxs[src]->rsh->x.send, bytes, hipMemcpyDeviceToDevice, d->stream));
    }
    for (int dst = 0; dst < world; ++dst) {
        HIPCHK(hipSetDevice(ctxs[dst]->device));
        HIPCHK(hipStreamSynchronize(ctxs[dst]->stream));
    }
    for (int r = 0; r < world; ++r) ctxs[r]->rsh->nx = 0;
    return VP_OK;
}

int vp_shard_exchange_local(vp_ctx **ctxs, int world) {
    if (!ctxs || world < 1) return VP_EINVAL;
    {
        bool rs = true;
        for (int r = 0; r < world; ++r)
            if (!ctxs[r] || !ctxs[r]->rsh || ctxs[r]->rsh->world != world || ctxs[r]->rsh->rank != r || (ctxs[r]->pcs && ctxs[r]->pcs->nx)) rs = false;
        if (rs && ctxs[0]->rsh->nx) return rs_exchange_local(ctxs, world);
    }
    for (int r = 0; r < world; ++r) if (!ctxs[r] || !ctxs[r]->pcs || ctxs[r]->pcs->world != world || ctxs[r]->pcs->rank != r) return VP_EINVAL;
    const int nx = ctxs[0]->pcs->nx;
    for (int r = 0; r < world; ++r) if (ctxs[r]->pcs->nx != nx) { ctxs[0]->err = "vp_shard_exchange_local: ranks are at different collectives"; return VP_EINVAL; }
    vp_ctx *ctx = ctxs[0];
    for (int i = 0; i < nx; ++i) {
        const size_t bytes = ctxs[0]->pcs->x[i].bytes;
        const int kind = ctxs[0]->pcs->x[i].kind;
        for (int r = 0; r < world; ++r) if (ctxs[r]->pcs->x[i].bytes != bytes || ctxs[r]->pcs->x[i].kind != kind) { ctx->err = "vp_shard_exchange_local: mismatched collective"; return VP_EINVAL; }
        for (int src = 0; src < world; ++src)
            for (int dst = 0; dst < world; ++dst) {
                const PcShard::X &xs = ctxs[src]->pcs->x[i], &xd = ctxs[dst]->pcs->x[i];
                const char *from = (const char *) xs.send + (kind == 1 ? (size_t) dst * bytes : 0);
                HIPCHK(hipMemcpy((char *) xd.recv + (size_t) src * bytes, from, bytes, hipMemcpyDeviceToDevice));
            }
    }
    for (int r = 0; r < world; ++r) ctxs[r]->pcs->nx = 0;
    HIPCHK(hipDeviceSynchronize());
    return VP_OK;
}

int vp_shard_pending(vp_ctx *ctx, int *n) {
    if (!ctx || !n) return VP_EINVAL;
    VP_LOCK(ctx);
    *n = ctx->pcs ? ctx->pcs->nx : 0;
    if (!*n && ctx->rsh) *n = ctx->rsh->nx;
    return VP_OK;
}
int vp_shard_exchange_info(vp_ctx *ctx, int i, int *kind, uint64_t *bytes) {
    if (!ctx || !kind || !bytes) return VP_EINVAL;
    VP_LOCK(ctx);
// ... 97 lines not shown
```

virgo-plus_amd/host/vphost.cpp:

```cpp
#include "vphost.h"

#include <chrono>
#include <cstdlib>
#include <cstring>
#include <memory>
#include <string>

#include "circuit.hpp"
#include "prover.hpp"
#include "verifier.hpp"

struct vph_circuit { layeredCircuit c; };
struct vph_session {
    vph_circuit *circ;
    std::unique_ptr<prover> p;
    std::vector<F> tape;
    std::vector<uint8_t> fri_roots; std::vector<F> fri_final, fri_r;
    std::vector<uint8_t> full_record;
    std::vector<F> fft_gkr_msgs; double pc_times[3] = {0, 0, 0};
    double t_init = 0, t_round = 0, t_fin = 0;
    std::vector<F> last_point;
    std::vector<F> ptape_fft, ptape_fri;
    std::vector<uint8_t> pp_gkr, pp_roots; std::vector<F> pp_all, pp_final; F pp_inner; uint64_t pp_written = 0;
    uint8_t pp_root_l[32], pp_root_h[32], pp_root_next[32];
// ... 427 lines not shown
    if (rc != VP_OK) { set_err(err, errlen, std::string("vp_fri_final: ") + vp_last_error(ctx)); return rc; }
    return 0;
}

int vph_fri_commit_batched(vph_session *s, const uint64_t *r_pairs, int n_steps, uint8_t *roots, uint64_t *final_pairs, char *err, int errlen) {
    if (s->p->commitmentSharded()) return fri_commit_sharded(s, r_pairs, n_steps, roots, final_pairs, true, err, errlen);
    vp_ctx *ctx = s->p->context();
    int rc = vp_fri_commit(ctx, reinterpret_cast<const vp_F *>(r_pairs), n_steps, roots);
    if (rc != VP_OK) { set_err(err, errlen, std::string("vp_fri_commit: ") + vp_last_error(ctx)); return rc; }
    rc = vp_fri_final(ctx, reinterpret_cast<vp_F *>(final_pairs));
    if (rc != VP_OK) { set_err(err, errlen, std::string("vp_fri_final: ") + vp_last_error(ctx)); return rc; }
    return 0;
}

int vph_prove_full(vph_session *s, uint8_t *transcript, uint64_t capacity, uint64_t *n_written, int batched, char *err, int errlen) {
    try {
        F::init();
        std::vector<uint8_t> out;
        prover::hhash_digest rl = s->p->commit_private();
        out.insert(out.end(), rl.b, rl.b + 32);
        verifier v(batched ? nullptr : s->p.get(), s->circ->c);
        bool ok;
        if (batched) {
            std::vector<F> tape = v.drawTape();
            std::vector<uint8_t> tr;
            s->p->proveGKR(tape, tr);
            v.pred_dev = s->p.get();
            ok = v.check(tape, tr);
        } else {
            ok = v.verify();
        }
        out.insert(out.end(), v.transcript().begin(), v.transcript().end());
        s->last_point.assign(v.finalPoint().begin(), v.finalPoint().begin() + s->circ->c.circuit[0].bitLength);
        std::vector<F> pub;
        initBetaTable(pub, s->circ->c.circuit[0].bitLength, v.finalPoint().begin(), F_ONE);
        pub.resize(1ull << s->circ->c.circuit[0].bitLength);
        F inner; std::vector<F> all_sum;
        prover::hhash_digest rh = s->p->commit_public(pub, inner, all_sum);
        out.insert(out.end(), rh.b, rh.b + 32);
        const uint8_t *ib = reinterpret_cast<const uint8_t *>(&inner);
        out.insert(out.end(), ib, ib + 16);
        const uint8_t *ab = reinterpret_cast<const uint8_t *>(all_sum.data());
        out.insert(out.end(), ab, ab + 65 * 16);
        if (out.size() > capacity) { set_err(err, errlen, "transcript buffer too small"); return -1; }
        memcpy(transcript, out.data(), out.size());
        if (n_written) *n_written = out.size();
        return ok ? 0 : 1;
    } catch (const std::exception &e) {
        set_err(err, errlen, e.what());
        return -2;
    }
}

int vph_draw_protocol_tape(vph_session *s) {
    const int n = s->circ->c.circuit[0].bitLength;
    if (n < 7) return -1;
    F::init();
    verifier v(nullptr, s->circ->c);
    s->tape = v.drawTape();
    const int ln = n - 6;
    s->ptape_fft.resize((size_t) verifier::fftGkrDraws(ln));
    for (auto &x : s->ptape_fft) x = F::random();
    s->ptape_fri.resize(ln);
    for (auto &x : s->ptape_fri) x = F::random();
    return 0;
}
int vph_prove_protocol_ex(vph_session *s, uint8_t *transcript, uint64_t capacity, uint64_t *n_written, uint8_t *fri_roots, uint64_t roots_cap,
                          uint64_t *final_pairs, double sec[6], int flags, char *err, int errlen) {
    if (s->p->commitmentSharded()) { set_err(err, errlen, "vph_prove_protocol: not on a session with a sharded commitment (vph_prove_and_verify_full runs it)"); return -1; }
    vp_ctx *ctx = s->p->context();
    const bool defer = (flags & VPH_PASS_DEFERRED) != 0, queue_next = defer && (flags & VPH_PASS_QUEUE_NEXT) != 0;
    struct FftGuard { prover *p; bool armed; ~FftGuard() { if (armed) p->fftGkrCancel(); } } fft_guard{s->p.get(), false};
    auto chk = [&](int rc, const char *what) { if (rc != VP_OK) throw std::runtime_error(std::string(what) + ": " + vp_last_error(ctx)); };
    try {
        const layeredCircuit &C = s->circ->c;
        const int n = C.circuit[0].bitLength, ln = n - 6;
        if (s->tape.empty() || (int) s->ptape_fri.size() != ln) { set_err(err, errlen, "vph_draw_protocol_tape first"); return -1; }
        int max_bl = 0;
        for (auto &l : C.circuit) max_bl = std::max(max_bl, l.bitLength);
        using clk = std::chrono::high_resolution_clock;
        auto since = [](clk::time_point t) { return std::chrono::duration<double>(clk::now() - t).count(); };
        const auto t0 = clk::now();
        static const bool fft_sync = getenv("VPH_FFT_GKR_SYNC") != nullptr;
        u64 nt = 0, nb = 0;
        s->p->gkrSizes(nt, nb);
        if (s->tape.size() != nt) throw std::runtime_error("the tape has the wrong length");
        s->pp_gkr.resize(nb); s->pp_all.resize(65); s->pp_roots.resize((size_t) 32 * ln); s->pp_final.resize(2048);
        chk(vp_set_deferred(ctx, defer ? 1 : 0), "vp_set_deferred");
        uint64_t epoch = 0; int valid = 0;
        chk(vp_commit_private_state(ctx, &epoch, &valid), "vp_commit_private_state");
        const bool have_head = s->head_queued && valid && epoch == s->head_epoch;
        s->head_queued = false;
        auto t = clk::now();
        double s_fft = 0, s_priv = 0, s_gkr = 0, s_pub = 0, s_fri = 0;
        if (!have_head) {
            chk(vp_commit_private(ctx, s->pp_root_l), "vp_commit_private");
            s_priv = since(t);
        }
        t = clk::now();
        chk(vp_prove_gkr(ctx, reinterpret_cast<const vp_F *>(s->tape.data()), nt, s->pp_gkr.data(), nb, &s->pp_written), "vp_prove_gkr");
        s_gkr = since(t);
        t = clk::now();
        if (!fft_sync) { s->p->fftGkrBegin(ln, s->ptape_fft); fft_guard.armed = true; }
        s_fft = since(t);
        s->last_point.assign(s->tape.end() - max_bl, s->tape.end() - max_bl + n);
        t = clk::now();
        chk(vp_commit_public_eq(ctx, reinterpret_cast<const vp_F *>(s->last_point.data()), n, reinterpret_cast<vp_F *>(&s->pp_inner),
                                reinterpret_cast<vp_F *>(s->pp_all.data()), s->pp_root_h), "vp_commit_public_eq");
        s_pub = since(t);
        if (fft_sync) { t = clk::now(); s->fft_gkr_msgs = s->p->fftGkr(ln, s->ptape_fft); s_fft = since(t); }
        t = clk::now();
        chk(vp_fri_commit(ctx, reinterpret_cast<const vp_F *>(s->ptape_fri.data()), ln, s->pp_roots.data()), "vp_fri_commit");
        chk(vp_fri_final(ctx, reinterpret_cast<vp_F *>(s->pp_final.data())), "vp_fri_final");
        s_fri = since(t);
        int n_mine = 0;
        chk(vp_pending(ctx, &n_mine), "vp_pending");
        if (queue_next) {
            chk(vp_commit_private(ctx, s->pp_root_next), "vp_commit_private (next pass)");
            uint64_t e2 = 0; int v2 = 0;
            chk(vp_commit_private_state(ctx, &e2, &v2), "vp_commit_private_state");
            s->head_queued = true; s->head_epoch = e2;
        }
        if (defer) {
            chk(vp_flush(ctx, n_mine), "vp_flush");
            double ms[5] = {0, 0, 0, 0, 0};
            chk(vp_phase_ms(ctx, ms), "vp_phase_ms");
            s_priv = ms[0] * 1e-3; s_gkr = ms[1] * 1e-3; s_pub = ms[2] * 1e-3; s_fri = (ms[3] + ms[4]) * 1e-3;
        }
        chk(vp_set_deferred(ctx, 0), "vp_set_deferred");
        if (!fft_sync) { t = clk::now(); fft_guard.armed = false; s->fft_gkr_msgs = s->p->fftGkrEnd(ln); s_fft += since(t); }
        const uint64_t total = 32 + s->pp_written + 32 + 16 + 65 * 16;
        if (total > capacity || (fri_roots && roots_cap < s->pp_roots.size())) { set_err(err, errlen, "output buffer too small"); return -1; }
        uint8_t *o = transcript;
        memcpy(o, have_head ? s->pp_root_next : s->pp_root_l, 32); o += 32;
        memcpy(o, s->pp_gkr.data(), s->pp_written); o += s->pp_written;
        memcpy(o, s->pp_root_h, 32); o += 32;
        memcpy(o, &s->pp_inner, 16); o += 16;
        memcpy(o, s->pp_all.data(), 65 * 16);
        if (n_written) *n_written = total;
        s->fri_roots = s->pp_roots;
        s->fri_final = s->pp_final;
        s->fri_r = s->ptape_fri;
        if (fri_roots) memcpy(fri_roots, s->fri_roots.data(), s->fri_roots.size());
        if (final_pairs) memcpy(final_pairs, s->fri_final.data(), s->fri_final.size() * sizeof(F));
        s->p->addProveTime(s_gkr);
        if (sec) { sec[0] = since(t0); sec[1] = s_priv; sec[2] = s_gkr; sec[3] = s_pub; sec[4] = s_fft; sec[5] = s_fri; }
        return 0;
    } catch (const std::exception &e) {
        (void) vp_flush(ctx, -1);
        (void) vp_set_deferred(ctx, 0);
        s->head_queued = false;
        set_err(err, errlen, e.what());
        return -2;
    }
}
int vph_prove_protocol(vph_session *s, uint8_t *transcript, uint64_t capacity, uint64_t *n_written, uint8_t *fri_roots, uint64_t roots_cap,
                       uint64_t *final_pairs, double sec[6], char *err, int errlen) {
    return vph_prove_protocol_ex(s, transcript, capacity, n_written, fri_roots, roots_cap, final_pairs, sec, 0, err, errlen);
}

int vph_verify_transcript(vph_circuit *c, const uint8_t *transcript, uint64_t n, int skip_predicates) {
    try {
        F::init();
        verifier v(nullptr, c->c);
        const std::vector<F> tape = v.drawTape();
        v.skip_predicates = skip_predicates != 0;
        std::vector<uint8_t> tr(transcript, transcript + n);
        return v.check(tape, tr) ? 0 : 1;
    } catch (const std::exception &) { return 1; }
}

uint64_t vph_transcript_bytes(vph_session *s) {
    u64 a = 0, b = 0;
    s->p->gkrSizes(a, b);
    return b;
}

}
```

virgo-plus_amd/host/vphost.h:

```cpp
#ifndef VPHOST_H
#define VPHOST_H
#include <stdint.h>
#include "../../include/vpgpu.h"
#ifdef __cplusplus
extern "C" {
#endif

typedef struct vph_circuit vph_circuit;
typedef struct vph_session vph_session;

typedef struct {
    double prove_sec;
    double gkr_device_ms;
    double evaluate_ms;
    double verify_sec;
    double fold_ms;
    uint64_t fold_launches;
    uint64_t fold_bytes;
    uint64_t rounds;
    uint64_t launches;
    double proof_kb;
    int verified;
} vph_result;

vph_circuit *vph_circuit_from_pws(const char *path, int blocks, long seed, char *err, int errlen);
vph_circuit *vph_circuit_randomize(int layers, int log_size, long seed);
vph_circuit *vph_circuit_custom(int n_layers, const uint64_t *layer_sizes, const int32_t *ty, const int32_t *l, const uint64_t *u,
                                const uint64_t *v, const uint64_t *c_pairs, const uint8_t *is_assert);
void vph_circuit_free(vph_circuit *);
int vph_circuit_layers(const vph_circuit *);
uint64_t vph_circuit_gates(const vph_circuit *);
uint64_t vph_circuit_layer_size(const vph_circuit *, int layer);
int vph_circuit_layer_bitlen(const vph_circuit *, int layer);
void vph_circuit_hash(const vph_circuit *, uint64_t out[2]);

vph_session *vph_session_create(vph_circuit *, int device, char *err, int errlen);
vph_session *vph_session_create_opts(vph_circuit *, int device, const vp_options *opt , char *err, int errlen);
void vph_session_free(vph_session *);
int vph_set_profiling(vph_session *, int level);
void *vph_session_ctx(vph_session *);
vph_session *vph_session_create_round_sharded(vph_circuit *, const int *devices, int world, int min_log, const vp_options *opt, char *err, int errlen);
vph_session *vph_session_create_sharded(vph_circuit *, const int *devices, int world, int min_log, int shard_commitment, const vp_options *opt,
                                        char *err, int errlen);
void *vph_session_rank_ctx(vph_session *, int rank);
int vph_session_world(vph_session *);
int vph_session_partials(vph_session *, vp_F *out, int capacity);
void vph_session_clear_partials(vph_session *);
void vph_session_drop_rank(vph_session *, int rank);
double vph_session_gather_sec(vph_session *);
int vph_layer_values(vph_session *, int layer, uint64_t *out_pairs, uint64_t n);

int vph_prove_interactive(vph_session *, uint8_t *transcript, uint64_t capacity, uint64_t *n_written,
                          vph_result *res, char *err, int errlen);
int vph_draw_tape(vph_session *);
int vph_prove_gkr(vph_session *, uint8_t *transcript, uint64_t capacity, uint64_t *n_written, vph_result *res,
                  char *err, int errlen);
int vph_check(vph_session *, const uint8_t *transcript, uint64_t n, int skip_predicates, double *verify_sec);
uint64_t vph_transcript_bytes(vph_session *);
int vph_commit_private(vph_session *, uint8_t root[32], double *ms, char *err, int errlen);
int vph_commit_public(vph_session *, const uint64_t *pub_pairs, uint64_t n_pub, uint8_t out[32 + 16 + 65 * 16], double *ms,
                      char *err, int errlen);
int vph_prove_and_verify_full(vph_session *, int reps, uint8_t *transcript, uint64_t capacity, uint64_t *n_written,
                              double *gkr_prove_sec, double *pc_prove_sec, double *verify_sec, char *err, int errlen);
enum { VPH_VERIFY_BATCHED_OPENINGS = 1 };
int vph_prove_and_verify_full_ex(vph_session *, int reps, int flags, uint8_t *transcript, uint64_t capacity, uint64_t *n_written,
                                 double *gkr_prove_sec, double *pc_prove_sec, double *verify_sec, char *err, int errlen);
int vph_last_full_record(vph_session *, uint8_t *buf, uint64_t cap, uint64_t *n);
int vph_verify_full_record(vph_circuit *, const uint8_t *record, uint64_t n);
int vph_last_fri(vph_session *, uint8_t *roots, uint64_t roots_cap, uint64_t *final_pairs, uint64_t *r_pairs);
int64_t vph_last_fft_gkr(vph_session *, uint64_t *pairs, uint64_t cap_elems);
void vph_last_pc_times(vph_session *, double out[3]);
int vph_last_point(vph_session *, uint64_t *pairs, int cap);
void vph_interactive_breakdown(vph_session *, double out[3]);
void vph_test_sha3(const uint8_t *in, uint8_t *out, uint64_t n);
int vph_fri_commit(vph_session *, const uint64_t *r_pairs, int n_steps, uint8_t *roots, uint64_t *final_pairs, char *err, int errlen);
int vph_fri_commit_batched(vph_session *, const uint64_t *r_pairs, int n_steps, uint8_t *roots, uint64_t *final_pairs, char *err, int errlen);
int vph_commit_private_masked(vph_session *, const uint64_t *mask_pairs, uint64_t n_mask, uint8_t root[32], double *ms, char *err, int errlen);
int vph_commit_public_eq(vph_session *, const uint64_t *point_pairs, int n_point, uint8_t out[32 + 16 + 65 * 16], double *ms, char *err, int errlen);
int vph_fri_open_many(vph_session *, int n, const int32_t *oracle, const uint64_t *leaf, uint64_t *values_pairs, uint8_t *paths, int path_stride,
                      int32_t *path_len, char *err, int errlen);
int vph_fri_query(vph_session *, int n_queries, const uint64_t *leaf0, uint8_t *out, uint64_t capacity, uint64_t *n_written, char *err, int errlen);
int vph_prove_full(vph_session *, uint8_t *transcript, uint64_t capacity, uint64_t *n_written, int batched, char *err,
                   int errlen);
int vph_draw_protocol_tape(vph_session *);
int vph_prove_protocol(vph_session *, uint8_t *transcript, uint64_t capacity, uint64_t *n_written, uint8_t *fri_roots, uint64_t roots_cap,
                       uint64_t *final_pairs, double sec[6], char *err, int errlen);
enum { VPH_PASS_DEFERRED = 1, VPH_PASS_QUEUE_NEXT = 2 };
int vph_prove_protocol_ex(vph_session *, uint8_t *transcript, uint64_t capacity, uint64_t *n_written, uint8_t *fri_roots, uint64_t roots_cap,
                          uint64_t *final_pairs, double sec[6], int flags, char *err, int errlen);
int vph_verify_transcript(vph_circuit *, const uint8_t *transcript, uint64_t n, int skip_predicates);
int vph_prove_fs(vph_session *, uint8_t *proof, uint64_t capacity, uint64_t *n_written, vph_result *res, char *err, int errlen);
int vph_verify_fs(vph_circuit *, const uint8_t *proof, uint64_t n);
double vph_commit_device_ms(vph_session *);
int vph_set_shard(vph_session *, int rank, int world);
int vph_shard_vu_partials(vph_session *, uint64_t *partials, int capacity);
int vph_shard_vu_set(vph_session *, const uint64_t *sums, int n);
int vph_shard_chains(vph_session *, int32_t *owner, double *cost, int capacity);

#ifdef __cplusplus
}
#endif
#endif
```

Baseline: 162.4 billion field-ops/s.

## Defer private/public commitment Merkle hashing into the batched FRI commit launch

Adds a late-hash mode, on by default in prove_protocol, where private and public commitment leaf hashing and Merkle building are skipped at commit time. They are instead merged into the multi-tree leaf-hash and Merkle launches of vp_fri_commit. Any API that needs those trees first forces the outstanding hashing. The aim is fewer kernel launches and better GPU occupancy for the small Merkle top levels, at the cost of roots being filled in later and extra bookkeeping. Correctness depends on the root pointers staying valid until the FRI callback runs.

```diff
diff --git a/include/vpgpu.h b/include/vpgpu.h
--- a/include/vpgpu.h
+++ b/include/vpgpu.h
@@ -123,6 +123,7 @@
 int vp_set_deferred(vp_ctx *, int on);
 int vp_flush(vp_ctx *, int count);
 int vp_pending(vp_ctx *, int *n);
+int vp_pc_hash_late(vp_ctx *, int on);
 int vp_phase_ms(vp_ctx *, double out[5]);
 int vp_commit_private_state(vp_ctx *, uint64_t *epoch, int *valid);
 
diff --git a/virgo-plus_amd/__init__.py b/virgo-plus_amd/__init__.py
--- a/virgo-plus_amd/__init__.py
+++ b/virgo-plus_amd/__init__.py
@@ -116,6 +116,7 @@
         L.vp_warm.argtypes = [vp, ctypes.c_uint32]
         L.vp_flush.argtypes = [vp, ctypes.c_int]
         L.vp_pending.argtypes = [vp, ctypes.POINTER(ctypes.c_int)]
+        L.vp_pc_hash_late.argtypes = [vp, ctypes.c_int]
         L.vp_phase_ms.argtypes = [vp, ctypes.POINTER(ctypes.c_double)]
         L.vp_commit_private.argtypes = [vp, vp]
         L.vp_fft_gkr_sizes.argtypes = [ctypes.c_int, vp, vp]
@@ -905,7 +906,7 @@
         if lib_host().vph_draw_protocol_tape(self.h):
             raise RuntimeError("draw_protocol_tape: the commitment needs an input layer of at least 2^7 wires")
 
-    def prove_protocol(self, deferred=False, queue_next=False):
+    def prove_protocol(self, deferred=False, queue_next=False, hash_per_call=False):
         import numpy as np
         if not hasattr(self, "_pp"):
             cap = self._cap + 32 + 32 + 16 + 65 * 16
@@ -913,7 +914,7 @@
                         (ctypes.c_double * 6)(), ctypes.c_uint64(0), ctypes.create_string_buffer(512))
         buf, cap, roots, fin, sec, n, err = self._pp
         rc = lib_host().vph_prove_protocol_ex(self.h, ctypes.cast(buf, ctypes.c_void_p), cap, ctypes.byref(n), ctypes.cast(roots, ctypes.c_void_p), len(roots),
-                                              fin.ctypes.data, sec, (1 if deferred or queue_next else 0) | (2 if queue_next else 0), err, len(err))
+                                              fin.ctypes.data, sec, (1 if deferred or queue_next else 0) | (2 if queue_next else 0) | (4 if hash_per_call else 0), err, len(err))
         if rc:
             raise RuntimeError("prove_protocol failed: " + err.value.decode())
         st = self.circuit.layer_bitlen(0) - 6
diff --git a/virgo-plus_amd/csrc/vpgpu.hip b/virgo-plus_amd/csrc/vpgpu.hip
--- a/virgo-plus_amd/csrc/vpgpu.hip
+++ b/virgo-plus_amd/csrc/vpgpu.hip
@@ -219,6 +219,9 @@
     bool pc_dry = false;
     unsigned char *h_pub = nullptr; size_t h_pub_cap = 0;
     u64 private_epoch = 0;
+    int hash_late = 0;
+    unsigned pc_unhashed = 0;
+    uint8_t *late_root[2] = {nullptr, nullptr};
 
     PcShard *pcs = nullptr;
     FgkState *fgk = nullptr;
@@ -290,6 +293,7 @@
 };
 #define VP_LOCK(ctx) CtxLock vp_ctx_lock_(ctx, false)
 int flush_pending(vp_ctx *ctx, size_t count);
+int pc_hash_outstanding(vp_ctx *ctx, unsigned which);
 #define VP_ENTER_Q(ctx) CtxLock vp_ctx_lock_(ctx, true); do { HIPCHK(hipSetDevice((ctx)->device)); if ((ctx)->tail_active) (void) tail_quit(ctx); (ctx)->tail_suspended = false; (ctx)->tail_lost = false; (ctx)->ring_call = 0; } while (0)
 #define VP_ENTER(ctx) VP_ENTER_Q(ctx); do { if (!(ctx)->pending.empty()) VPCHK(flush_pending((ctx), (size_t) -1)); } while (0)
 
@@ -1076,6 +1080,7 @@
     (void) hipSetDevice(ctx->device);
     if (ctx->tail_active) (void) tail_quit(ctx);
     (void) hipStreamSynchronize(ctx->stream);
+    (void) pc_hash_outstanding(ctx, 3u);
     vp_free_shard_state(ctx);
     rs_free(ctx);
     vp_free_comm(ctx);
@@ -1110,6 +1115,7 @@
     if (n_layers > VP_MAX_TAB) { ctx->err = "too many layers"; return VP_ELIMIT; }
     RandKeep keep_callers_random_stream;
     VP_ENTER(ctx);
+    VPCHK(pc_hash_outstanding(ctx, 3u));
     HIPCHK(hipStreamSynchronize(ctx->stream));
     if (ctx->gkr_graph) { (void) hipGraphExecDestroy(ctx->gkr_graph); ctx->gkr_graph = nullptr; }
     ctx->graph_failed = false; ctx->plan_tuned = false; ctx->plan_tune_cached = false;
@@ -1323,6 +1329,7 @@
 int vp_evaluate(vp_ctx *ctx, const vp_F *inputs, uint64_t n_inputs) {
     if (!ctx || !inputs || ctx->n_layers < 2 || n_inputs != ctx->L[0].size) return VP_EINVAL;
     VP_ENTER(ctx);
+    VPCHK(pc_hash_outstanding(ctx, 3u));
     LayerDev &L0 = ctx->L[0];
     ctx->pc_private_done = false; ctx->pc_public_done = false; ctx->pc_mask_ms = 0;
     HIPCHK(hipEventRecord(ctx->ev0, ctx->stream));
@@ -1874,7 +1881,14 @@
 int vp_flush(vp_ctx *ctx, int count) {
     if (!ctx) return VP_EINVAL;
     VP_ENTER_Q(ctx);
-    return flush_pending(ctx, count < 0 ? (size_t) -1 : (size_t) count);
+    VPCHK(flush_pending(ctx, count < 0 ? (size_t) -1 : (size_t) count));
+    return ctx->hash_late ? VP_OK : pc_hash_outstanding(ctx, 3u);
+}
+int vp_pc_hash_late(vp_ctx *ctx, int on) {
+    if (!ctx) return VP_EINVAL;
+    VP_ENTER_Q(ctx);
+    ctx->hash_late = on ? 1 : 0;
+    return VP_OK;
 }
 int vp_phase_ms(vp_ctx *ctx, double out[5]) {
     if (!ctx || !out) return VP_EINVAL;
diff --git a/virgo-plus_amd/csrc/vpgpu_pc.inc b/virgo-plus_amd/csrc/vpgpu_pc.inc
--- a/virgo-plus_amd/csrc/vpgpu_pc.inc
+++ b/virgo-plus_amd/csrc/vpgpu_pc.inc
@@ -330,6 +330,27 @@
     return VP_OK;
 }
 
+int pc_hash_outstanding(vp_ctx *ctx, unsigned which) {
+    which &= ctx->pc_unhashed;
+    if (!which) return VP_OK;
+    if (ctx->L.empty() || !ctx->pc_cw || !ctx->pc_tree) { ctx->pc_unhashed = 0; ctx->err = "internal: unhashed oracle without its codeword"; return VP_EINVAL; }
+    const int n = ctx->L[0].bl;
+    const u32 N = 1u << (n - 6), n_leaves = 1u << (n - 2);
+    uint8_t got[2][32];
+    for (int o = 0; o < 2; ++o) {
+        if (!(which >> o & 1)) continue;
+        const F *cw = o ? ctx->pc_hcw : ctx->pc_cw;
+        Dig *tree = o ? ctx->pc_tree_h : ctx->pc_tree;
+        PC_PROF(VP_K_LEAF_HASH, nblk(n_leaves), 1, (u64) n_leaves * (64 * 32 + 32), (u64) n_leaves * 65, pc_launch_leaf_hash(ctx, cw, N, tree + n_leaves));
+        VPCHK(pc_merkle(ctx, tree, n_leaves));
+        HIPCHK(hipMemcpyAsync(got[o], tree + 1, 32, hipMemcpyDeviceToHost, ctx->stream));
+    }
+    ctx->pc_unhashed &= ~which;
+    VPCHK(check_stream(ctx));
+    for (int o = 0; o < 2; ++o) if ((which >> o & 1) && ctx->late_root[o]) { memcpy(ctx->late_root[o], got[o], 32); ctx->late_root[o] = nullptr; }
+    return VP_OK;
+}
+
 int pcs_commit_private(vp_ctx *ctx, uint8_t root[32]);
 int pcs_commit_public(vp_ctx *ctx, const vp_F *pub, uint64_t n_pub, const vp_F *point, vp_F *inner, vp_F all_sum[65], uint8_t root_h[32]);
 int pcs_fri_commit(vp_ctx *ctx, const vp_F *r, int n_steps, uint8_t *roots);
@@ -367,6 +388,7 @@
     if (oracle < 0 || ctx->L.empty()) return VP_EINVAL;
     if (oracle >= VP_OPEN_MAX_ORACLES) { ctx->err = "FRI level not committed yet"; return VP_EINVAL; }
     if (ctx->pcs) return pcs_open_desc(ctx, oracle, d);
+    VPCHK(pc_hash_outstanding(ctx, 3u));
     const int n = ctx->L[0].bl, ln = n - 6, lm = n - 1;
     const u32 N = 1u << ln, M = 1u << lm;
     if (oracle == 0) { if (!ctx->pc_private_done) return VP_EINVAL; d->cw = ctx->pc_cw; d->tree = ctx->pc_tree; d->Nc = N; d->n_leaves = M >> 1; }
@@ -520,6 +542,8 @@
                           const vp_F *pub_mask = nullptr, uint64_t n_pub_mask = 0) {
     const int n = ctx->L[0].bl, ln = n - 6, lm = n - 1;
     const u32 N = 1u << ln, M = 1u << lm;
+    VPCHK(pc_hash_outstanding(ctx, 2u));
+    const bool late = ctx->hash_late && !pub_mask;
     F *P = ctx->pc_tmp, *ST = ctx->pc_tmp + (size_t) 128 * N, *H = ctx->pc_tmp + (size_t) 256 * N;
     F *parts = ctx->pc_small, *d_inner = ctx->pc_small + 1024, *d_all = ctx->pc_small + 1025;
     const u32 used = (u32) ctx->L[0].size, g = std::min<u32>(1024, nblk(used));
@@ -572,17 +596,19 @@
         hipLaunchKernelGGL(k_mask_hcoef, dim3(nblk((u64) B)), dim3(VP_BLOCK), 0, ctx->stream, (const F *) (t + 4 * B), ms, (u32) B, f_make(ms, 0), t, S0m, d_all + 64);
         VPCHK(pc_mask_encode(ctx, t, ms, ctx->pc_hm_cw));
         pc_launch_leaf_hash_masked(ctx, ctx->pc_hcw, N, ctx->pc_hm_cw, ctx->pc_tree_h + n_leaves);
-    } else
+    } else if (!late)
     PC_PROF(VP_K_LEAF_HASH, nblk(n_leaves), 1, (u64) n_leaves * (64 * 32 + 32), (u64) n_leaves * 65,
             pc_launch_leaf_hash(ctx, ctx->pc_hcw, N, ctx->pc_tree_h + n_leaves));
-    VPCHK(pc_merkle(ctx, ctx->pc_tree_h, n_leaves));
+    if (!late) VPCHK(pc_merkle(ctx, ctx->pc_tree_h, n_leaves));
     unsigned char *st = nullptr;
     VPCHK(ring_alloc(ctx, 32 + 66 * sizeof(F), (void **) &st));
-    HIPCHK(hipMemcpyAsync(st, ctx->pc_tree_h + 1, 32, hipMemcpyDeviceToHost, ctx->stream));
+    if (!late) HIPCHK(hipMemcpyAsync(st, ctx->pc_tree_h + 1, 32, hipMemcpyDeviceToHost, ctx->stream));
     HIPCHK(hipMemcpyAsync(st + 32, d_inner, 66 * sizeof(F), hipMemcpyDeviceToHost, ctx->stream));
     ctx->pc_public_done = true; ctx->fri_step = -1;
-    return defer_end(ctx, ev_a, VP_PH_PUBLIC, [ctx, st, root_h, inner, all_sum](float ms) {
-        memcpy(root_h, st, 32); memcpy(inner, st + 32, sizeof(F)); memcpy(all_sum, st + 32 + sizeof(F), 65 * sizeof(F));
+    if (late) { ctx->pc_unhashed |= 2u; ctx->late_root[1] = root_h; }
+    return defer_end(ctx, ev_a, VP_PH_PUBLIC, [ctx, st, root_h, inner, all_sum, late](float ms) {
+        if (!late) memcpy(root_h, st, 32);
+        memcpy(inner, st + 32, sizeof(F)); memcpy(all_sum, st + 32 + sizeof(F), 65 * sizeof(F));
         ctx->commit_ms = ms;
         return VP_OK;
     });
@@ -600,6 +626,8 @@
     if (n > PC_MAX_N) { ctx->err = "input layer of more than 2^25 wires: the reference's commitment indexes its codeword with int (poly_commit.h:87-166), "
                                    "which overflows at 2^26 wires"; return VP_ELIMIT; }
     const u32 N = 1u << ln, M = 1u << lm;
+    VPCHK(pc_hash_outstanding(ctx, 3u));
+    const bool late = ctx->hash_late && !mask;
     u32 ms = 0;
     if (mask) { VPCHK(pc_mask_geometry(ctx, n_mask, &ms)); VPCHK(flush_pending(ctx, (size_t) -1)); }
     VPCHK(pc_root_table(ctx, lm));
@@ -626,6 +654,11 @@
         VPCHK(pc_mask_lde(ctx, mask, n_mask, ms, ctx->pc_lm_cw));
         pc_launch_leaf_hash_masked(ctx, ctx->pc_cw, N, ctx->pc_lm_cw, ctx->pc_tree + n_leaves);
         ctx->pc_mask_ms = ms;
+    } else if (late) {
+        ctx->pc_unhashed |= 1u; ctx->late_root[0] = root;
+        ctx->pc_private_done = true; ++ctx->private_epoch;
+        ctx->pc_public_done = false;
+        return defer_end(ctx, ev_a, VP_PH_PRIVATE, [ctx](float ms) { ctx->commit_ms = ms; return VP_OK; });
     } else
     PC_PROF(VP_K_LEAF_HASH, nblk(n_leaves), 1, (u64) n_leaves * (64 * 32 + 32), (u64) n_leaves * 65,
             pc_launch_leaf_hash(ctx, ctx->pc_cw, N, ctx->pc_tree + n_leaves));
@@ -797,6 +830,7 @@
     if (ctx->pcs) { VP_ENTER(ctx); return pcs_fri_step(ctx, r, root); }
     if (!ctx->pc_public_done) return VP_EINVAL;
     VP_ENTER(ctx);
+    VPCHK(pc_hash_outstanding(ctx, 3u));
     const int n = ctx->L[0].bl, ln = n - 6, lm = n - 1;
     const u32 N = 1u << ln, M = 1u << lm;
     if (!ctx->pc_fri_all) {
@@ -874,6 +908,7 @@
     if (n_steps > ln || n_steps > VP_FRI_MAX) { ctx->err = "too many FRI steps"; return VP_EINVAL; }
     if (ctx->pc_mask_ms) {
         VPCHK(flush_pending(ctx, (size_t) -1));
+        VPCHK(pc_hash_outstanding(ctx, 3u));
         double ms_sum = 0;
         for (int k = 0; k < n_steps; ++k) { VPCHK(vp_fri_step(ctx, r + k, roots + 32 * (size_t) k)); ms_sum += ctx->commit_ms; }
         ctx->commit_ms = ms_sum;
@@ -894,6 +929,20 @@
     ctx->fri_cw_off.clear(); ctx->fri_tree_off.clear();
     FriLeafArgs la{}; MerkleArgs ma{};
     u32 blocks = 0; size_t cw_off = 0;
+    if (n_steps + 2 > VP_FRI_MAX) VPCHK(pc_hash_outstanding(ctx, 3u));
+    const unsigned merged = ctx->pc_unhashed;
+    uint8_t *late_root[2] = {nullptr, nullptr};
+    int ne = 0;
+    for (int o = 0; o < 2; ++o) {
+        if (!(merged >> o & 1)) continue;
+        Dig *tree = o ? ctx->pc_tree_h : ctx->pc_tree;
+        const u32 n_leaves = M >> 1;
+        ma.tree[ne] = tree; ma.count[ne] = n_leaves;
+        la.cw[la.n] = o ? ctx->pc_hcw : ctx->pc_cw; la.leaves[la.n] = tree + n_leaves; la.N[la.n] = N; blocks += nblk(n_leaves); ++la.n;
+        late_root[ne] = ctx->late_root[o];
+        ++ne;
+    }
+    const int nt = ne + n_steps;
     const bool fold3 = n_steps >= 3 && ln >= 9;
     for (int k = 0; k < n_steps; ++k) {
         const u32 Nk = N >> k, No = Nk >> 1;
@@ -941,7 +990,7 @@
                                    host_inv_real(2), 0, 0u));
         const u32 n_leaves = 16 * No;
         Dig *tree = ctx->pc_fri_tree + ctx->fri_tree_used;
-        ma.tree[k] = tree; ma.count[k] = n_leaves;
+        ma.tree[ne + k] = tree; ma.count[ne + k] = n_leaves;
         {
             la.cw[la.n] = out; la.leaves[la.n] = tree + n_leaves; la.N[la.n] = No; blocks += nblk(n_leaves); ++la.n;
         }
@@ -949,11 +998,12 @@
         ctx->fri_tree_used += 2 * (size_t) n_leaves;
     }
     u64 all_leaves = 0;
-    for (int k = 0; k < n_steps; ++k) all_leaves += ma.count[k];
+    for (int k = 0; k < nt; ++k) all_leaves += ma.count[k];
     if (la.n) PC_PROF(VP_K_LEAF_HASH, blocks, la.n, all_leaves * (64 * 32 + 32), all_leaves * 65, pc_launch_leaf_hash_multi(ctx, la));
+    if (merged) { ctx->pc_unhashed = 0; ctx->late_root[0] = ctx->late_root[1] = nullptr; }
     for (;;) {
         MerkleArgs lv{}; u32 b = 0;
-        for (int k = 0; k < n_steps; ++k) {
+        for (int k = 0; k < nt; ++k) {
             const u32 c = ma.count[k] >> 1;
             if (c <= 512) continue;
             lv.tree[lv.n] = ma.tree[k]; lv.count[lv.n] = c; lv.blk_start[lv.n] = b; b += nblk(c); ++lv.n;
@@ -965,17 +1015,24 @@
         for (int q = 0; q < lv.n; ++q) hs += lv.count[q];
         PC_PROF(VP_K_MERKLE, b, lv.n, 96ull * hs, hs, hipLaunchKernelGGL(k_merkle_level_multi, dim3(b), dim3(VP_BLOCK), 0, ctx->stream, lv));
     }
-    ma.n = n_steps;
+    ma.n = nt;
     {
         u64 hs = 0;
-        for (int k = 0; k < n_steps; ++k) hs += ma.count[k] ? ma.count[k] - 1 : 0;
-        PC_PROF(VP_K_MERKLE, n_steps, n_steps, 96ull * hs, hs, hipLaunchKernelGGL(k_merkle_top_multi, dim3(n_steps), dim3(VP_BLOCK), 0, ctx->stream, ma, d_roots));
-    }
-    void *st = nullptr;
-    VPCHK(ring_alloc(ctx, (size_t) 32 * n_steps, &st));
-    HIPCHK(hipMemcpyAsync(st, d_roots, (size_t) 32 * n_steps, hipMemcpyDeviceToHost, ctx->stream));
+        for (int k = 0; k < nt; ++k) hs += ma.count[k] ? ma.count[k] - 1 : 0;
+        PC_PROF(VP_K_MERKLE, nt, nt, 96ull * hs, hs, hipLaunchKernelGGL(k_merkle_top_multi, dim3(nt), dim3(VP_BLOCK), 0, ctx->stream, ma, d_roots));
+    }
+    unsigned char *st = nullptr;
+    VPCHK(ring_alloc(ctx, (size_t) 32 * nt, (void **) &st));
+    HIPCHK(hipMemcpyAsync(st, d_roots, (size_t) 32 * nt, hipMemcpyDeviceToHost, ctx->stream));
     ctx->fri_step = n_steps;
-    return defer_end(ctx, ev_a, VP_PH_FRI, [ctx, st, roots, n_steps](float ms) { memcpy(roots, st, (size_t) 32 * n_steps); ctx->commit_ms = ms; return VP_OK; });
+    uint8_t *lr0 = late_root[0], *lr1 = late_root[1];
+    return defer_end(ctx, ev_a, VP_PH_FRI, [ctx, st, roots, n_steps, ne, lr0, lr1](float ms) {
+        if (ne > 0 && lr0) memcpy(lr0, st, 32);
+        if (ne > 1 && lr1) memcpy(lr1, st + 32, 32);
+        memcpy(roots, st + 32 * (size_t) ne, (size_t) 32 * n_steps);
+        ctx->commit_ms = ms;
+        return VP_OK;
+    });
 }
 
 int vp_fri_final(vp_ctx *ctx, vp_F *final_code) {
@@ -1018,6 +1075,7 @@
     if (!ctx || !values || !path || !path_len || oracle < 0) return VP_EINVAL;
     VP_ENTER(ctx);
     if (ctx->pcs) return pcs_fri_open(ctx, oracle, leaf, values, path, path_capacity, path_len);
+    VPCHK(pc_hash_outstanding(ctx, 3u));
     const int n = ctx->L[0].bl, ln = n - 6, lm = n - 1;
     const u32 N = 1u << ln, M = 1u << lm;
     const F *cw; const Dig *tree; u32 Nc, n_leaves;
diff --git a/virgo-plus_amd/csrc/vpgpu_pc_shard.inc b/virgo-plus_amd/csrc/vpgpu_pc_shard.inc
--- a/virgo-plus_amd/csrc/vpgpu_pc_shard.inc
+++ b/virgo-plus_amd/csrc/vpgpu_pc_shard.inc
@@ -666,6 +666,7 @@
 int vp_pc_load_input(vp_ctx *ctx, const vp_F *inputs, uint64_t n_inputs, int bit_length) {
     if (!ctx || !inputs || bit_length < 7 || bit_length > 30 || n_inputs == 0 || n_inputs > (1ull << bit_length)) return VP_EINVAL;
     VP_ENTER(ctx);
+    VPCHK(pc_hash_outstanding(ctx, 3u));
     HIPCHK(hipStreamSynchronize(ctx->stream));
     if (ctx->gkr_graph) { (void) hipGraphExecDestroy(ctx->gkr_graph); ctx->gkr_graph = nullptr; }
     free_plan(ctx);
@@ -701,6 +702,7 @@
     if (world > 1 && ln - lw < 1) { ctx->err = "vp_pc_set_shard: slice too short for this many ranks"; return VP_ELIMIT; }
     if (world > 1 && ln > PC_MAX_LN_LONG) { ctx->err = "vp_pc_set_shard: input layer of more than 2^25 wires"; return VP_ELIMIT; }
     VP_ENTER(ctx);
+    VPCHK(pc_hash_outstanding(ctx, 3u));
     HIPCHK(hipStreamSynchronize(ctx->stream));
     vp_free_shard_state(ctx);
     if (world == 1 && !(ctx->cm && ctx->cm->comm && ctx->cm->world == 1)) return VP_OK;
diff --git a/virgo-plus_amd/host/vphost.cpp b/virgo-plus_amd/host/vphost.cpp
--- a/virgo-plus_amd/host/vphost.cpp
+++ b/virgo-plus_amd/host/vphost.cpp
@@ -533,11 +533,14 @@
         auto since = [](clk::time_point t) { return std::chrono::duration<double>(clk::now() - t).count(); };
         const auto t0 = clk::now();
         static const bool fft_sync = getenv("VPH_FFT_GKR_SYNC") != nullptr;
+        static const bool hash_per_call_env = getenv("VPH_HASH_PER_CALL") != nullptr;
+        const bool hash_once = !hash_per_call_env && !(flags & VPH_PASS_HASH_PER_CALL);
         u64 nt = 0, nb = 0;
         s->p->gkrSizes(nt, nb);
         if (s->tape.size() != nt) throw std::runtime_error("the tape has the wrong length");
         s->pp_gkr.resize(nb); s->pp_all.resize(65); s->pp_roots.resize((size_t) 32 * ln); s->pp_final.resize(2048);
         chk(vp_set_deferred(ctx, defer ? 1 : 0), "vp_set_deferred");
+        chk(vp_pc_hash_late(ctx, hash_once ? 1 : 0), "vp_pc_hash_late");
         uint64_t epoch = 0; int valid = 0;
         chk(vp_commit_private_state(ctx, &epoch, &valid), "vp_commit_private_state");
         const bool have_head = s->head_queued && valid && epoch == s->head_epoch;
@@ -564,6 +567,7 @@
         chk(vp_fri_commit(ctx, reinterpret_cast<const vp_F *>(s->ptape_fri.data()), ln, s->pp_roots.data()), "vp_fri_commit");
         chk(vp_fri_final(ctx, reinterpret_cast<vp_F *>(s->pp_final.data())), "vp_fri_final");
         s_fri = since(t);
+        chk(vp_pc_hash_late(ctx, 0), "vp_pc_hash_late");
         int n_mine = 0;
         chk(vp_pending(ctx, &n_mine), "vp_pending");
         if (queue_next) {
@@ -598,6 +602,7 @@
         if (sec) { sec[0] = since(t0); sec[1] = s_priv; sec[2] = s_gkr; sec[3] = s_pub; sec[4] = s_fft; sec[5] = s_fri; }
         return 0;
     } catch (const std::exception &e) {
+        (void) vp_pc_hash_late(ctx, 0);
         (void) vp_flush(ctx, -1);
         (void) vp_set_deferred(ctx, 0);
         s->head_queued = false;
diff --git a/virgo-plus_amd/host/vphost.h b/virgo-plus_amd/host/vphost.h
--- a/virgo-plus_amd/host/vphost.h
+++ b/virgo-plus_amd/host/vphost.h
@@ -85,7 +85,7 @@
 int vph_draw_protocol_tape(vph_session *);
 int vph_prove_protocol(vph_session *, uint8_t *transcript, uint64_t capacity, uint64_t *n_written, uint8_t *fri_roots, uint64_t roots_cap,
                        uint64_t *final_pairs, double sec[6], char *err, int errlen);
-enum { VPH_PASS_DEFERRED = 1, VPH_PASS_QUEUE_NEXT = 2 };
+enum { VPH_PASS_DEFERRED = 1, VPH_PASS_QUEUE_NEXT = 2, VPH_PASS_HASH_PER_CALL = 4 };
 int vph_prove_protocol_ex(vph_session *, uint8_t *transcript, uint64_t capacity, uint64_t *n_written, uint8_t *fri_roots, uint64_t roots_cap,
                           uint64_t *final_pairs, double sec[6], int flags, char *err, int errlen);
 int vph_verify_transcript(vph_circuit *, const uint8_t *transcript, uint64_t n, int skip_predicates);
```

New measurement: 164.6 billion field-ops/s (median of 6 runs). +1.3%, better.
